# maxpit/human-pose-estimation

Measured on AMD Instinct MI355X. Metric: images/sec (224x224, batch 256/GPU), higher is better.
Workload: dtype f32; 1 GPU; batch=256/GPU 224x224x3 synthetic images, fp32 ResNet-50 v1 + 3-iter regressor + SMPL LBS at all 3 stages (configs[1] at batch 256; the BASELINE metric batch); global_batch=256, parallelism=dp1 (batch shard, replicated weights), regressor=synthetic 'survey' variant, input=float32 images resident in HBM

## Files before the change

human-pose-estimation_amd/_lib.py:

```python
from __future__ import annotations

import ctypes as C
import os

import numpy as np

_HERE = os.path.dirname(os.path.abspath(__file__))
LIB_PATH = os.path.join(_HERE, "lib", "libhpe_hip.so")

NUM_CONV = 53
NUM_DENSE = 3
NUM_CRITIC_DENSE = 9
NUM_VERTS = 6890
THETA_DIM = 85
FEATURE_DIM = 2048


class HpeError(RuntimeError):
    pass


class HpeConfig(C.Structure):
    _fields_ = [
        ("struct_size", C.c_int),
# ... 109 lines not shown
                ("shift", C.c_void_p), ("y", C.c_void_p), ("split_k", C.POINTER(C.c_int))]


CONV_KERNELS = ("f32", "f32s", "bf16", "bf16_p8", "halo3", "wino", "wino_fused", "wino4", "wino4_fused")
BLOCK_JOINS = ("separate", "dual", "chain")


class HpeConvRoute(C.Structure):
    _fields_ = [("struct_size", C.c_int), ("kernel", C.c_int), ("mode", C.c_int), ("tile", C.c_int), ("in_slab8", C.c_int), ("out_slab8", C.c_int),
                ("join", C.c_int), ("join_kernel", C.c_int), ("join_tile", C.c_int), ("next_slab8", C.c_int), ("packs", C.c_uint), ("reserved", C.c_int)]


def conv_route(lib, cfg, idx, B, concurrent=False, residual=False, workspace=True):
    r = HpeConvRoute(struct_size=C.sizeof(HpeConvRoute))
    check(lib.hpe_debug_conv_route(C.byref(cfg), int(idx), int(B), int(concurrent), int(residual), int(workspace), C.byref(r)))
    return r


ENCODER_PACKINGS = ("w", "w_split", "wino_u", "wino4_u", "stem_w", "scale", "shift", "w_dual", "w_dual_split", "shift_dual", "dxw", "flat")

OUTPUT_FIELDS = ("verts", "joints", "cams", "theta", "J_transformed", "kp2d", "verts2d", "Rs")


class HpeOutputs(C.Structure):
    _fields_ = [(n, C.c_void_p) for n in OUTPUT_FIELDS]


REDUCE_FN = C.CFUNCTYPE(C.c_int, C.c_void_p, C.c_void_p, C.c_longlong, C.c_void_p)

_PROTOS = {
    "hpe_last_error": (C.c_char_p, []),
    "hpe_version": (C.c_char_p, []),
    "hpe_conv_layer_name": (C.c_char_p, [C.c_int]),
    "hpe_bn_layer_name": (C.c_char_p, [C.c_int]),
    "hpe_conv_layer_geometry": (C.c_int, [C.c_int, C.POINTER(C.c_int)]),
    "hpe_config_init": (None, [C.POINTER(HpeConfig)]),
    "hpe_create": (C.c_int, [C.POINTER(HpeConfig), C.POINTER(C.c_void_p)]),
    "hpe_destroy": (C.c_int, [C.c_void_p]),
    "hpe_load_smpl": (C.c_int, [C.c_void_p, C.POINTER(HpeSmplModel)]),
    "hpe_load_conv": (C.c_int, [C.c_void_p, C.c_int] + [C.c_void_p] * 6),
    "hpe_load_dense": (C.c_int, [C.c_void_p, C.c_int, C.c_void_p, C.c_void_p]),
    "hpe_load_mean_theta": (C.c_int, [C.c_void_p, C.c_void_p]),
    "hpe_finalize": (C.c_int, [C.c_void_p]),
    "hpe_forward": (C.c_int, [C.c_void_p, C.c_void_p, C.c_int, C.POINTER(HpeOutputs), C.c_int, C.c_void_p]),
    "hpe_forward_pipelined": (C.c_int, [C.c_void_p, C.c_void_p, C.c_int, C.POINTER(HpeOutputs), C.c_int, C.c_void_p]),
    "hpe_join": (C.c_int, [C.c_void_p, C.c_void_p]),
    "hpe_tail": (C.c_int, [C.c_void_p, C.c_void_p, C.c_int, C.POINTER(HpeOutputs), C.c_int, C.c_void_p]),
    "hpe_tail_stream": (C.c_void_p, [C.c_void_p]),
    "hpe_encoder": (C.c_int, [C.c_void_p, C.c_void_p, C.c_int, C.c_void_p, C.c_void_p]),
    "hpe_regress_stage": (C.c_int, [C.c_void_p, C.c_void_p, C.c_void_p, C.c_int, C.c_void_p, C.c_void_p]),
    "hpe_smpl": (C.c_int, [C.c_void_p, C.c_void_p, C.c_int, C.POINTER(HpeOutputs), C.c_void_p]),
    "hpe_smpl_backward": (C.c_int, [C.c_void_p, C.c_void_p, C.c_int, C.POINTER(HpeOutputs), C.c_void_p, C.c_void_p]),
    "hpe_orth_proj": (C.c_int, [C.c_void_p, C.c_void_p, C.c_int, C.c_int, C.c_void_p, C.c_void_p]),
    "hpe_reproject_vertices": (C.c_int, [C.c_void_p, C.c_void_p, C.c_int, C.c_int, C.c_float, C.c_float, C.c_void_p, C.c_void_p]),
    "hpe_preprocess_u8": (C.c_int, [C.c_void_p, C.c_int, C.c_int, C.c_int, C.c_void_p, C.POINTER(C.c_int), C.c_void_p]),
    "hpe_preprocess_u8_batch": (C.c_int, [C.c_void_p, C.POINTER(C.c_longlong), C.POINTER(C.c_int), C.c_int, C.c_int, C.c_void_p, C.POINTER(C.c_int),
                                          C.c_void_p, C.c_void_p]),
    "hpe_augment_plan": (C.c_int, [C.c_int, C.c_void_p, C.c_void_p, C.c_void_p, C.c_void_p, C.c_void_p, C.c_int, C.c_void_p, C.c_void_p, C.c_void_p]),
    "hpe_augment_batch": (C.c_int, [C.c_void_p, C.c_void_p, C.c_void_p, C.c_void_p, C.c_void_p, C.c_int, C.c_void_p, C.c_void_p, C.c_void_p, C.c_void_p]),
    "hpe_adam_advance": (C.c_int, [C.c_void_p, C.c_double, C.c_double, C.c_double, C.c_void_p]),
    "hpe_adam_apply": (C.c_int, [C.c_void_p, C.c_void_p, C.c_void_p, C.c_void_p, C.c_longlong, C.c_void_p, C.c_float, C.c_float, C.c_float, C.c_void_p]),
    "hpe_adam_set_step": (C.c_int, [C.c_void_p, C.c_longlong, C.c_double, C.c_double, C.c_void_p]),
    "hpe_debug_adam_power": (C.c_int, [C.c_double, C.c_longlong, C.POINTER(C.c_double)]),
    "hpe_jpeg_info": (C.c_int, [C.c_int, C.c_void_p, C.c_void_p, C.c_void_p]),
    "hpe_jpeg_decode": (C.c_int, [C.c_int, C.c_void_p, C.c_void_p, C.c_void_p, C.c_int, C.c_void_p, C.c_longlong, C.c_void_p, C.c_void_p, C.c_void_p]),
    "hpe_jpeg_backend": (C.c_int, [C.c_void_p, C.c_void_p, C.c_int, C.c_void_p, C.c_longlong, C.c_void_p, C.c_longlong, C.c_void_p, C.c_longlong,
                                   C.c_void_p]),
    "hpe_jpeg_encode_layout": (C.c_int, [C.c_int, C.c_void_p, C.c_void_p, C.c_int, C.c_int, C.c_int, C.c_void_p, C.c_void_p]),
    "hpe_jpeg_forward": (C.c_int, [C.c_void_p, C.c_void_p, C.c_int, C.c_void_p, C.c_longlong, C.c_void_p, C.c_longlong, C.c_void_p]),
    "hpe_jpeg_entropy_encode": (C.c_int, [C.c_void_p, C.c_int, C.c_void_p, C.c_longlong, C.c_int, C.c_int, C.c_int, C.c_int, C.c_void_p, C.c_longlong,
                                          C.c_void_p, C.c_void_p]),
    "hpe_png_backend": (C.c_int, [C.c_void_p, C.c_void_p, C.c_int, C.c_void_p, C.c_longlong, C.c_void_p, C.c_longlong, C.c_void_p, C.c_longlong,
                                  C.c_void_p]),
    "hpe_png_filter": (C.c_int, [C.c_void_p, C.c_void_p, C.c_int, C.c_void_p, C.c_longlong, C.c_void_p, C.c_longlong, C.c_void_p]),
    "hpe_draw_panels": (C.c_int, [C.c_void_p] * 6 + [C.c_int, C.c_int, C.c_int, C.c_void_p, C.c_void_p]),
    "hpe_draw_skeleton": (C.c_int, [C.c_void_p] * 4 + [C.c_int, C.c_int, C.c_int, C.c_int, C.c_int, C.c_void_p]),
    "hpe_get_original": (C.c_int, [C.c_void_p, C.c_void_p, C.c_int, C.c_int, C.c_int, C.POINTER(C.c_int), C.c_float, C.c_int, C.c_void_p, C.POINTER(C.c_float), C.c_void_p, C.c_void_p, C.c_void_p]),
    "hpe_kp_loss": (C.c_int, [C.c_void_p, C.c_void_p, C.c_int, C.c_int, C.c_void_p, C.c_void_p]),
    "hpe_kp_loss_backward": (C.c_int, [C.c_void_p, C.c_void_p, C.c_int, C.c_int, C.c_void_p, C.c_void_p, C.c_void_p]),
    "hpe_mesh_loss": (C.c_int, [C.c_void_p, C.c_void_p, C.c_void_p, C.c_int, C.c_int, C.c_int, C.c_int, C.c_void_p, C.c_void_p]),
    "hpe_mesh_loss_grad": (C.c_int, [C.c_void_p, C.c_void_p, C.c_void_p, C.c_int, C.c_int, C.c_int, C.c_int, C.c_void_p, C.c_void_p, C.c_void_p,
                                     C.c_void_p, C.c_void_p]),
    "hpe_val_losses": (C.c_int, [C.c_void_p, C.c_void_p, C.c_void_p, C.POINTER(C.c_void_p), C.POINTER(C.c_void_p), C.c_int, C.c_int, C.c_int,
                                 C.c_int, C.c_int, C.c_int, C.c_void_p, C.c_void_p]),
    "hpe_critic_layer_name": (C.c_char_p, [C.c_int]),
    "hpe_critic_layer_shape": (C.c_int, [C.c_int, C.POINTER(C.c_int)]),
    "hpe_load_critic": (C.c_int, [C.c_void_p, C.POINTER(HpeCriticModel)]),
    "hpe_critic": (C.c_int, [C.c_void_p, C.c_void_p, C.c_int, C.c_void_p, C.c_int, C.c_void_p, C.c_int, C.c_void_p, C.c_void_p, C.c_void_p]),
    "hpe_critic_backward": (C.c_int, [C.c_void_p, C.c_void_p, C.c_int, C.c_void_p, C.c_int, C.c_void_p, C.c_int, C.c_void_p, C.c_void_p,
                                      C.c_void_p, C.c_void_p, C.c_void_p, C.c_void_p]),
    "hpe_critic_param_floats": (C.c_int, []),
    "hpe_critic_param_offset": (C.c_int, [C.c_int, C.c_int]),
    "hpe_critic_weight_grad_ws_floats": (C.c_longlong, [C.c_int]),
    "hpe_critic_reserve": (C.c_int, [C.c_void_p, C.c_int]),
    "hpe_critic_weight_grad": (C.c_int, [C.c_void_p, C.c_void_p, C.c_int, C.c_void_p, C.c_int, C.c_void_p, C.c_int, C.c_void_p, C.c_void_p,
                                         C.c_void_p, C.c_void_p, C.c_void_p, C.c_int, C.c_void_p, C.c_void_p]),
    "hpe_critic_get_params": (C.c_int, [C.c_void_p, C.c_void_p, C.c_void_p]),
    "hpe_critic_set_params_dev": (C.c_int, [C.c_void_p, C.c_void_p, C.c_void_p]),
    "hpe_regressor_param_floats": (C.c_int, []),
    "hpe_regressor_param_offset": (C.c_int, [C.c_int, C.c_int]),
    "hpe_regressor_get_params": (C.c_int, [C.c_void_p, C.c_void_p, C.c_void_p]),
    "hpe_regressor_set_params_dev": (C.c_int, [C.c_void_p, C.c_void_p, C.c_void_p]),
    "hpe_regressor_forward_train": (C.c_int, [C.c_void_p, C.c_void_p, C.c_int, C.c_void_p, C.c_void_p, C.c_void_p]),
    "hpe_regressor_backward": (C.c_int, [C.c_void_p, C.c_void_p, C.c_int, C.c_void_p, C.c_void_p, C.c_void_p, C.c_void_p, C.c_void_p]),
    "hpe_encoder_param_floats": (C.c_int, []),
    "hpe_encoder_param_offset": (C.c_int, [C.c_int, C.c_int]),
    "hpe_encoder_train_reserve": (C.c_int, [C.c_void_p, C.c_int]),
    "hpe_encoder_train_ws_floats": (C.c_longlong, [C.c_int]),
    "hpe_encoder_wg_slices": (C.c_int, [C.c_int, C.c_int]),
    "hpe_encoder_forward_train": (C.c_int, [C.c_void_p, C.c_void_p, C.c_int, C.c_void_p, C.c_void_p]),
    "hpe_encoder_backward": (C.c_int, [C.c_void_p, C.c_void_p, C.c_int, C.c_void_p, C.c_void_p, C.c_void_p]),
    "hpe_encoder_get_params": (C.c_int, [C.c_void_p, C.c_void_p, C.c_void_p]),
    "hpe_encoder_set_params": (C.c_int, [C.c_void_p, C.c_void_p]),
    "hpe_encoder_set_params_dev": (C.c_int, [C.c_void_p, C.c_void_p, C.c_void_p]),
    "hpe_debug_encoder_packing_bytes": (C.c_longlong, [C.c_void_p, C.c_int, C.c_int]),
    "hpe_debug_encoder_packing": (C.c_int, [C.c_void_p, C.c_int, C.c_int, C.c_void_p, C.c_void_p]),
    "hpe_debug_conv_backward": (C.c_int, [C.c_void_p, C.c_int, C.c_void_p, C.c_void_p, C.c_void_p, C.c_int, C.c_void_p, C.c_void_p, C.c_void_p]),
    "hpe_debug_maxpool_backward": (C.c_int, [C.c_void_p, C.c_void_p, C.c_int, C.c_int, C.c_int, C.c_void_p, C.c_void_p]),
    "hpe_debug_avgpool_backward": (C.c_int, [C.c_void_p, C.c_int, C.c_int, C.c_int, C.c_void_p, C.c_void_p]),
    "hpe_debug_encoder_stash": (C.c_int, [C.c_void_p, C.c_int, C.c_void_p, C.c_void_p]),
    "hpe_debug_encoder_stash_batch": (C.c_int, [C.c_void_p]),
    "hpe_encoder_stat_floats": (C.c_int, []),
    "hpe_encoder_stat_offset": (C.c_int, [C.c_int, C.c_int]),
    "hpe_encoder_train_reserve_batchnorm": (C.c_int, [C.c_void_p, C.c_int]),
    "hpe_encoder_train_ws_floats_batchnorm": (C.c_longlong, [C.c_int]),
    "hpe_debug_encoder_bn_slices": (C.c_int, [C.c_int, C.c_int]),
    "hpe_encoder_forward_batchnorm": (C.c_int, [C.c_void_p, C.c_void_p, C.c_int, C.c_void_p, C.c_void_p]),
    "hpe_encoder_backward_batchnorm": (C.c_int, [C.c_void_p, C.c_void_p, C.c_int, C.c_void_p, C.c_void_p, C.c_void_p]),
    "hpe_encoder_get_stats": (C.c_int, [C.c_void_p, C.c_void_p, C.c_void_p]),
    "hpe_encoder_update_stats": (C.c_int, [C.c_void_p, C.c_void_p, C.c_double, C.c_int, C.c_void_p]),
    "hpe_encoder_set_stats_dev": (C.c_int, [C.c_void_p, C.c_void_p, C.c_void_p]),
    "hpe_debug_conv_batchnorm": (C.c_int, [C.c_void_p, C.c_int, C.c_void_p, C.c_int, C.c_void_p, C.c_int, C.c_void_p, C.c_void_p, C.c_void_p, C.c_void_p]),
    "hpe_debug_conv_backward_batchnorm": (C.c_int, [C.c_void_p, C.c_int, C.c_void_p, C.c_void_p, C.c_void_p, C.c_void_p, C.c_int, C.c_void_p, C.c_void_p,
                                                    C.c_void_p]),
    "hpe_debug_encoder_stash_raw": (C.c_int, [C.c_void_p, C.c_int, C.c_void_p, C.c_void_p]),
    "hpe_debug_encoder_batch_stats": (C.c_int, [C.c_void_p, C.c_void_p, C.c_void_p]),
    "hpe_encoder_set_reduce": (C.c_int, [C.c_void_p, REDUCE_FN, C.c_void_p, C.c_int]),
    "hpe_debug_bn_sums": (C.c_int, [C.c_void_p, C.c_int, C.c_void_p, C.c_int, C.c_void_p, C.c_void_p]),
    "hpe_debug_bn_finish": (C.c_int, [C.c_void_p, C.c_int, C.c_void_p, C.c_longlong, C.c_void_p, C.c_int, C.c_void_p, C.c_int, C.c_void_p, C.c_void_p,
                                      C.c_void_p]),
    "hpe_debug_bn_backward_sums": (C.c_int, [C.c_void_p, C.c_int, C.c_void_p, C.c_void_p, C.c_void_p, C.c_int, C.c_void_p, C.c_longlong, C.c_void_p,
                                             C.c_void_p]),
    "hpe_debug_bn_backward_finish": (C.c_int, [C.c_void_p, C.c_int, C.c_void_p, C.c_void_p, C.c_void_p, C.c_void_p, C.c_int, C.c_void_p, C.c_void_p,
                                               C.c_longlong, C.c_void_p, C.c_void_p, C.c_void_p]),
    "hpe_device_status": (C.c_int, [C.c_void_p, C.c_void_p]),
    "hpe_debug_conv": (C.c_int, [C.c_void_p, C.c_int, C.c_void_p, C.c_int, C.c_void_p, C.c_int, C.c_void_p, C.c_void_p]),
    "hpe_debug_chain": (C.c_int, [C.c_void_p, C.c_int, C.c_void_p, C.c_void_p, C.c_int, C.c_void_p, C.c_void_p, C.POINTER(C.c_int), C.c_void_p]),
    "hpe_debug_stem": (C.c_int, [C.c_void_p, C.c_void_p, C.c_int, C.c_int, C.c_void_p, C.c_void_p]),
    "hpe_debug_gemm": (C.c_int, [C.c_void_p, C.c_void_p, C.c_void_p, C.c_int, C.c_int, C.c_int, C.c_int, C.c_int, C.c_void_p, C.c_int, C.c_void_p, C.c_void_p]),
    "hpe_debug_gemm_ex": (C.c_int, [C.c_void_p, C.POINTER(HpeDebugGemm), C.c_void_p]),
    "hpe_debug_gemm_check": (C.c_int, [C.POINTER(HpeDebugGemm), C.c_int, C.c_int]),
    "hpe_debug_gemm_launch": (C.c_int, [C.c_void_p, C.POINTER(HpeDebugGemm), C.c_int, C.c_int, C.c_void_p]),
    "hpe_debug_conv_route": (C.c_int, [C.POINTER(HpeConfig), C.c_int, C.c_int, C.c_int, C.c_int, C.c_int, C.POINTER(HpeConvRoute)]),
    "hpe_debug_maxpool": (C.c_int, [C.c_void_p, C.c_int, C.c_int, C.c_int, C.c_void_p, C.c_void_p]),
    "hpe_debug_avgpool": (C.c_int, [C.c_void_p, C.c_int, C.c_int, C.c_int, C.c_void_p, C.c_void_p]),
    "hpe_debug_joint_regress": (C.c_int, [C.c_void_p, C.c_void_p, C.c_int, C.c_int, C.c_void_p, C.c_void_p]),
    "hpe_enable_timing": (C.c_int, [C.c_void_p, C.c_int]),
    "hpe_get_timings": (C.c_int, [C.c_void_p, C.POINTER(C.c_float)]),
    "hpe_get_span_stats": (C.c_int, [C.c_void_p, C.POINTER(C.c_float), C.POINTER(C.c_int)]),
    "hpe_get_loss_timings": (C.c_int, [C.c_void_p, C.POINTER(C.c_float)]),
    "hpe_debug_set_loss_counter": (C.c_int, [C.c_void_p, C.c_void_p]),
    "hpe_get_conv_timings": (C.c_int, [C.c_void_p, C.POINTER(C.c_float)]),
    "hpe_render_params_init": (None, [C.POINTER(HpeRenderParams)]),
    "hpe_renderer_create": (C.c_int, [C.c_int, C.c_void_p, C.c_int, C.c_int, C.c_int, C.POINTER(C.c_void_p)]),
    "hpe_renderer_destroy": (C.c_int, [C.c_void_p]),
    "hpe_render": (C.c_int, [C.c_void_p, C.c_void_p, C.c_void_p, C.c_int, C.c_int, C.c_int, C.c_void_p, C.POINTER(HpeRenderParams), C.c_void_p,
                             C.c_void_p]),
    "hpe_debug_render_ids": (C.c_int, [C.c_void_p, C.c_void_p, C.c_void_p, C.c_int, C.c_int, C.c_int, C.POINTER(HpeRenderParams), C.c_void_p,
                                       C.c_void_p, C.c_void_p]),
    "hpe_debug_render_vertices": (C.c_int, [C.c_void_p, C.c_void_p, C.c_void_p, C.c_int, C.c_int, C.c_int, C.POINTER(HpeRenderParams),
                                            C.c_void_p, C.c_void_p]),
}

_lib = None


def load():
    global _lib
    if _lib is not None:
        return _lib
    if not os.path.exists(LIB_PATH):
        raise HpeError(
            "%s not found: build it with `python -c 'import __graft_entry__ as g; g.build()'` "
            "(hipcc --offload-arch=gfx950).  There is no CPU fallback." % LIB_PATH
        )
    try:
        import torch
    except Exception:
        pass
    lib = C.CDLL(LIB_PATH, mode=C.RTLD_GLOBAL)
    for name, (res, args) in _PROTOS.items():
        fn = getattr(lib, name)
        fn.restype = res
        fn.argtypes = args
    _lib = lib
    return lib


def declared_symbols():
    return sorted(_PROTOS)


def check(rc):
    if rc != 0:
        msg = load().hpe_last_error()
        raise HpeError("libhpe_hip error %d: %s" % (rc, msg.decode() if msg else "?"))


def f32(a):
    arr = np.ascontiguousarray(a, dtype=np.float32)
    return arr, arr.ctypes.data_as(C.c_void_p)
```

human-pose-estimation_amd/build.py:

```python
from __future__ import annotations

import os
import shutil
import subprocess
import sys

HERE = os.path.dirname(os.path.abspath(__file__))
CSRC = os.path.join(HERE, "csrc")
LIBDIR = os.path.join(HERE, "lib")
LIB = os.path.join(LIBDIR, "libhpe_hip.so")
SOURCES = ["conv_gemm.hip", "conv_gemm_f32s.hip", "conv_gemm_bf16.hip", "conv_gemm_bf16_p8.hip", "conv_chain_bf16.hip", "conv_chain_f32.hip", "conv3_halo_bf16.hip", "conv_wino.hip", "conv_wino4.hip", "stem_fused.hip", "encoder_ops.hip", "smpl.hip", "losses.hip", "prepost.hip", "render.hip", "hpe_plan.hip", "hpe_finalize.hip", "hpe_encoder.hip", "hpe_api.hip", "hpe_render_api.hip", "smpl_bwd.hip", "critic.hip", "critic_train.hip", "regressor_train.hip", "augment.hip", "encoder_train.hip", "encoder_grad.hip", "encoder_repack.hip", "encoder_bn.hip", "jpeg_entropy.hip", "jpeg_decode.hip", "jpeg_huffman_enc.hip", "jpeg_encode.hip", "png_decode.hip", "png_encode.hip", "draw.hip", "adam.hip"]
CFLAGS = ["--offload-arch=gfx950", "-O3", "-std=c++17", "-fPIC", "-fvisibility=hidden", "-fno-fast-math"]


def _hipcc():
    for cand in (os.environ.get("HIPCC"), shutil.which("hipcc"), "/opt/rocm/bin/hipcc"):
        if cand and os.path.exists(cand):
            return cand
    raise RuntimeError("hipcc not found (set HIPCC or install ROCm under /opt/rocm)")


def _deps():
    return [os.path.join(CSRC, f) for f in os.listdir(CSRC) if f.endswith(".h")] + [os.path.join(HERE, "..", "include", "hpe.h")]


def _obj_stale(src, obj):
    if not os.path.exists(obj):
        return True
    t = os.path.getmtime(obj)
    return any(os.path.getmtime(d) > t for d in [src] + _deps() if os.path.exists(d))


def _flags_now():
    return " ".join(CFLAGS + os.environ.get("HPE_EXTRA_FLAGS", "").split())


def built_flags():
    tag = os.path.join(LIBDIR, "obj", "flags.txt")
    return open(tag).read() if os.path.exists(tag) else ""


def _stale():
    if not os.path.exists(LIB):
        return True
    if built_flags() != _flags_now():
        return True
    t = os.path.getmtime(LIB)
    deps = [os.path.join(CSRC, f) for f in os.listdir(CSRC)] + [os.path.join(HERE, "..", "include", "hpe.h")]
    return any(os.path.getmtime(d) > t for d in deps if os.path.exists(d))


def build(force=False, verbose=False):
    if not force and not _stale():
        return LIB
    os.makedirs(LIBDIR, exist_ok=True)
    objdir = os.path.join(LIBDIR, "obj")
    os.makedirs(objdir, exist_ok=True)
    extra = os.environ.get("HPE_EXTRA_FLAGS", "").split()
    tag = os.path.join(objdir, "flags.txt")
    flags_now = _flags_now()
    if force or not os.path.exists(tag) or open(tag).read() != flags_now:
        for f in os.listdir(objdir):
            os.remove(os.path.join(objdir, f))
    hipcc = _hipcc()
    jobs = []
    for s in SOURCES:
        src = os.path.join(CSRC, s)
        if not os.path.exists(src):
            continue
        obj = os.path.join(objdir, s.replace(".hip", ".o"))
        jobs.append((src, obj))

    def compile_one(job):
        src, obj = job
        if not _obj_stale(src, obj):
            return None
        cmd = [hipcc] + CFLAGS + extra + ["-c", "-o", obj + ".tmp%d" % os.getpid(), src]
        if verbose:
            print(" ".join(cmd), file=sys.stderr)
        r = subprocess.run(cmd, capture_output=True, text=True)
        if r.returncode != 0:
            return "hipcc failed on %s:\n%s%s" % (os.path.basename(src), r.stdout, r.stderr)
        os.replace(obj + ".tmp%d" % os.getpid(), obj)
        return None

    from concurrent.futures import ThreadPoolExecutor

    with ThreadPoolExecutor(max_workers=min(len(jobs), max(1, (os.cpu_count() or 2) - 1))) as ex:
        errs = [e for e in ex.map(compile_one, jobs) if e]
    if errs:
        raise RuntimeError("\n".join(errs))
    open(tag, "w").write(flags_now)
    tmp = LIB + ".tmp%d" % os.getpid()
    cmd = [hipcc, "--offload-arch=gfx950", "-shared", "-fPIC", "-o", tmp] + [o for _, o in jobs]
    r = subprocess.run(cmd, capture_output=True, text=True)
    if r.returncode != 0:
        raise RuntimeError("link failed:\n" + r.stdout + r.stderr)
    os.replace(tmp, LIB)
    return LIB


if __name__ == "__main__":
    print(build(force="--force" in sys.argv, verbose=True))
```

human-pose-estimation_amd/csrc/conv_gemm_common.h:

```cpp
#pragma once
#include <hip/hip_runtime.h>

#include "hpe_internal.h"

#define BK 32

namespace {

struct RowAddr {
    int base;
    unsigned mask;
};

template <int MODE, int CHUNK = 1>
__device__ __forceinline__ RowAddr make_row(const GemmArgs& p, int m, int c) {
    RowAddr r;
    r.mask = 0x1ffu;
    if (m >= p.M) m = p.M - 1;
    if (MODE == GEMM_DENSE || MODE == GEMM_DUAL) {
        r.base = m * p.lda + c * CHUNK;
    } else {
        const int hw = p.Ho * p.Wo;
        const int b = m / hw;
        const int rem = m - b * hw;
        const int ho = rem / p.Wo;
        const int wo = rem - ho * p.Wo;
        if (MODE == GEMM_STRIDED) {
            r.base = ((b * p.Hi + ho * p.stride) * p.Wi + wo * p.stride) * p.Cin + c * CHUNK;
        } else if (MODE == GEMM_CONV3) {
            r.base = ((b * p.Hi + ho) * p.Wi + wo) * p.Cin + c * CHUNK;
            unsigned mk = 0;
#pragma unroll
            for (int tap = 0; tap < 9; ++tap) {
                const int dh = tap / 3 - 1, dw = tap % 3 - 1;
                if ((unsigned)(ho + dh) < (unsigned)p.Hi && (unsigned)(wo + dw) < (unsigned)p.Wi) mk |= 1u << tap;
            }
            r.mask = mk;
        } else {
            r.base = ((b * p.Hi + 2 * ho + (c * CHUNK >> 5)) * p.Wi + 2 * wo) * 4 + (c * CHUNK & 31);
        }
    }
    return r;
}

struct SlabPos {
    int off;
    int tap;
    int cs;
};

template <int MODE, int SLAB = BK, int STEM_ROWS = 1>
__device__ __forceinline__ void slab_advance(const GemmArgs& p, SlabPos& sp) {
    if (MODE == GEMM_DENSE || MODE == GEMM_STRIDED || MODE == GEMM_DUAL) {
        sp.off += SLAB;
    } else if (MODE == GEMM_CONV3) {
        sp.cs += 1;
        sp.off += SLAB;
        if (sp.cs == p.cin_slabs) {
            sp.cs = 0;
            sp.tap += 1;
            const int kh = sp.tap / 3;
            sp.off = ((kh - 1) * p.Wi + (sp.tap - kh * 3 - 1)) * p.Cin;
        }
    } else {
        sp.off += STEM_ROWS * p.Wi * 4;
    }
}

template <int MODE>
__device__ __forceinline__ SlabPos slab_first(const GemmArgs& p) {
    SlabPos sp;
    sp.tap = 0;
    sp.cs = 0;
    sp.off = (MODE == GEMM_CONV3) ? (-p.Wi - 1) * p.Cin : 0;
    return sp;
}

template <int MODE>
__device__ __forceinline__ SlabPos slab_seek(const GemmArgs& p, int slab) {
    SlabPos sp;
    sp.tap = 0;
    sp.cs = 0;
    if (MODE == GEMM_DENSE || MODE == GEMM_STRIDED || MODE == GEMM_DUAL) {
        sp.off = slab * BK;
    } else if (MODE == GEMM_CONV3) {
        sp.tap = slab / p.cin_slabs;
        sp.cs = slab - sp.tap * p.cin_slabs;
        const int kh = sp.tap / 3;
        sp.off = ((kh - 1) * p.Wi + (sp.tap - kh * 3 - 1)) * p.Cin + sp.cs * BK;
    } else {
        sp.off = slab * p.Wi * 4;
    }
    return sp;
}

#ifdef HPE_F32_RES_NT
#define HPE_RES_LOAD(ptr) __builtin_nontemporal_load(ptr)
#else
#define HPE_RES_LOAD(ptr) (*(ptr))
#endif
template <int BM, int BN, int WM, int WN, int NP>
__device__ __forceinline__ void conv_epilogue(const GemmArgs& p, float* lds, f32x16 (&acc)[BM / WM / 32][BN / WN / 32], int m0, int n0, int t,
                                              int lane, int wm, int wn, const f32x4 (&rpre)[NP], bool use_pre) {
    constexpr int MT = BM / WM / 32;
    constexpr int NT = BN / WN / 32;
    constexpr int NTHR = 64 * WM * WN;
    constexpr int EP = BN + 4;
    {
        const int col_l = lane & 31;
        const int row_l = 4 * (lane >> 5);
#pragma unroll
        for (int j = 0; j < NT; ++j) {
            const int cl = (wn * NT + j) * 32 + col_l;
            const int n = n0 + cl;
            const bool n_ok = n < p.N;
            const float sc = n_ok ? p.scale[n] : 0.f;
            const float sh = n_ok ? p.shift[n] : 0.f;
#pragma unroll
            for (int i = 0; i < MT; ++i) {
                const int rl = (wm * MT + i) * 32 + row_l;
#pragma unroll
                for (int e = 0; e < 16; ++e) lds[(rl + (e & 3) + 8 * (e >> 2)) * EP + cl] = acc[i][j][e] * sc + sh;
            }
        }
    }
    __syncthreads();
    {
        constexpr int TPR = BN / 4;
        constexpr int RPP = NTHR / TPR;
        const int r = t / TPR;
        const int c4 = (t - r * TPR) * 4;
        const int n = n0 + c4;
        const bool full = (n + 3) < p.N;
#pragma unroll
        for (int pass = 0; pass < BM / RPP; ++pass) {
            const int row = pass * RPP + r;
            const int m = m0 + row;
            if (m >= p.M || n >= p.N) continue;
            f32x4 v = *reinterpret_cast<const f32x4*>(&lds[row * EP + c4]);
            if (full) {
                if (use_pre) v += rpre[pass < NP ? pass : 0];
                else if (p.res) v += HPE_RES_LOAD(reinterpret_cast<const f32x4*>(p.res + (size_t)m * p.ldres + n));
                if (p.relu) {
                    v.x = fmaxf(v.x, 0.f);
                    v.y = fmaxf(v.y, 0.f);
                    v.z = fmaxf(v.z, 0.f);
                    v.w = fmaxf(v.w, 0.f);
                }
                if (p.y_slab8)
                    *reinterpret_cast<f32x4*>(p.y + ((size_t)(n >> 3) * p.M + m) * 8 + (n & 7)) = v;
                else
                    *reinterpret_cast<f32x4*>(p.y + (size_t)m * p.ldy + n) = v;
            } else {
                const float vv[4] = {v.x, v.y, v.z, v.w};
#pragma unroll
                for (int u = 0; u < 4; ++u) {
                    if (n + u < p.N) {
                        float o = vv[u];
                        if (p.res) o += p.res[(size_t)m * p.ldres + n + u];
                        if (p.relu) o = fmaxf(o, 0.f);
                        p.y[(size_t)m * p.ldy + n + u] = o;
                    }
                }
            }
        }
    }
}

}
```

human-pose-estimation_amd/csrc/encoder_repack.hip:

```cpp
#include <hip/hip_runtime.h>

#include <string>

#include "hpe_ctx.h"

namespace {

struct RepackLayer {
    float *w, *scale, *shift, *wino_u, *wino4_u, *dxw;
    unsigned short* w_split;
    short kh, wino_split;
    int cin, cout, n_pad, k_pad;
    int off[4];
    int stat;
};

struct RepackDual {
    float *w, *shift;
    unsigned short* split;
    int i2c, i1, K1, K2, N, n_pad;
};

enum { F_WT, F_BN, F_WINO, F_WINO4, F_DXW, F_DUAL, F_COUNT };

// ... 67 lines not shown

__global__ __launch_bounds__(256) void repack_stem_kernel(unsigned short* __restrict__ stem_w, const float* __restrict__ kernel) {
    const int o = blockIdx.x * 256 + threadIdx.x;
    if (o >= 64 * 224) return;
    const int n = o / 224, k = o - n * 224;
    const int kh = k >> 5, kw = (k & 31) >> 2, ci = k & 3;
    float v = 0.f;
    if (kw < 7 && ci < 3) v = kernel[((kh * 7 + kw) * 3 + ci) * 64 + n];
    store_split(stem_w + o, 64 * 224, v);
}

template <int TT>
__global__ __launch_bounds__(256) void repack_wino_kernel(const RepackTable* __restrict__ T, const float* __restrict__ flat) {
    unsigned lb;
    const RepackLayer& L = T->L[find_item(T->F[TT == 4 ? F_WINO : F_WINO4], blockIdx.x, &lb)];
    const int c4 = L.cin / 4;
    const int nb = lb / c4, cb = lb - nb * c4;
    const int n = nb * 64 + (threadIdx.x >> 2), ci = cb * 4 + (threadIdx.x & 3);
    const float* src = flat + L.off[0];
    double g[3][3];
#pragma unroll
    for (int a = 0; a < 3; ++a)
#pragma unroll
        for (int b = 0; b < 3; ++b) g[a][b] = src[(((size_t)a * 3 + b) * L.cin + ci) * L.cout + n];
    float* out = TT == 4 ? L.wino_u + wino_u_base(n, ci, L.cin) : L.wino4_u + wino4_u_base(n, ci, L.cin);
    constexpr size_t step = TT == 4 ? 512 : 256;
#pragma unroll
    for (int xi = 0; xi < TT; ++xi)
#pragma unroll
        for (int nu = 0; nu < TT; ++nu) {
            double gx[3], gn[3];
#pragma unroll
            for (int a = 0; a < 3; ++a) {
                gx[a] = TT == 4 ? wino_g(xi, a) : wino4_g(xi, a);
                gn[a] = TT == 4 ? wino_g(nu, a) : wino4_g(nu, a);
            }
            const float u = wino_elem(gx, gn, g);
            out[(size_t)(xi * TT + nu) * step] = u;
            if (TT == 4 && L.wino_split)
                store_split(wino_u_split_of(L.wino_u, L.cin, L.cout) + wino_us_base(n, ci, L.cin) + (size_t)(xi * 4 + nu) * 512, WINO_US_PIECE, u);
        }
}

__global__ __launch_bounds__(256) void repack_dxw_kernel(const RepackTable* __restrict__ T, const float* __restrict__ flat) {
    unsigned lb;
    const RepackLayer& L = T->L[find_item(T->F[F_DXW], blockIdx.x, &lb)];
    const int taps = L.kh * L.kh, K = taps * L.cout;
    const unsigned o = lb * 256 + threadIdx.x;
    const int ci = (int)(o / (unsigned)K), r = (int)(o - (unsigned)ci * K);
    if (ci >= ((L.cin + 127) / 128) * 128) return;
    const int t = r / L.cout, n = r - t * L.cout;
    L.dxw[o] = ci < L.cin ? flat[L.off[0] + ((size_t)(taps - 1 - t) * L.cin + ci) * L.cout + n] : 0.f;
}

__global__ __launch_bounds__(256) void repack_dual_kernel(const RepackTable* __restrict__ T, const float* __restrict__ flat,
                                                          const float* __restrict__ mean, const double* __restrict__ sd) {
#pragma clang fp contract(off)
    unsigned lb;
    const RepackDual& D = T->D[find_item(T->F[F_DUAL], blockIdx.x, &lb)];
    const int K = D.K1 + D.K2;
    const int kt_n = (K + TILE_K - 1) / TILE_K;
    const int nt = lb / kt_n, kt = lb - nt * kt_n;
    const int k = kt * TILE_K + (threadIdx.x & 63);
    if (k >= K) return;
    const RepackLayer &L2 = T->L[D.i2c], &L1 = T->L[D.i1];
    const RepackLayer& L = k < D.K1 ? L2 : L1;
    const float* src = flat + L.off[0] + (size_t)(k < D.K1 ? k : k - D.K1) * D.N;
    const int n0 = nt * TILE_N + (threadIdx.x >> 6) * 8;
#pragma unroll
    for (int j = 0; j < 8; ++j) {
        const int n = n0 + j;
        if (n >= D.n_pad) break;
        float v = 0.f;
        if (n < D.N) {
            double inv, shift;
            bn_fold_sd(flat[L.off[2] + n], flat[L.off[1] + n], mean[L.stat + n], flat[L.off[3] + n], sd[L.stat + n], &inv, &shift);
            v = (float)(inv * (double)src[n]);
            if (k == 0) {
                double inv1, shift1;
                bn_fold_sd(flat[L1.off[2] + n], flat[L1.off[1] + n], mean[L1.stat + n], flat[L1.off[3] + n], sd[L1.stat + n], &inv1, &shift1);
                D.shift[n] = (float)(shift + shift1);
            }
        }
        D.w[(size_t)n * K + k] = v;
        if (D.split) store_split(D.split + (size_t)n * 3 * K + k, K, v);
    }
}

unsigned blocks_of(int form, const ConvSpec& s, const ConvLayer& L, int idx) {
    switch (form) {
        case F_WT: return (unsigned)(L.n_pad / TILE_N) * ((L.k_pad + TILE_K - 1) / TILE_K);
        case F_BN: return (unsigned)(s.cout + 255) / 256;
        case F_WINO: return L.wino_u ? (unsigned)(s.cin / 4) * (s.cout / 64) : 0;
        case F_WINO4: return L.wino4_u ? (unsigned)(s.cin / 4) * (s.cout / 64) : 0;
        case F_DXW: return (unsigned)((conv_dxw_floats(idx) + 255) / 256);
    }
    return 0;
}

int check_debug(hpe_ctx* c, int idx, int which) {
    if (!c) return fail(HPE_ERR_INVALID, "null ctx");
    if (idx < 0 || idx >= HPE_NUM_CONV || which < 0 || which >= HPE_PACK_COUNT) return fail(HPE_ERR_INVALID, "hpe_debug_encoder_packing: idx or which out of range");
    if (c->dead) return fail(HPE_ERR_STATE, "hpe_finalize failed on this ctx: destroy it and create a new one");
    if (!c->finalized) return fail(HPE_ERR_STATE, "hpe_finalize() has not been called");
    if (!c->have_encoder) return fail(HPE_ERR_STATE, "encoder weights were not loaded before hpe_finalize");
    if (c->bf16) return fail(HPE_ERR_STATE, "hpe_debug_encoder_packing needs an fp32 context");
    return HPE_OK;
}

const void* packing_of(hpe_ctx* c, int idx, int which, size_t* bytes) {
    const ConvSpec& s = specs()[idx];
    const ConvLayer& L = c->conv[idx];
    const size_t wt = (size_t)L.n_pad * L.k_pad, dual = (size_t)round_up(s.cout, 128) * L.k_dual, u = (size_t)s.cin * s.cout;
    const void* p = nullptr;
    size_t n = 0;
    switch (which) {
        case HPE_PACK_W: p = L.w, n = wt * 4; break;
        case HPE_PACK_W_SPLIT: p = L.w_split, n = wt * 3 * 2; break;
        case HPE_PACK_WINO_U: p = L.wino_u, n = u * 16 * 4; break;
        case HPE_PACK_WINO4_U: p = L.wino4_u, n = u * 36 * 4; break;
        case HPE_PACK_STEM_W: p = L.stem_w, n = (size_t)3 * 64 * 224 * 2; break;
        case HPE_PACK_SCALE: p = L.scale, n = (size_t)s.cout * 4; break;
        case HPE_PACK_SHIFT: p = L.shift, n = (size_t)s.cout * 4; break;
        case HPE_PACK_W_DUAL: p = L.w_dual, n = dual * 4; break;
        case HPE_PACK_W_DUAL_SPLIT: p = L.w_dual_split, n = dual * 3 * 2; break;
        case HPE_PACK_SHIFT_DUAL: p = L.shift_dual, n = (size_t)s.cout * 4; break;
        case HPE_PACK_DXW: p = c->et.dxw[idx], n = conv_dxw_floats(idx) * 4; break;
        case HPE_PACK_FLAT:
            if (c->et.flat) p = c->et.flat + layout().off[idx][0];
            n = ((size_t)s.kh * s.kw * s.cin * s.cout + 3 * (size_t)s.cout) * 4;
            break;
    }
    *bytes = p ? n : 0;
    return *bytes ? p : nullptr;
}

}

size_t encoder_repack_reserve_floats() { return (sizeof(RepackTable) + 3) / 4; }

int encoder_repack_reserve(hpe_ctx* c) {
    RepackTable t{};
    for (int i = 0; i < HPE_NUM_CONV; ++i) {
        const ConvSpec& s = specs()[i];
        const ConvLayer& L = c->conv[i];
        RepackLayer& r = t.L[i];
        r.w = L.w;
        r.scale = L.scale;
        r.shift = L.shift;
        r.wino_u = L.wino_u;
        r.wino_split = L.wino_u_split != nullptr;
        r.wino4_u = L.wino4_u;
        r.dxw = c->et.dxw[i];
        r.w_split = static_cast<unsigned short*>(L.w_split);
        r.kh = s.kh;
        r.cin = s.cin;
        r.cout = s.cout;
        r.n_pad = L.n_pad;
        r.k_pad = L.k_pad;
        for (int w = 0; w < 4; ++w) r.off[w] = layout().off[i][w];
        r.stat = layout().stat[i];
        if (s.kh != s.kw || L.n_pad % TILE_N != 0 || ((L.wino_u || L.wino4_u) && (s.cin % 8 != 0 || s.cout % 64 != 0)))
            return fail(HPE_ERR_STATE, std::string("encoder repack: unexpected geometry of ") + s.name);
    }
    for (int f = 0; f < F_DUAL; ++f) {
        RepackForm& F = t.F[f];
        unsigned b = 0;
        for (int i = 0; i < HPE_NUM_CONV; ++i) {
            const unsigned nb = blocks_of(f, specs()[i], c->conv[i], i);
            if (!nb) continue;
            F.item[F.n] = i;
            F.block0[F.n++] = b;
            b += nb;
        }
        F.block0[F.n] = b;
    }
    {
        RepackForm& F = t.F[F_DUAL];
        unsigned b = 0;
        for (const ResBlock& blk : blocks()) {
            if (!blk.first || !c->conv[blk.i2c].w_dual) continue;
            const ConvLayer& L2 = c->conv[blk.i2c];
            RepackDual& d = t.D[F.n];
            d.w = L2.w_dual;
            d.shift = L2.shift_dual;
            d.split = static_cast<unsigned short*>(L2.w_dual_split);
            d.i2c = blk.i2c;
            d.i1 = blk.i1;
            d.K1 = L2.k1_dual;
            d.K2 = L2.k_dual - L2.k1_dual;
            d.N = specs()[blk.i2c].cout;
            d.n_pad = round_up(d.N, 128);
            F.item[F.n] = F.n;
            F.block0[F.n++] = b;
            b += (unsigned)(d.n_pad / TILE_N) * ((L2.k_dual + TILE_K - 1) / TILE_K);
        }
        F.block0[F.n] = b;
    }
    float* p = nullptr;
    int rc = dev_alloc(c, &p, encoder_repack_reserve_floats(), false);
    if (rc) return rc;
    HIP_TRY(hipMemcpy(p, &t, sizeof(t), hipMemcpyHostToDevice));
    c->et.repack = p;
    static_assert(F_COUNT <= 8, "grid array");
    for (int f = 0; f < F_COUNT; ++f) c->et.repack_grid[f] = t.F[f].block0[t.F[f].n];
    return HPE_OK;
}

hipError_t encoder_repack_launch(hpe_ctx* c, const float* flat, hipStream_t st) {
    const EncTrainWork& w = c->et;
    const RepackTable* T = static_cast<const RepackTable*>(w.repack);
    const unsigned* grid = w.repack_grid;
    if (grid[F_WT]) hipLaunchKernelGGL(repack_wt_kernel, dim3(grid[F_WT]), dim3(256), 0, st, T, flat);
    if (grid[F_BN]) hipLaunchKernelGGL(repack_bn_kernel, dim3(grid[F_BN]), dim3(256), 0, st, T, flat, w.mean, w.sd);
    if (c->conv[0].stem_w)
        hipLaunchKernelGGL(repack_stem_kernel, grid1(64 * 224), dim3(256), 0, st, static_cast<unsigned short*>(c->conv[0].stem_w),
                           flat + layout().off[0][0]);
    if (grid[F_WINO]) hipLaunchKernelGGL(repack_wino_kernel<4>, dim3(grid[F_WINO]), dim3(256), 0, st, T, flat);
    if (grid[F_WINO4]) hipLaunchKernelGGL(repack_wino_kernel<6>, dim3(grid[F_WINO4]), dim3(256), 0, st, T, flat);
    if (grid[F_DXW]) hipLaunchKernelGGL(repack_dxw_kernel, dim3(grid[F_DXW]), dim3(256), 0, st, T, flat);
    if (grid[F_DUAL]) hipLaunchKernelGGL(repack_dual_kernel, dim3(grid[F_DUAL]), dim3(256), 0, st, T, flat, w.mean, w.sd);
    HIPE(hipGetLastError());
    return hipMemcpyAsync(w.flat, flat, (size_t)layout().total * sizeof(float), hipMemcpyDeviceToDevice, st);
}

hipError_t encoder_repack_stats_launch(hpe_ctx* c, hipStream_t st) {
    const EncTrainWork& w = c->et;
    const RepackTable* T = static_cast<const RepackTable*>(w.repack);
    const unsigned* grid = w.repack_grid;
    if (grid[F_BN]) hipLaunchKernelGGL(repack_bn_kernel, dim3(grid[F_BN]), dim3(256), 0, st, T, w.flat, w.mean, w.sd);
    if (grid[F_DUAL]) hipLaunchKernelGGL(repack_dual_kernel, dim3(grid[F_DUAL]), dim3(256), 0, st, T, w.flat, w.mean, w.sd);
    return hipGetLastError();
}

#pragma GCC visibility push(default)
extern "C" {

long long hpe_debug_encoder_packing_bytes(hpe_ctx* c, int idx, int which) {
    if (!c || idx < 0 || idx >= HPE_NUM_CONV || which < 0 || which >= HPE_PACK_COUNT) return 0;
    if (c->dead || !c->finalized || !c->have_encoder || c->bf16) return 0;
    size_t n;
    packing_of(c, idx, which, &n);
    return (long long)n;
}

int hpe_debug_encoder_packing(hpe_ctx* c, int idx, int which, void* dst, void* stream) {
    int rc = check_debug(c, idx, which);
    if (rc) return rc;
    if (!dst) return fail(HPE_ERR_INVALID, "null dst_dev");
    size_t n;
    const void* p = packing_of(c, idx, which, &n);
    if (!p) return fail(HPE_ERR_STATE, "hpe_debug_encoder_packing: this context does not hold that form of that layer");
    DeviceGuard g(c->cfg.device);
    HIP_TRY(hipMemcpyAsync(dst, p, n, hipMemcpyDeviceToDevice, static_cast<hipStream_t>(stream)));
    return HPE_OK;
}

}
#pragma GCC visibility pop
```

human-pose-estimation_amd/csrc/hpe_api.hip:

```cpp
#include <hip/hip_runtime.h>

#include <algorithm>
#include <cmath>
#include <cstdint>
#include <cstdio>
#include <cstdlib>
#include <cstring>
#include <string>
#include <vector>

#include "gemm_contract.h"
#include "hpe_ctx.h"

namespace {
thread_local std::string g_err;
}

int fail(int code, const std::string& msg) {
    g_err = msg;
    return code;
}

int check_ready(hpe_ctx* c, int B, int need) {
    if (!c) return fail(HPE_ERR_INVALID, "null ctx");
// ... 624 lines not shown
    const ConvSpec& sn = specs()[idx2c + (first ? 2 : 1)];
    const int C2 = first ? specs()[idx2c + 1].cin : 0;
    if (s2.kh != 1 || s2.cout != 4 * s2.cin || sn.kh != 1 || sn.stride != 1 || sn.cin != s2.cout || !hpe_chain_bf16_supported(s2.cin, s2.cout, sn.cout, C2) ||
        (first && (!c->conv[idx2c].w_dual || specs()[idx2c + 1].stride != 1)))
        return fail(HPE_ERR_INVALID, "hpe_debug_chain: idx2c must be the branch2c of a stage-2 / stage-3 block that is followed by an identity block");
    DeviceGuard g(c->cfg.device);
    hipStream_t st = static_cast<hipStream_t>(stream);
    const long M = (long)B * s2.hout * s2.hout;
    HIP_TRY(hpe_launch_f32_to_bf16(t2, c->T2, M * s2.cin, st));
    HIP_TRY(hpe_launch_f32_to_bf16(residual, c->X0, M * (first ? C2 : s2.cout), st));
    HIP_TRY(run_chain(c, idx2c, first, c->T2, c->X0, B, c->X1, c->T1, st));
    HIP_TRY(hpe_launch_bf16_to_f32(c->X1, t3, M * s2.cout, st));
    HIP_TRY(hpe_launch_bf16_to_f32(c->T1, u1, M * sn.cout, st));
    if (occupancy) HIP_TRY(hpe_chain_bf16_occupancy(occupancy));
    return HPE_OK;
}

int hpe_debug_stem(hpe_ctx* c, const float* images, int B, int rows_per_strip, float* y, void* stream) {
    int rc = check_ready(c, B, NEED_ENC);
    if (rc) return rc;
    if (!images || !y) return fail(HPE_ERR_INVALID, "null pointer");
    if (c->bf16) return fail(HPE_ERR_STATE, "hpe_debug_stem works on fp32 contexts only");
    DeviceGuard g(c->cfg.device);
    const int R = rows_per_strip > 0 ? rows_per_strip : hpe_stem_fused_pick_rows(B);
    HIP_TRY(hpe_launch_stem_fused(images, c->conv[0].stem_w, c->conv[0].scale, c->conv[0].shift, y, B, R, 0, static_cast<hipStream_t>(stream)));
    return HPE_OK;
}

static GemmArgs debug_gemm_args(const HpeDebugGemm* g, int slab) {
    static_assert(HPE_GEMM_DENSE == GEMM_DENSE && HPE_GEMM_STRIDED == GEMM_STRIDED && HPE_GEMM_CONV3 == GEMM_CONV3 && HPE_GEMM_DUAL == GEMM_DUAL,
                  "include/hpe.h numbers the modes as GemmMode does");
    GemmArgs p{};
    p.x = g->x, p.x2 = g->x2, p.w = g->wt, p.res = g->residual, p.y = g->y;
    p.M = g->M, p.N = g->N, p.K = g->K;
    p.lda = g->lda, p.ldw = g->ldw, p.ldy = g->ldy, p.ldres = g->ldres, p.w_rows = g->w_rows;
    p.Hi = g->Hi, p.Wi = g->Wi, p.Cin = g->Cin, p.Ho = g->Ho, p.Wo = g->Wo, p.stride = g->stride;
    p.cin_slabs = g->Cin / slab;
    p.k1_slabs = g->k1_slabs;
    p.relu = g->relu;
    p.y_slab8 = g->y_slab8;
    return p;
}

static std::string debug_gemm_refusal(const HpeDebugGemm* g) {
    if (!g) return "null HpeDebugGemm";
    if (g->struct_size != (int)sizeof(HpeDebugGemm))
        return "HpeDebugGemm.struct_size is " + std::to_string(g->struct_size) + ", this library's is " + std::to_string(sizeof(HpeDebugGemm)) +
               " (other revision of include/hpe.h?)";
    if (g->mode != HPE_GEMM_DENSE && g->mode != HPE_GEMM_STRIDED && g->mode != HPE_GEMM_CONV3 && g->mode != HPE_GEMM_DUAL)
        return "HpeDebugGemm.mode must be dense, strided, conv3 or dual";
    return "";
}

static std::string debug_gemm_rejected(const HpeDebugGemm* g, const char* clause) {
    return "mode " + std::to_string(g->mode) + " tile " + std::to_string(g->tile) + " M " + std::to_string(g->M) + " N " + std::to_string(g->N) + " K " +
           std::to_string(g->K) + " is outside the launcher's contract (gemm_contract.h), clause \"" + clause + "\": nothing was launched";
}

int hpe_debug_gemm_ex(hpe_ctx* c, const HpeDebugGemm* g, void* stream) {
    if (g && g->split_k) *g->split_k = 0;
    if (!c || !c->finalized) return fail(HPE_ERR_STATE, "needs a finalized ctx");
    const std::string why = debug_gemm_refusal(g);
    if (!why.empty()) return fail(HPE_ERR_INVALID, why);
    if ((!g->scale || !g->shift) && g->N > 1024) return fail(HPE_ERR_INVALID, "hpe_debug_gemm_ex: N <= 1024 without scale / shift");
    DeviceGuard guard(c->cfg.device);
    GemmArgs p = debug_gemm_args(g, 32);
    p.scale = g->scale ? g->scale : c->ones;
    p.shift = g->shift ? g->shift : c->zeros;
    p.zero = c->zeros;
    if (g->use_splitk) {
        p.partial = c->partial;
        p.partial_floats = c->partial_floats;
    }
    if (const char* clause = gemm_contract(p, g->mode, g->tile, GEMM_K_F32)) return fail(HPE_ERR_INVALID, "hpe_debug_gemm_ex: " + debug_gemm_rejected(g, clause));
    int split_k = 0;
    const hipError_t e = hpe_launch_gemm(p, g->mode, g->tile, c->plan.splitk_min_slabs, static_cast<hipStream_t>(stream), &split_k);
    if (g->split_k) *g->split_k = split_k;
    if (e == hipErrorInvalidValue && split_k == 0) return fail(HPE_ERR_INVALID, "hpe_debug_gemm_ex: the launcher refused the plan's splitk_min_slabs, nothing was launched");
    HIP_TRY(e);
    return HPE_OK;
}

int hpe_debug_gemm_check(const HpeDebugGemm* g, int kernel, int w_piece) {
    const std::string why = debug_gemm_refusal(g);
    if (!why.empty()) return fail(HPE_ERR_INVALID, why);
    if (kernel < GEMM_K_F32 || kernel > GEMM_K_BF16_P8) return fail(HPE_ERR_INVALID, "hpe_debug_gemm_check: kernel must be 0 (fp32), 1 (f32s), 2 (bf16) or 3 (bf16_p8)");
    const GemmKernel k = static_cast<GemmKernel>(kernel);
    GemmArgs p = debug_gemm_args(g, gemm_rules(k).slab);
    alignas(16) static const float present[4] = {};
    p.scale = p.shift = p.zero = present;
    if (k == GEMM_K_F32S) p.w_piece = w_piece;
    if (const char* clause = gemm_contract(p, g->mode, g->tile, k)) return fail(HPE_ERR_INVALID, "hpe_debug_gemm_check: " + debug_gemm_rejected(g, clause));
    return HPE_OK;
}

int hpe_debug_gemm_launch(hpe_ctx* c, const HpeDebugGemm* g, int kernel, int w_piece, void* stream) {
    if (kernel == GEMM_K_F32) return hpe_debug_gemm_ex(c, g, stream);
    if (g && g->split_k) *g->split_k = 0;
    const std::string why = debug_gemm_refusal(g);
    if (!why.empty()) return fail(HPE_ERR_INVALID, why);
    if (kernel < GEMM_K_F32 || kernel > GEMM_K_BF16_P8) return fail(HPE_ERR_INVALID, "hpe_debug_gemm_launch: kernel must be 0 (fp32), 1 (f32s), 2 (bf16) or 3 (bf16_p8)");
    if ((!g->scale || !g->shift) && g->N > 1024) return fail(HPE_ERR_INVALID, "hpe_debug_gemm_launch: N <= 1024 without scale / shift");
    const GemmKernel k = static_cast<GemmKernel>(kernel);
    GemmArgs p = debug_gemm_args(g, gemm_rules(k).slab);
    if (k == GEMM_K_F32S) p.w_piece = w_piece;
    alignas(16) static const float present[4] = {};
    p.scale = g->scale ? g->scale : present;
    p.shift = g->shift ? g->shift : present;
    p.zero = present;
    if (const char* clause = gemm_contract(p, g->mode, g->tile, k)) return fail(HPE_ERR_INVALID, "hpe_debug_gemm_launch: " + debug_gemm_rejected(g, clause));
    if (!c || !c->finalized) return fail(HPE_ERR_STATE, "needs a finalized ctx");
    DeviceGuard guard(c->cfg.device);
    p.scale = g->scale ? g->scale : c->ones;
    p.shift = g->shift ? g->shift : c->zeros;
    p.zero = c->zeros;
    if (g->use_splitk) {
        p.partial = c->partial;
        p.partial_floats = c->partial_floats;
    }
    if (const char* clause = gemm_contract(p, g->mode, g->tile, k)) return fail(HPE_ERR_INVALID, "hpe_debug_gemm_launch: " + debug_gemm_rejected(g, clause));
    int split_k = 1;
    hipStream_t st = static_cast<hipStream_t>(stream);
    const hipError_t e = k == GEMM_K_F32S ? hpe_launch_gemm_f32s(p, g->mode, g->tile, st)
                       : k == GEMM_K_BF16 ? hpe_launch_gemm_bf16(p, g->mode, g->tile, st)
                                          : hpe_launch_gemm_bf16_p8(p, g->mode, st, &split_k);
    if (g->split_k) *g->split_k = split_k;
    HIP_TRY(e);
    return HPE_OK;
}

int hpe_debug_conv_route(const HpeConfig* cfg, int idx, int B, int concurrent, int residual, int workspace, HpeConvRoute* out) {
    static_assert(HPE_CONV_K_F32 == CONV_K_F32 && HPE_CONV_K_HALO3 == CONV_K_HALO3 && HPE_CONV_K_WINO4_FUSED == CONV_K_WINO4_FUSED && HPE_CONV_K_COUNT == CONV_K_WINO4_FUSED + 1,
                  "include/hpe.h numbers the kernels as ConvKernel does");
    if (!cfg || !out) return fail(HPE_ERR_INVALID, "null argument");
    if (cfg->struct_size != (int)sizeof(HpeConfig) || out->struct_size != (int)sizeof(HpeConvRoute))
        return fail(HPE_ERR_INVALID, "hpe_debug_conv_route: HpeConfig.struct_size / HpeConvRoute.struct_size are " + std::to_string(cfg->struct_size) + " / " +
                                         std::to_string(out->struct_size) + ", this library's are " + std::to_string(sizeof(HpeConfig)) + " / " + std::to_string(sizeof(HpeConvRoute)));
    if (idx < 0 || idx >= HPE_NUM_CONV || B < 1) return fail(HPE_ERR_INVALID, "hpe_debug_conv_route: idx must be in [0, HPE_NUM_CONV) and B >= 1");
    const HpePlan pl = hpe_resolve_plan(*cfg);
    const bool bf16 = cfg->encoder_dtype == 1;
    const ConvQuery q{B, concurrent != 0, residual != 0, workspace != 0};
    const ConvRoute r = route_conv(pl, bf16, idx, q);
    *out = HpeConvRoute{(int)sizeof(HpeConvRoute), r.kernel, r.mode, r.tile, r.in_slab8, 0, 0, -1, -1, 0, layer_packs(pl, bf16, idx), 0};
    for (const ResBlock& blk : blocks()) {
        if (idx != blk.i2a && idx != blk.i2c) continue;
        const BlockRoute b = route_block(pl, bf16, blk, q);
        if (idx == blk.i2a) out->out_slab8 = b.r2a.out_slab8;
        if (idx == blk.i2c) out->join = b.join, out->next_slab8 = b.u1_slab8;
        if (idx == blk.i2c && b.join == JOIN_DUAL) out->join_kernel = b.r2c.kernel, out->join_tile = b.r2c.tile;
    }
    return HPE_OK;
}

int hpe_debug_gemm(hpe_ctx* c, const float* x, const float* wt, int M, int N, int K, int w_rows, int tile, const float* residual,
                   int relu, float* y, void* stream) {
    if (!c || !c->finalized || !c->have_regressor) return fail(HPE_ERR_STATE, "needs a finalized ctx with the regressor loaded");
    if (!x || !wt || !y || N > 1024) return fail(HPE_ERR_INVALID, "bad argument (N <= 1024)");
    HpeDebugGemm g{};
    g.struct_size = (int)sizeof(HpeDebugGemm);
    g.mode = HPE_GEMM_DENSE;
    g.tile = tile;
    g.x = x;
    g.wt = wt;
    g.residual = residual;
    g.y = y;
    g.M = M;
    g.N = N;
    g.K = K;
    g.lda = K;
    g.ldw = K;
    g.w_rows = w_rows;
    g.ldy = N;
    g.ldres = N;
    g.relu = relu;
    g.use_splitk = 0;
    return hpe_debug_gemm_ex(c, &g, stream);
}

int hpe_debug_maxpool(const float* x, int B, int H, int C, float* y, void* stream) {
    if (!x || !y || B < 1) return fail(HPE_ERR_INVALID, "bad argument");
    HIP_TRY(hpe_launch_maxpool(x, y, B, H, C, static_cast<hipStream_t>(stream)));
    return HPE_OK;
}

int hpe_debug_avgpool(const float* x, int B, int HW, int C, float* y, void* stream) {
    if (!x || !y || B < 1) return fail(HPE_ERR_INVALID, "bad argument");
    HIP_TRY(hpe_launch_avgpool(x, y, B, HW, C, C, static_cast<hipStream_t>(stream)));
    return HPE_OK;
}

int hpe_debug_joint_regress(hpe_ctx* c, const float* X, int n, int use_kp, float* out, void* stream) {
    if (!c || !c->finalized || !c->have_smpl) return fail(HPE_ERR_STATE, "SMPL not finalized");
    if (!X || !out || n < 1) return fail(HPE_ERR_INVALID, "bad argument");
    DeviceGuard g(c->cfg.device);
    HIP_TRY(hpe_launch_joint_regress(X, use_kp ? c->smpl.kp_reg : c->smpl.j_reg, n, use_kp ? c->num_kp : 24, out, nullptr, nullptr,
                                     static_cast<hipStream_t>(stream)));
    return HPE_OK;
}

int hpe_device_status(hpe_ctx* c, void* stream) {
    if (!c || !c->finalized) return fail(HPE_ERR_STATE, "needs a finalized ctx");
    DeviceGuard g(c->cfg.device);
    HIP_TRY(hipStreamSynchronize(static_cast<hipStream_t>(stream)));
    if (c->dev_err) {
        unsigned w = 0;
        HIP_TRY(hipMemcpy(&w, c->dev_err, sizeof w, hipMemcpyDeviceToHost));
        if (w) {
            (void)hipMemset(c->dev_err, 0, sizeof w);
            return fail(HPE_ERR_HIP, "device error word " + std::to_string(w) +
                                         ": a stream-K wait of the Winograd GEMM timed out, outputs since the last check are invalid");
        }
    }
    return HPE_OK;
}

int hpe_enable_timing(hpe_ctx* c, int enable) {
    if (!c) return fail(HPE_ERR_INVALID, "null ctx");
    c->timing = enable;
    c->span_n = 0;
    c->timed_valid = false;
    c->conv_timed_valid = false;
    return HPE_OK;
}

int hpe_get_timings(hpe_ctx* c, float ms[5]) {
    if (!c || !ms) return fail(HPE_ERR_INVALID, "null argument");
    if (!c->timed_valid) return fail(HPE_ERR_STATE, "no timed call recorded (hpe_enable_timing first)");
    DeviceGuard g(c->cfg.device);
    HIP_TRY(hipEventSynchronize(c->ev[4]));
    for (int i = 0; i < 5; ++i) ms[i] = 0.f;
    HIP_TRY(hipEventElapsedTime(&ms[0], c->ev[0], c->ev[1]));
    HIP_TRY(hipEventElapsedTime(&ms[4], c->ev[0], c->ev[4]));
    if (c->conv_timed_valid) {
        for (int i = 0; i < HPE_NUM_CONV; ++i) {
            float t = 0.f;
            HIP_TRY(hipEventElapsedTime(&t, c->cev0[i], c->cev1[i]));
            ms[1] += t;
        }
    }
    ms[2] = ms[4] - ms[0];
    return HPE_OK;
}

int hpe_get_span_stats(hpe_ctx* c, float ms[3], int* n_calls) {
    if (!c || !ms || !n_calls) return fail(HPE_ERR_INVALID, "null argument");
    if (c->span_n == 0) return fail(HPE_ERR_STATE, "no timed call recorded (hpe_enable_timing first)");
    DeviceGuard g(c->cfg.device);
    const unsigned n = c->span_n < (unsigned)hpe_ctx::SPAN_RING ? c->span_n : (unsigned)hpe_ctx::SPAN_RING;
    double sum = 0.0;
    float lo = 1e30f, hi = 0.f;
    for (unsigned i = 0; i < n; ++i) {
        float t = 0.f;
        HIP_TRY(hipEventSynchronize(c->span1[i]));
        HIP_TRY(hipEventElapsedTime(&t, c->span0[i], c->span1[i]));
        sum += t;
        lo = t < lo ? t : lo;
        hi = t > hi ? t : hi;
    }
    ms[0] = (float)(sum / n);
    ms[1] = lo;
    ms[2] = hi;
    *n_calls = (int)n;
    return HPE_OK;
}

int hpe_get_loss_timings(hpe_ctx* c, float ms[2]) {
    if (!c || !ms) return fail(HPE_ERR_INVALID, "null argument");
    if (c->loss_timed_stages == 0) return fail(HPE_ERR_STATE, "no timed hpe_val_losses call recorded (hpe_enable_timing first)");
    DeviceGuard g(c->cfg.device);
    HIP_TRY(hipEventSynchronize(c->lev_all[1]));
    HIP_TRY(hipEventElapsedTime(&ms[0], c->lev_all[0], c->lev_all[1]));
    ms[1] = 0.f;
    for (int s = 0; s < c->loss_timed_stages; ++s) {
        float t = 0.f;
        HIP_TRY(hipEventElapsedTime(&t, c->lev0[s], c->lev1[s]));
        ms[1] += t;
    }
    return HPE_OK;
}

int hpe_debug_set_loss_counter(hpe_ctx* c, void* counter_dev) {
    if (!c) return fail(HPE_ERR_INVALID, "null ctx");
    c->loss_counter = static_cast<unsigned long long*>(counter_dev);
    return HPE_OK;
}

int hpe_get_conv_timings(hpe_ctx* c, float* ms) {
    if (!c || !ms) return fail(HPE_ERR_INVALID, "null argument");
    if (!c->conv_timed_valid) return fail(HPE_ERR_STATE, "no level-2 timed call recorded");
    DeviceGuard g(c->cfg.device);
    HIP_TRY(hipEventSynchronize(c->ev[4]));
    for (int i = 0; i < HPE_NUM_CONV; ++i) HIP_TRY(hipEventElapsedTime(&ms[i], c->cev0[i], c->cev1[i]));
    return HPE_OK;
}

}
#pragma GCC visibility pop
```

human-pose-estimation_amd/csrc/hpe_ctx.h:

```cpp
#pragma once
#include <hip/hip_runtime.h>

#include <cmath>
#include <cstdint>
#include <cstring>
#include <string>
#include <vector>

#include "../../include/hpe.h"
#include "bf16_split.h"
#include "hpe_internal.h"
#include "hpe_plan.h"

int fail(int code, const std::string& msg);

#define HIP_TRY(expr)                                                                                             \
    do {                                                                                                          \
        hipError_t _e = (expr);                                                                                   \
        if (_e != hipSuccess)                                                                                     \
            return fail(HPE_ERR_HIP, std::string(#expr) + ": " + hipGetErrorString(_e) + " (" __FILE__ ":" +      \
                                         std::to_string(__LINE__) + ")");                                         \
    } while (0)

struct ConvSpec {
    char name[24];
    char bn[24];
    int kh, kw, cin, cout, stride, hin, hout;
};

const std::vector<ConvSpec>& specs();

struct ResBlock {
    int stage;
    bool first, last;
    int i2a, i2b, i2c, i1;
    int in;
};
const std::vector<ResBlock>& blocks();

inline int round_up(int x, int m) { return ((x + m - 1) / m) * m; }

struct ConvLayer {
    std::vector<float> kernel, bias, gamma, beta, mean, var;
    bool loaded = false;
    float* w = nullptr;
    float* scale = nullptr;
    float* shift = nullptr;
    float* w_dual = nullptr;
    float* shift_dual = nullptr;
    int k_dual = 0, k1_dual = 0;
    void* w_split = nullptr;
    void* w_dual_split = nullptr;
    void* stem_w = nullptr;
    float* wino_u = nullptr;
    unsigned short* wino_u_split = nullptr;
    float* wino4_u = nullptr;
    int n_pad = 0, k_pad = 0;
};

inline int conv_wt_k(int idx, int kh, int kw, int ci) {
    const ConvSpec& s = specs()[idx];
    return idx == 0 ? kh * 32 + kw * 4 + ci : (kh * s.kw + kw) * s.cin + ci;
}

inline int conv_k_pad(int idx, bool bf16) { return round_up(idx == 0 ? 7 * 32 : specs()[idx].kh * specs()[idx].kw * specs()[idx].cin, bf16 ? 64 : 32); }


__host__ __device__ inline size_t wino_u_base(int n, int ci, int cin) {
    return ((((size_t)(n >> 6) * (cin / 8) + (ci >> 3)) * 16) * 2 + ((ci >> 2) & 1)) * 256 + (size_t)(n & 63) * 4 + (ci & 3);
}
constexpr size_t WINO_US_PIECE = 16 * 64 * 8;
__host__ __device__ inline size_t wino_us_base(int n, int ci, int cin) {
    return ((size_t)(n >> 6) * (cin / 8) + (ci >> 3)) * 3 * WINO_US_PIECE + (size_t)(n & 63) * 8 + (ci & 7);
}
__host__ __device__ inline unsigned short* wino_u_split_of(float* wino_u, int cin, int cout) {
    return reinterpret_cast<unsigned short*>(wino_u + (size_t)16 * cin * cout);
}
__host__ __device__ inline size_t wino4_u_base(int n, int ci, int cin) {
    return (((size_t)(n >> 6) * (cin / 4) + (ci >> 2)) * 36) * 256 + (size_t)(n & 63) * 4 + (ci & 3);
}
__host__ __device__ inline double wino_g(int xi, int a) {
    constexpr double G[4][3] = {{1, 0, 0}, {0.5, 0.5, 0.5}, {0.5, -0.5, 0.5}, {0, 0, 1}};
    return G[xi][a];
}
__host__ __device__ inline double wino4_g(int xi, int a) {
    constexpr double G4[6][3] = {{0.25, 0, 0}, {-1.0 / 6, -1.0 / 6, -1.0 / 6}, {-1.0 / 6, 1.0 / 6, -1.0 / 6},
                                 {1.0 / 24, 1.0 / 12, 1.0 / 6}, {1.0 / 24, -1.0 / 12, 1.0 / 6}, {0, 0, 1}};
    return G4[xi][a];
}
__host__ __device__ inline float wino_elem(const double gx[3], const double gn[3], const double g[3][3]) {
#pragma clang fp contract(off)
    double u = 0.0;
    for (int a = 0; a < 3; ++a)
        for (int b = 0; b < 3; ++b) u += gx[a] * gn[b] * g[a][b];
    return (float)u;
}

__host__ __device__ inline void bn_fold_sd(float gamma, float bias, float mean, float beta, double sd, double* scale, double* shift) {
#pragma clang fp contract(off)
    *scale = (double)gamma / sd;
    *shift = ((double)bias - (double)mean) * *scale + (double)beta;
}
inline double bn_sd(const ConvLayer& L, int n, float eps) { return std::sqrt((double)L.var[n] + (double)eps); }
inline void bn_fold(const ConvLayer& L, int n, float eps, double* scale, double* shift) {
    bn_fold_sd(L.gamma[n], L.bias[n], L.mean[n], L.beta[n], bn_sd(L, n, eps), scale, shift);
}
inline float bn_istd(const ConvLayer& L, int n, float eps) { return (float)(1.0 / std::sqrt((double)L.var[n] + (double)eps)); }

struct DenseLayer {
    std::vector<float> kernel, bias;
    bool loaded = false;
};

constexpr int STEM_HP = 230;
constexpr int STEM_WP = 232;
constexpr int THETA_LD = 96;
constexpr size_t WINO_V_PITCH = 802816 + 16384;
constexpr size_t WINO_V_SLACK = 524288;


struct RegTrainWork {
    float *w1k = nullptr;
    float *w2k = nullptr;
    float *w3k = nullptr;
    float *p1 = nullptr;
    float *a1 = nullptr, *a2 = nullptr;
    float *th = nullptr;
    float *g = nullptr;
    float *r = nullptr;
    float *da = nullptr;
    float *dz1 = nullptr, *dz2 = nullptr;
    float *sum1 = nullptr;
    float *zeros = nullptr;
    float *partial = nullptr;
    size_t partial_floats = 0;
};

struct EncTrainWork {
    int B = 0;
    int stash_B = 0;
    float *flat = nullptr;
    float *mean = nullptr, *istd = nullptr;
    double *sd = nullptr;
    void *repack = nullptr;
    unsigned repack_grid[8] = {};
    float *stash = nullptr;
    float *g0 = nullptr, *g1 = nullptr;
    float *sbig = nullptr;
    float *t0 = nullptr, *t1 = nullptr, *ssmall = nullptr;
    float *partial = nullptr;
    size_t partial_floats = 0;
    float *dsh = nullptr;
    float *wgp = nullptr;
    float *zeros = nullptr;
    float *feat = nullptr;
    float *dxw[HPE_NUM_CONV] = {};
    int bn_B = 0;
    int bn_stat_B = 0;
    float *zstash = nullptr;
    float *bn_batch = nullptr;
    float *bn_stats = nullptr;
    double *bn_part = nullptr;
    int *bn_hw = nullptr;
    hpe_reduce_fn reduce = nullptr;
    void *reduce_user = nullptr;
    int reduce_G = 0;
    int reduce_failed = -1;
    int bn_stat_G = 0;
};
constexpr int BN_MAX_SLICES = 512;
constexpr int BN_PART_COLS = 262144;
constexpr int WG_MAX_SLICES = 128;
constexpr int WG_WGP_FLOATS = 1152 * 512;
static_assert(WG_WGP_FLOATS >= 3 * 2 * 2048, "the reduce buffers of data-parallel training fit the weight gradient's scratch");
inline size_t conv_dxw_floats(int idx) {
    const ConvSpec& s = specs()[idx];
    return idx == 0 ? 0 : (size_t)round_up(s.cin, 128) * s.kh * s.kw * s.cout;
}
struct EncLayout {
    int off[HPE_NUM_CONV][4];
    int stat[HPE_NUM_CONV];
    size_t stash[HPE_NUM_CONV];
    size_t stash_pool, stash_per_image;
    int total, channels;
};
const EncLayout& layout();

struct hpe_ctx {
    HpeConfig cfg{};
    bool finalized = false;
    bool dead = false;
    HpePlan plan;
    bool bf16 = false;
    bool have_encoder = false, have_regressor = false, have_smpl = false;
    ConvLayer conv[HPE_NUM_CONV];
    DenseLayer dense[HPE_NUM_DENSE];
    bool smpl_loaded = false, mean_loaded = false;
    std::vector<float> h_vt, h_sd, h_pd, h_jreg, h_w, h_kreg;
    std::vector<int> h_par;
    int num_kp = 19;
    float h_mean[HPE_THETA_DIM];
    float *w1f = nullptr, *w1t = nullptr, *w2 = nullptr, *w3 = nullptr, *b1 = nullptr, *b2 = nullptr, *b3 = nullptr;
    float *ones = nullptr, *zeros = nullptr, *mean_dev = nullptr;
    EncTrainWork et{};
    RegTrainWork rt{};
    SmplDev smpl{};
    SmplWork work{};
    SmplBwdWork bwd{};
    float* smpl_basis_src = nullptr;
    float *padded = nullptr, *X0 = nullptr, *X1 = nullptr, *T1 = nullptr, *T2 = nullptr, *SC = nullptr;
    float *feat = nullptr, *P1 = nullptr, *H1 = nullptr, *H2 = nullptr, *thA = nullptr, *thB = nullptr;
    float* critic_buf = nullptr;
    CriticW critic{};
    bool have_critic = false;
    float* critic_ws = nullptr;
    size_t critic_ws_floats = 0;
    float* loss_ws = nullptr;
    size_t loss_ws_floats = 0;
    std::vector<void*> allocs;
    float* partial = nullptr;
    size_t partial_floats = 0;
    float* wino_v = nullptr;
    float* wino_ws = nullptr;
    unsigned* wino_flags = nullptr;
    unsigned* dev_err = nullptr;
    unsigned wino_epoch = 0;
    int n_cu = 0;
    bool loss_attr_done = false;
    unsigned long long* loss_counter = nullptr;
    hipStream_t aux[3]{};
    hipEvent_t ev_fork{}, ev_join[3]{};
    hipStream_t tail_st{};
    hipEvent_t ev_enc{}, ev_tail{}, ev_feat_free[2]{};
    bool feat_free_valid[2] = {false, false};
    bool tail_pending = false;
    unsigned pipe_idx = 0;
    float* feat_alt = nullptr;
    int co_running = 1;
    float* w4_split = nullptr;
    float* partial_tail = nullptr;
    size_t partial_tail_floats = 0;
    bool dense_on_tail = false;
    int timing = 0;
    hipEvent_t ev[8]{};
    static constexpr int SPAN_RING = 64;
    hipEvent_t span0[SPAN_RING]{}, span1[SPAN_RING]{};
    unsigned span_n = 0;
    hipEvent_t cev0[HPE_NUM_CONV]{}, cev1[HPE_NUM_CONV]{};
    hipEvent_t lev0[16]{}, lev1[16]{}, lev_all[2]{};
    int loss_timed_stages = 0;
    bool ev_ok = false, timed_valid = false, conv_timed_valid = false;
};

struct DeviceGuard {
    int prev = -1;
    bool changed = false;
    explicit DeviceGuard(int dev) {
        if (hipGetDevice(&prev) == hipSuccess && prev != dev) changed = hipSetDevice(dev) == hipSuccess;
    }
    ~DeviceGuard() {
        if (changed) (void)hipSetDevice(prev);
    }
};

int dev_alloc(hpe_ctx* c, float** p, size_t n_floats, bool zero);
int upload(hpe_ctx* c, float** p, const std::vector<float>& h);
int upload_split(hpe_ctx* c, void** p, const std::vector<float>& wt, int rows, int K);

#define HIPE(expr)                               \
    do {                                         \
        hipError_t _e = (expr);                  \
        if (_e != hipSuccess) return _e;         \
    } while (0)

enum { NEED_ENC = 1, NEED_REG = 2, NEED_SMPL = 4 };
int check_ready(hpe_ctx* c, int B, int need);

int finalize_impl(hpe_ctx* c);
void release_device_state(hpe_ctx* c);
int repack_encoder(hpe_ctx* c);

hipError_t run_conv(hpe_ctx* c, int idx, const ConvRoute& r, const float* x, int B, const float* res, int relu, float* y, hipStream_t st,
                    float* wino_v = nullptr, int slot = 0, const float* scale = nullptr, const float* shift = nullptr);
hipError_t run_conv_nhwc(hpe_ctx* c, int idx, const float* x, int B, const float* res, int relu, float* y, hipStream_t st,
                         const float* scale = nullptr, const float* shift = nullptr);
hipError_t run_chain(hpe_ctx* c, int i2c, bool first, const float* t2, const float* res, int B, float* t3, float* u1, hipStream_t st,
                     bool u1_slab8 = false);
hipError_t encoder_impl(hpe_ctx* c, const float* images, int B, float* features, int ldfeat, hipStream_t st);
hipError_t run_dense(hpe_ctx* c, const float* x, int lda, int M, int K, const float* w, int w_rows, int N, const float* scale, const float* shift,
                     const float* res, int ldres, int relu, float* y, int ldy, hipStream_t st, float* partial = nullptr, size_t partial_floats = 0);
hipError_t regress_impl(hpe_ctx* c, const float* th_prev, float* th_next, int B, hipStream_t st);
hipError_t features_proj(hpe_ctx* c, const float* features, int B, hipStream_t st);
hipError_t tail_impl(hpe_ctx* c, const float* feat, int B, const HpeOutputs* stage_outs, int n_outs, hipStream_t ts, hipEvent_t feat_free);
hipError_t join_tail(hpe_ctx* c, hipStream_t st);
int forward_impl(hpe_ctx* c, const float* images, int B, const HpeOutputs* stage_outs, int n_outs, hipStream_t st, bool pipelined);

size_t encoder_repack_reserve_floats();
int encoder_repack_reserve(hpe_ctx* c);
hipError_t encoder_repack_launch(hpe_ctx* c, const float* flat_dev, hipStream_t st);

hipError_t encoder_repack_stats_launch(hpe_ctx* c, hipStream_t st);

int bn_slices(int M, int N);
hipError_t bn_launch_stats(const float* z, int M, int N, float eps, double* part, float* mu, float* var, float* r, hipStream_t st);
hipError_t bn_launch_apply(const float* z, const float* mu, const float* r, const float* gamma, const float* beta, const float* res, int relu, float* y,
                           int M, int N, hipStream_t st);
hipError_t bn_launch_bwd_reduce(const float* dy, const float* y, const float* z, const float* mu, const float* r, int M, int N, double* part, float* db,
                                float* dgamma, float* dbeta, hipStream_t st);
hipError_t bn_launch_bwd_apply(const float* dy, const float* y, const float* z, const float* mu, const float* r, const float* gamma, const float* dgamma,
                               const float* dbeta, int M, int N, float* dz, float* dzraw, hipStream_t st, double M_all = 0.0);
hipError_t bn_launch_stats_sums(const float* z, int M, int N, double* part, double* sums, hipStream_t st);
hipError_t bn_launch_stats_from_sums(const double* sums, double M_all, int N, float eps, float* mu, float* var, float* r, hipStream_t st);
hipError_t bn_launch_bwd_sums(const float* dy, const float* y, const float* z, const float* mu, const float* r, int M, int N, double* part, double* sums,
                              float* db, float* dgamma, float* dbeta, hipStream_t st);
hipError_t bn_launch_bwd_from_sums(const double* sums, int N, float* red, hipStream_t st);
hipError_t bn_launch_momentum(float* stats, const float* batch, const int* hw, int B, int channels, double momentum, int unbiased, hipStream_t st);
hipError_t bn_launch_install(const float* stats, int channels, float eps, float* keep, float* mean, float* istd, double* sd, hipStream_t st);

void wg_slicing(int idx, int B, int* P, int* slices);
size_t wg_partial_floats(int B);
void gate(const float* dy, const float* y, const float* s, float* dz, float* dzs, long n, int N, hipStream_t st);
hipError_t weight_grad(hpe_ctx* c, int idx, const float* x, const float* dz, int B, float* grad_layer, hipStream_t st, bool bn = false);
hipError_t data_grad(hpe_ctx* c, int idx, const float* dzs, int B, const float* res, float* out, hipStream_t st);
void scatter2(const float* lo, float* hi, int B, int H, int C, hipStream_t st);
void avgpool_bwd(const float* dy, float* dx, int B, int HW, int C, hipStream_t st);
void maxpool_bwd(const float* x, const float* dy, float* dx, int B, int H, int C, hipStream_t st);

int regressor_param_offset(int idx, bool bias);
hipError_t regressor_train_forward(hpe_ctx* c, const float* features, int B, const float* drop, hipStream_t st);
hipError_t regressor_train_backward(hpe_ctx* c, const float* features, int B, const float* drop, const float* grad_thetas, float* grad_flat,
                                    float* grad_features, hipStream_t st);
hipError_t regressor_params_copy(hpe_ctx* c, float* flat, bool set, hipStream_t st);
```

human-pose-estimation_amd/csrc/hpe_encoder.hip:

```cpp
#include <hip/hip_runtime.h>

#include <cmath>
#include <cstdint>
#include <cstdio>
#include <cstdlib>
#include <cstring>
#include <string>
#include <vector>

#include "hpe_ctx.h"

static hipError_t launch_gemm(hpe_ctx* c, GemmArgs& p, const ConvRoute& r, const void* w_split, hipStream_t st) {
    if (!r.concurrent) p.partial = c->partial, p.partial_floats = c->partial_floats;
    if (r.kernel == CONV_K_BF16 || r.kernel == CONV_K_BF16_P8) return hpe_launch_gemm_bf16(p, r.mode, r.tile, st);
    if (r.kernel != CONV_K_F32S) return hpe_launch_gemm(p, r.mode, r.tile, c->plan.splitk_min_slabs, st);
    if (!w_split) return hipErrorInvalidValue;
    p.w = static_cast<const float*>(w_split);
    p.w_piece = p.ldw;
    p.ldw *= 3;
    return hpe_launch_gemm_f32s(p, r.mode, r.tile, st);
}

hipError_t run_conv(hpe_ctx* c, int idx, const ConvRoute& r, const float* x, int B, const float* res, int relu, float* y, hipStream_t st,
                    float* wino_v, int slot, const float* scale, const float* shift) {
    const ConvSpec& s = specs()[idx];
    const ConvLayer& L = c->conv[idx];
    if (!scale) scale = L.scale;
    if (!shift) shift = L.shift;
    const int H = s.hin;
    const bool f2 = r.kernel == CONV_K_WINO || r.kernel == CONV_K_WINO_FUSED, f4 = r.kernel == CONV_K_WINO4 || r.kernel == CONV_K_WINO4_FUSED;
    if ((r.kernel >= CONV_K_HALO3 && res) || (f2 && !L.wino_u) || (f4 && !L.wino4_u) || ((f2 || f4) && !r.in_slab8 && !wino_v)) return hipErrorInvalidValue;
    switch (r.kernel) {
        case CONV_K_WINO4_FUSED: return hpe_launch_wino4_fused_conv3(x, L.wino4_u, scale, shift, c->zeros, y, s.cout, B, H, H, s.cin, s.cout, relu, st);
        case CONV_K_WINO_FUSED: return hpe_launch_wino_fused_conv3(x, L.wino_u_split, scale, shift, c->zeros, y, s.cout, B, H, H, s.cin, s.cout, relu, st);
        case CONV_K_WINO4:
            return hpe_launch_wino4_conv3(x, s.cin, L.wino4_u, scale, shift, y, s.cout, B, H, H, s.cin, s.cout, relu, wino_v, st, r.concurrent ? c->co_running : 1,
                                          c->w4_split && slot >= 0 && slot < 4 ? c->w4_split + (size_t)slot * hpe_wino4_split_ws_floats() : nullptr, c->plan.wino4_n32,
                                          c->plan.w4_abl);
        case CONV_K_WINO: {
            WinoStreamK sk{};
            if (c->wino_ws && slot >= 0 && slot < 4) {
                sk.ws = c->wino_ws + (size_t)slot * c->n_cu * HPE_WINO_WS_FLOATS;
                sk.flags = c->wino_flags + (size_t)slot * c->n_cu;
                sk.epoch = ++c->wino_epoch;
                if (sk.epoch == 0) sk.epoch = ++c->wino_epoch;
                sk.n_wg = c->n_cu;
                sk.err = c->dev_err;
            }
            return hpe_launch_wino_conv3(x, s.cin, L.wino_u, scale, shift, y, s.cout, B, H, H, s.cin, s.cout, relu, wino_v, c->wino_ws ? &sk : nullptr, st);
        }
        case CONV_K_HALO3: {
            Halo3Args h{};
            h.x = reinterpret_cast<const __bf16*>(x), h.w = reinterpret_cast<const __bf16*>(L.w), h.y = reinterpret_cast<__bf16*>(y);
            h.scale = scale, h.shift = shift;
            h.M = B * s.hout * s.hout, h.N = s.cout, h.ldw = L.k_pad;
            h.relu = relu, h.two = c->plan.halo3_two;
            return hpe_launch_halo3_bf16(h, H, s.cin, st);
        }
    }
    GemmArgs p{};
    p.x = x, p.w = L.w, p.scale = scale, p.shift = shift, p.res = res, p.y = y, p.zero = c->zeros;
    p.M = B * s.hout * s.hout, p.N = s.cout, p.K = L.k_pad;
    p.lda = s.cin, p.ldw = L.k_pad, p.w_rows = L.n_pad, p.ldy = p.ldres = s.cout;
    p.Hi = p.Wi = H, p.Cin = s.cin, p.Ho = p.Wo = s.hout, p.stride = s.stride;
    p.cin_slabs = s.cin / (c->bf16 ? 64 : 32);
    p.relu = relu, p.y_slab8 = r.out_slab8 ? 1 : 0;
    if (r.mode == GEMM_STEM) p.Hi = STEM_HP, p.Wi = STEM_WP, p.Cin = 4;
    return launch_gemm(c, p, r, L.w_split, st);
}

hipError_t run_conv_nhwc(hpe_ctx* c, int idx, const float* x, int B, const float* res, int relu, float* y, hipStream_t st, const float* scale,
                         const float* shift) {
    const ConvRoute r = route_conv(c->plan, c->bf16, idx, ConvQuery{B, false, res != nullptr, c->wino_v != nullptr});
    if (r.in_slab8) {
        const ConvSpec& s = specs()[idx];
        HIPE(hpe_launch_nhwc_to_slab8(x, c->T1, (long)B * s.hin * s.hin, s.cin, st));
        x = c->T1;
    }
    return run_conv(c, idx, r, x, B, res, relu, y, st, c->wino_v, 0, scale, shift);
}

static hipError_t run_dual(hpe_ctx* c, int i2c, int i1, const ConvRoute& r, const float* t2, const float* x, int B, float* y, hipStream_t st) {
    const ConvSpec& s2 = specs()[i2c];
    const ConvSpec& s1 = specs()[i1];
    const ConvLayer& L = c->conv[i2c];
    GemmArgs p{};
    p.x = t2, p.x2 = x, p.w = L.w_dual, p.scale = c->ones, p.shift = L.shift_dual, p.y = y, p.zero = c->zeros;
    p.M = B * s2.hout * s2.hout, p.N = s2.cout, p.K = L.k_dual;
    p.k1_slabs = L.k1_dual / (c->bf16 ? 64 : 32), p.relu = 1;
    p.lda = s2.cin, p.ldw = L.k_dual, p.w_rows = round_up(s2.cout, 128), p.ldy = s2.cout;
    p.Hi = p.Wi = s1.hin, p.Cin = s1.cin, p.Ho = p.Wo = s1.hout, p.stride = s1.stride;
    return launch_gemm(c, p, r, L.w_dual_split, st);
}

hipError_t run_chain(hpe_ctx* c, int i2c, bool first, const float* t2, const float* res, int B, float* t3, float* u1, hipStream_t st,
                     bool u1_slab8) {
    const ConvSpec& s2 = specs()[i2c];
    const int inext = i2c + (first ? 2 : 1);
    const ConvSpec& sn = specs()[inext];
    const ConvLayer& L2 = c->conv[i2c];
    const ConvLayer& Ln = c->conv[inext];
    if (!c->bf16) {
        ChainArgsF32 q{};
        q.t2 = t2;
        q.res = res;
        q.w2c = L2.w;
        q.w2a = Ln.w;
        q.scaleA = L2.scale;
        q.shiftA = L2.shift;
        q.scaleB = Ln.scale;
        q.shiftB = Ln.shift;
        q.t3 = t3;
        q.u1 = u1;
        q.M = B * s2.hout * s2.hout;
        q.ldw2c = L2.k_pad;
        q.ldw2a = Ln.k_pad;
        q.u1_slab8 = u1_slab8 ? 1 : 0;
        return hpe_launch_chain_f32(q, s2.cin, s2.cout, sn.cout, st);
    }
    ChainArgs p{};
    p.t2 = reinterpret_cast<const __bf16*>(t2);
    if (first) {
        p.x2 = reinterpret_cast<const __bf16*>(res);
        p.w2c = reinterpret_cast<const __bf16*>(L2.w_dual);
        p.scaleA = c->ones;
        p.shiftA = L2.shift_dual;
        p.ldw2c = L2.k_dual;
    } else {
        p.res = reinterpret_cast<const __bf16*>(res);
        p.w2c = reinterpret_cast<const __bf16*>(L2.w);
        p.scaleA = L2.scale;
        p.shiftA = L2.shift;
        p.ldw2c = L2.k_pad;
    }
    p.w2a = reinterpret_cast<const __bf16*>(Ln.w);
    p.scaleB = Ln.scale;
    p.shiftB = Ln.shift;
    p.t3 = reinterpret_cast<__bf16*>(t3);
    p.u1 = reinterpret_cast<__bf16*>(u1);
    p.M = B * s2.hout * s2.hout;
    p.ldw2a = Ln.k_pad;
    return hpe_launch_chain_bf16(p, s2.cin, s2.cout, sn.cout, first ? specs()[i2c + 1].cin : 0, st);
}

hipError_t run_dense(hpe_ctx* c, const float* x, int lda, int M, int K, const float* w, int w_rows, int N, const float* scale,
                     const float* shift, const float* res, int ldres, int relu, float* y, int ldy, hipStream_t st, float* partial,
                     size_t partial_floats) {
    if (M <= 4) return hpe_launch_dense_gemv(x, lda, M, K, w, N, scale, shift, res, ldres, relu, y, ldy, st);
    GemmArgs p{};
    p.zero = shift;
    p.partial = partial ? partial : c->dense_on_tail ? c->partial_tail : c->partial;
    p.partial_floats = partial ? partial_floats : c->dense_on_tail ? c->partial_tail_floats : c->partial_floats;
    p.x = x;
    p.w = w;
    p.scale = scale;
    p.shift = shift;
    p.res = res;
    p.y = y;
    p.M = M;
    p.N = N;
    p.K = K;
    p.lda = lda;
    p.ldw = K;
    p.w_rows = w_rows;
    p.ldy = ldy;
    p.ldres = ldres;
    p.relu = relu;
    return hpe_launch_gemm(p, GEMM_DENSE, TILE_64x64, c->plan.splitk_min_slabs, st);
}

static hipError_t timed_conv(hpe_ctx* c, int idx, const ConvRoute& r, const float* x, int B, const float* res, int relu, float* y, hipStream_t st,
                             float* wino_v = nullptr, int slot = 0) {
    const bool t2 = c->timing >= 2;
    if (t2) HIPE(hipEventRecord(c->cev0[idx], st));
    HIPE(run_conv(c, idx, r, x, B, res, relu, y, st, wino_v, slot));
    if (t2) HIPE(hipEventRecord(c->cev1[idx], st));
    return hipSuccess;
}

static hipError_t encoder_chunk(hpe_ctx* c, const float* images, int i0, int B, float* features, int ldfeat, hipStream_t st, int slot = 0,
                         bool concurrent = false) {
    const int esz = c->bf16 ? 2 : 4;
    auto at = [&](float* base, size_t elems) { return reinterpret_cast<float*>(reinterpret_cast<char*>(base) + elems * esz); };
    const size_t o_img = (size_t)i0 * HPE_IMG_SIZE * HPE_IMG_SIZE * 3;
    const size_t o_pad = (size_t)i0 * STEM_HP * STEM_WP * 4;
    const size_t o_big = (size_t)i0 * 802816;
    const size_t o_mid = (size_t)i0 * 200704;
    float* padded = at(c->padded, o_pad);
    float* SC = at(c->SC, o_big);
    float* T1 = at(c->T1, o_mid);
    float* T2 = at(c->T2, o_mid);
    float* cur = at(c->X0, o_big);
    float* nxt = at(c->X1, o_big);
    float* wv = (c->wino_v && (i0 == 0 || B >= 32)) ? c->wino_v + (size_t)i0 * WINO_V_PITCH : nullptr;
    const ConvQuery q{B, concurrent, false, wv != nullptr};
    if (c->plan.stem_fused && (reinterpret_cast<uintptr_t>(images + o_img) & 15) == 0) {
        const bool t2 = c->timing >= 2;
        if (t2) HIPE(hipEventRecord(c->cev0[0], st));
        HIPE(hpe_launch_stem_fused(images + o_img, c->conv[0].stem_w, c->conv[0].scale, c->conv[0].shift, cur, B, hpe_stem_fused_pick_rows(B),
                                   c->bf16 ? 1 : 0, st));
        if (t2) HIPE(hipEventRecord(c->cev1[0], st));
    } else if (c->bf16) {
        HIPE(hpe_launch_pad_input_bf16(images + o_img, padded, B, HPE_IMG_SIZE, HPE_IMG_SIZE, STEM_HP, STEM_WP, st));
        HIPE(timed_conv(c, 0, route_conv(c->plan, true, 0, q), padded, B, nullptr, 1, SC, st));
        HIPE(hpe_launch_maxpool_bf16(SC, cur, B, 112, 64, st));
    } else {
        HIPE(hpe_launch_pad_input(images + o_img, padded, B, HPE_IMG_SIZE, HPE_IMG_SIZE, STEM_HP, STEM_WP, st));
        HIPE(timed_conv(c, 0, route_conv(c->plan, false, 0, q), padded, B, nullptr, 1, SC, st));
        HIPE(hpe_launch_maxpool(SC, cur, B, 112, 64, st));
    }
    bool have_2a = false;
    for (const ResBlock& blk : blocks()) {
        const bool first = blk.first;
        const int i2a = blk.i2a, i2b = blk.i2b, i2c = blk.i2c, i1 = blk.i1;
        const BlockRoute br = route_block(c->plan, c->bf16, blk, q);
        if (have_2a) {
            if (c->timing >= 2) {
                HIPE(hipEventRecord(c->cev0[i2a], st));
                HIPE(hipEventRecord(c->cev1[i2a], st));
            }
        } else {
            HIPE(timed_conv(c, i2a, br.r2a, cur, B, nullptr, 1, T1, st));
        }
        have_2a = false;
        HIPE(timed_conv(c, i2b, br.r2b, T1, B, nullptr, 1, T2, st, wv, slot));
        const float* res = cur;
        if (br.join == JOIN_CHAIN) {
            const bool t2 = c->timing >= 2;
            if (t2) HIPE(hipEventRecord(c->cev0[i2c], st));
            HIPE(run_chain(c, i2c, first, T2, cur, B, nxt, T1, st, br.u1_slab8));
            if (t2) {
                HIPE(hipEventRecord(c->cev1[i2c], st));
                if (first) {
                    HIPE(hipEventRecord(c->cev0[i1], st));
                    HIPE(hipEventRecord(c->cev1[i1], st));
                }
            }
            have_2a = true;
        } else if (br.join == JOIN_DUAL) {
            const bool t2 = c->timing >= 2;
            if (t2) HIPE(hipEventRecord(c->cev0[i2c], st));
            HIPE(run_dual(c, i2c, i1, br.r2c, T2, cur, B, nxt, st));
            if (t2) {
                HIPE(hipEventRecord(c->cev1[i2c], st));
// ... 144 lines not shown
```

human-pose-estimation_amd/csrc/hpe_finalize.hip:

```cpp
#include <hip/hip_runtime.h>

#include <algorithm>
#include <cmath>
#include <cstdint>
#include <cstdio>
#include <cstdlib>
#include <cstring>
#include <string>
#include <vector>

#include "hpe_ctx.h"

int dev_alloc(hpe_ctx* c, float** p, size_t n_floats, bool zero) {
    void* q = nullptr;
    HIP_TRY(hipMalloc(&q, n_floats * sizeof(float)));
    c->allocs.push_back(q);
    if (zero) HIP_TRY(hipMemset(q, 0, n_floats * sizeof(float)));
    *p = static_cast<float*>(q);
    return HPE_OK;
}

int upload(hpe_ctx* c, float** p, const std::vector<float>& h) {
    int rc = dev_alloc(c, p, h.size(), false);
    if (rc) return rc;
    HIP_TRY(hipMemcpy(*p, h.data(), h.size() * sizeof(float), hipMemcpyHostToDevice));
    return HPE_OK;
}

static int upload_to(hpe_ctx* c, float** p, const std::vector<float>& h) {
    if (!*p) return upload(c, p, h);
    HIP_TRY(hipMemcpy(*p, h.data(), h.size() * sizeof(float), hipMemcpyHostToDevice));
    return HPE_OK;
}

static int upload_bf16(hpe_ctx* c, void** p, const std::vector<unsigned short>& h) {
    if (!*p) {
        HIP_TRY(hipMalloc(p, h.size() * 2));
        c->allocs.push_back(*p);
    }
    HIP_TRY(hipMemcpy(*p, h.data(), h.size() * 2, hipMemcpyHostToDevice));
    return HPE_OK;
}

static int upload_bf16(hpe_ctx* c, float** p, const std::vector<unsigned short>& h) {
    void* q = *p;
    const int rc = upload_bf16(c, &q, h);
    *p = static_cast<float*>(q);
    return rc;
}

static std::vector<unsigned short> to_bf16(const std::vector<float>& v) {
    std::vector<unsigned short> h(v.size());
    for (size_t q = 0; q < v.size(); ++q) h[q] = f2bf(v[q]);
    return h;
}

int upload_split(hpe_ctx* c, void** p, const std::vector<float>& wt, int rows, int K) {
    std::vector<unsigned short> ws((size_t)rows * 3 * K);
    for (int n = 0; n < rows; ++n)
        for (int k = 0; k < K; ++k) {
            unsigned short h[3];
            bf16_split3(wt[(size_t)n * K + k], h);
            unsigned short* d = &ws[(size_t)n * 3 * K + k];
            d[0] = h[0];
            d[K] = h[1];
            d[2 * K] = h[2];
        }
    return upload_bf16(c, p, ws);
}

#pragma GCC visibility push(default)
extern "C" {

int hpe_load_smpl(hpe_ctx* c, const HpeSmplModel* m) {
    if (!c || !m) return fail(HPE_ERR_INVALID, "null argument");
    if (c->finalized) return fail(HPE_ERR_STATE, "already finalized");
    if (!m->v_template || !m->shapedirs || !m->posedirs || !m->J_regressor || !m->weights || !m->kp_regressor || !m->parents)
        return fail(HPE_ERR_INVALID, "null SMPL array");
    if (m->num_kp < 1 || m->num_kp > HPE_MAX_KP) return fail(HPE_ERR_INVALID, "num_kp must be in [1,24]");
    if (m->parents[0] >= 0) return fail(HPE_ERR_INVALID, "parents[0] must be negative (root)");
    for (int i = 1; i < 24; ++i)
        if (m->parents[i] < 0 || m->parents[i] >= i) return fail(HPE_ERR_INVALID, "parents[i] must satisfy 0 <= parents[i] < i");
    const int V = HPE_NUM_VERTS;
    c->h_vt.assign(m->v_template, m->v_template + V * 3);
    c->h_sd.assign(m->shapedirs, m->shapedirs + (size_t)V * 3 * 10);
    c->h_pd.assign(m->posedirs, m->posedirs + (size_t)V * 3 * 207);
    c->h_jreg.assign(m->J_regressor, m->J_regressor + (size_t)24 * V);
    c->h_w.assign(m->weights, m->weights + (size_t)V * 24);
    c->h_kreg.assign(m->kp_regressor, m->kp_regressor + (size_t)m->num_kp * V);
    c->h_par.assign(m->parents, m->parents + 24);
    c->num_kp = m->num_kp;
    c->smpl_loaded = true;
    return HPE_OK;
}

int hpe_load_conv(hpe_ctx* c, int idx, const float* kernel, const float* bias, const float* gamma, const float* beta,
                  const float* mean, const float* var) {
    if (!c || idx < 0 || idx >= HPE_NUM_CONV) return fail(HPE_ERR_INVALID, "bad conv index");
    if (c->finalized) return fail(HPE_ERR_STATE, "already finalized");
    if (!kernel || !bias || !gamma || !beta || !mean || !var) return fail(HPE_ERR_INVALID, "null conv array");
    const ConvSpec& s = specs()[idx];
    ConvLayer& L = c->conv[idx];
    L.kernel.assign(kernel, kernel + (size_t)s.kh * s.kw * s.cin * s.cout);
    L.bias.assign(bias, bias + s.cout);
    L.gamma.assign(gamma, gamma + s.cout);
    L.beta.assign(beta, beta + s.cout);
    L.mean.assign(mean, mean + s.cout);
    L.var.assign(var, var + s.cout);
    L.loaded = true;
    return HPE_OK;
}

int hpe_load_dense(hpe_ctx* c, int idx, const float* kernel, const float* bias) {
    if (!c || idx < 0 || idx >= HPE_NUM_DENSE) return fail(HPE_ERR_INVALID, "bad dense index");
    if (c->finalized) return fail(HPE_ERR_STATE, "already finalized");
    if (!kernel || !bias) return fail(HPE_ERR_INVALID, "null dense array");
    const int din[3] = {2133, 1024, 1024}, dout[3] = {1024, 1024, 85};
    c->dense[idx].kernel.assign(kernel, kernel + (size_t)din[idx] * dout[idx]);
    c->dense[idx].bias.assign(bias, bias + dout[idx]);
    c->dense[idx].loaded = true;
    return HPE_OK;
}

int hpe_load_mean_theta(hpe_ctx* c, const float* mean85) {
    if (!c || !mean85) return fail(HPE_ERR_INVALID, "null argument");
    if (c->finalized) return fail(HPE_ERR_STATE, "already finalized");
    memcpy(c->h_mean, mean85, sizeof(float) * HPE_THETA_DIM);
    c->mean_loaded = true;
    return HPE_OK;
}

}
#pragma GCC visibility pop

void release_device_state(hpe_ctx* c) {
    for (void* p : c->allocs) (void)hipFree(p);
    c->allocs.clear();
    c->rt = RegTrainWork{};
    c->et = EncTrainWork{};
    if (c->critic_buf) {
        (void)hipFree(c->critic_buf);
        c->critic_buf = nullptr;
        c->critic = CriticW{};
        c->have_critic = false;
    }
    if (c->critic_ws) {
        (void)hipFree(c->critic_ws);
        c->critic_ws = nullptr;
        c->critic_ws_floats = 0;
    }
    for (auto& a : c->aux)
        if (a) {
            (void)hipStreamDestroy(a);
            a = nullptr;
        }
    auto kill = [](hipEvent_t& e) {
        if (e) {
            (void)hipEventDestroy(e);
            e = nullptr;
        }
    };
    kill(c->ev_fork);
    kill(c->ev_enc);
    kill(c->ev_tail);
    for (auto& e : c->ev_feat_free) kill(e);
    if (c->tail_st) {
        (void)hipStreamDestroy(c->tail_st);
        c->tail_st = nullptr;
    }
    for (auto& e : c->ev_join) kill(e);
    for (auto& e : c->ev) kill(e);
    for (auto& e : c->span0) kill(e);
    for (auto& e : c->span1) kill(e);
    for (auto& e : c->cev0) kill(e);
    for (auto& e : c->cev1) kill(e);
    for (auto& e : c->lev0) kill(e);
    for (auto& e : c->lev1) kill(e);
    for (auto& e : c->lev_all) kill(e);
    c->ev_ok = false;
}

static int check_loaded(hpe_ctx* c) {
    int nconv = 0, ndense = 0;
    for (int i = 0; i < HPE_NUM_CONV; ++i) nconv += c->conv[i].loaded ? 1 : 0;
    for (int i = 0; i < HPE_NUM_DENSE; ++i) ndense += c->dense[i].loaded ? 1 : 0;
    if (nconv != 0 && nconv != HPE_NUM_CONV) {
        for (int i = 0; i < HPE_NUM_CONV; ++i)
            if (!c->conv[i].loaded) return fail(HPE_ERR_STATE, std::string("conv layer not loaded: ") + specs()[i].name);
    }
    if (ndense != 0 && (ndense != HPE_NUM_DENSE || !c->mean_loaded))
        return fail(HPE_ERR_STATE, "regressor needs all 3 dense layers and the mean theta");
    c->have_encoder = nconv == HPE_NUM_CONV;
    c->have_regressor = ndense == HPE_NUM_DENSE && c->mean_loaded;
    c->have_smpl = c->smpl_loaded;
    if (!c->have_encoder && !c->have_regressor && !c->have_smpl) return fail(HPE_ERR_STATE, "nothing was loaded");
    return HPE_OK;
}

static int pack_dual_weights(hpe_ctx* c) {
    int rc;
    for (const ResBlock& blk : blocks()) {
        const unsigned packs = layer_packs(c->plan, c->bf16, blk.i2c);
        if (!(packs & PACK_W_DUAL)) continue;
        const ConvSpec& s2 = specs()[blk.i2c];
        const ConvSpec& s1 = specs()[blk.i1];
        ConvLayer& L2 = c->conv[blk.i2c];
        const ConvLayer& L1 = c->conv[blk.i1];
        const int K1 = s2.cin, K2 = s1.cin, N = s2.cout;
        const int n_pad = round_up(N, 128), K = K1 + K2;
        std::vector<float> wt((size_t)n_pad * K, 0.f), sh(N);
        for (int n = 0; n < N; ++n) {
            double inv2, inv1, shift2, shift1;
            bn_fold(L2, n, c->cfg.bn_eps, &inv2, &shift2);
            bn_fold(L1, n, c->cfg.bn_eps, &inv1, &shift1);
            for (int k = 0; k < K1; ++k) wt[(size_t)n * K + k] = (float)(inv2 * (double)L2.kernel[(size_t)k * N + n]);
            for (int k = 0; k < K2; ++k) wt[(size_t)n * K + K1 + k] = (float)(inv1 * (double)L1.kernel[(size_t)k * N + n]);
            sh[n] = (float)(shift2 + shift1);
        }
        if (c->bf16) {
            if ((rc = upload_bf16(c, &L2.w_dual, to_bf16(wt)))) return rc;
        } else {
            if ((rc = upload_to(c, &L2.w_dual, wt))) return rc;
            if ((packs & PACK_W_DUAL_SPLIT) && (rc = upload_split(c, &L2.w_dual_split, wt, n_pad, K))) return rc;
        }
        if ((rc = upload_to(c, &L2.shift_dual, sh))) return rc;
        L2.k_dual = K;
        L2.k1_dual = K1;
    }
    return HPE_OK;
}

static int pack_wino_weights(hpe_ctx* c, const ConvSpec& s, ConvLayer& L) {
    int rc;
    std::vector<float> U((size_t)16 * s.cin * s.cout);
    for (int ci = 0; ci < s.cin; ++ci)
        for (int n = 0; n < s.cout; ++n) {
            double g[3][3];
            for (int a = 0; a < 3; ++a)
                for (int b = 0; b < 3; ++b) g[a][b] = L.kernel[(((size_t)a * 3 + b) * s.cin + ci) * s.cout + n];
            const size_t base = wino_u_base(n, ci, s.cin);
            for (int xi = 0; xi < 4; ++xi)
                for (int nu = 0; nu < 4; ++nu) {
                    const double gx[3] = {wino_g(xi, 0), wino_g(xi, 1), wino_g(xi, 2)}, gn[3] = {wino_g(nu, 0), wino_g(nu, 1), wino_g(nu, 2)};
                    U[base + (size_t)(xi * 4 + nu) * 512] = wino_elem(gx, gn, g);
                }
        }
    if (!(c->plan.wino_fused && s.hin >= c->plan.wino_fused_min_hw)) return upload_to(c, &L.wino_u, U);
    const size_t nu = U.size();
    std::vector<unsigned short> Us((size_t)3 * nu);
    for (int ci = 0; ci < s.cin; ++ci)
        for (int n = 0; n < s.cout; ++n)
            for (int e = 0; e < 16; ++e) {
                unsigned short h[3];
                bf16_split3(U[wino_u_base(n, ci, s.cin) + (size_t)e * 512], h);
                for (int j = 0; j < 3; ++j) Us[wino_us_base(n, ci, s.cin) + j * WINO_US_PIECE + (size_t)e * 512] = h[j];
            }
    U.resize(nu + Us.size() / 2);
    memcpy(U.data() + nu, Us.data(), Us.size() * 2);
    if ((rc = upload_to(c, &L.wino_u, U))) return rc;
    L.wino_u_split = wino_u_split_of(L.wino_u, s.cin, s.cout);
    return HPE_OK;
}

static int pack_wino4_weights(hpe_ctx* c, const ConvSpec& s, ConvLayer& L) {
    int rc;
    std::vector<float> U((size_t)36 * s.cin * s.cout);
    for (int ci = 0; ci < s.cin; ++ci)
        for (int n = 0; n < s.cout; ++n) {
            double g[3][3];
            for (int a = 0; a < 3; ++a)
                for (int b = 0; b < 3; ++b) g[a][b] = L.kernel[(((size_t)a * 3 + b) * s.cin + ci) * s.cout + n];
            const size_t base = wino4_u_base(n, ci, s.cin);
            for (int xi = 0; xi < 6; ++xi)
                for (int nu = 0; nu < 6; ++nu) {
                    const double gx[3] = {wino4_g(xi, 0), wino4_g(xi, 1), wino4_g(xi, 2)}, gn[3] = {wino4_g(nu, 0), wino4_g(nu, 1), wino4_g(nu, 2)};
                    U[base + (size_t)(xi * 6 + nu) * 256] = wino_elem(gx, gn, g);
                }
        }
    if ((rc = upload_to(c, &L.wino4_u, U))) return rc;
    return HPE_OK;
}

static int pack_stem_weights(hpe_ctx* c, ConvLayer& L) {
    const size_t ld = 7 * 32;
    std::vector<float> wp(64 * ld, 0.f);
    for (int kh = 0; kh < 7; ++kh)
        for (int kw = 0; kw < 7; ++kw)
            for (int ci = 0; ci < 3; ++ci) {
                const int k = conv_wt_k(0, kh, kw, ci);
                for (int n = 0; n < 64; ++n) wp[n * ld + k] = L.kernel[(((size_t)kh * 7 + kw) * 3 + ci) * 64 + n];
            }
    if (c->bf16) return upload_bf16(c, &L.stem_w, to_bf16(wp));
    std::vector<unsigned short> ws(3 * wp.size());
    for (size_t o = 0; o < wp.size(); ++o) {
        unsigned short h[3];
        bf16_split3(wp[o], h);
        for (int j = 0; j < 3; ++j) ws[j * wp.size() + o] = h[j];
    }
    return upload_bf16(c, &L.stem_w, ws);
}

static int pack_conv_weights(hpe_ctx* c) {
    int rc;
    for (int i = 0; i < HPE_NUM_CONV; ++i) {
        const ConvSpec& s = specs()[i];
        ConvLayer& L = c->conv[i];
        const unsigned packs = layer_packs(c->plan, c->bf16, i);
        L.n_pad = round_up(s.cout, 128);
        L.k_pad = conv_k_pad(i, c->bf16);
        std::vector<float> wt((size_t)L.n_pad * L.k_pad, 0.f);
        for (int kh = 0; kh < s.kh; ++kh)
            for (int kw = 0; kw < s.kw; ++kw)
                for (int ci = 0; ci < s.cin; ++ci) {
                    const int k = conv_wt_k(i, kh, kw, ci);
                    const float* src = &L.kernel[(((size_t)kh * s.kw + kw) * s.cin + ci) * s.cout];
                    for (int n = 0; n < s.cout; ++n) wt[(size_t)n * L.k_pad + k] = src[n];
                }
        if (c->bf16) {
            if ((rc = upload_bf16(c, &L.w, to_bf16(wt)))) return rc;
        } else {
            if ((rc = upload_to(c, &L.w, wt))) return rc;
            if ((packs & PACK_W_SPLIT) && (rc = upload_split(c, &L.w_split, wt, L.n_pad, L.k_pad))) return rc;
            if ((packs & PACK_WINO_U) && (rc = pack_wino_weights(c, s, L))) return rc;
            if ((packs & PACK_WINO4_U) && (rc = pack_wino4_weights(c, s, L))) return rc;
        }
        if ((packs & PACK_STEM_W) && (rc = pack_stem_weights(c, L))) return rc;
        std::vector<float> sc(s.cout), sh(s.cout);
        for (int n = 0; n < s.cout; ++n) {
            double scale, shift;
            bn_fold(L, n, c->cfg.bn_eps, &scale, &shift);
            sc[n] = (float)scale;
            sh[n] = (float)shift;
        }
        if ((rc = upload_to(c, &L.scale, sc))) return rc;
        if ((rc = upload_to(c, &L.shift, sh))) return rc;
        std::vector<float>().swap(L.kernel);
    }
    return HPE_OK;
}

static int pack_regressor(hpe_ctx* c) {
    int rc;
    const struct {
        float** p;
        size_t n;
    } live[] = {
        {&c->w1f, (size_t)1024 * 2048},
        {&c->w1t, (size_t)1024 * THETA_LD},
        {&c->w2, (size_t)1024 * 1024},
        {&c->w3, (size_t)128 * 1024},
        {&c->b1, 1024},
        {&c->b2, 1024},
        {&c->b3, 128},
        {&c->mean_dev, HPE_THETA_DIM},
        {&c->rt.w1k, (size_t)(2048 + 128) * 1024},
        {&c->rt.w2k, (size_t)1024 * 1024},
        {&c->rt.w3k, (size_t)1024 * THETA_LD},
    };
    for (const auto& b : live)
        if ((rc = dev_alloc(c, b.p, b.n, true))) return rc;
    std::vector<float> flat((size_t)regressor_param_offset(4, false));
    for (int i = 0; i < HPE_NUM_DENSE; ++i) {
        std::copy(c->dense[i].kernel.begin(), c->dense[i].kernel.end(), flat.begin() + regressor_param_offset(i, false));
        std::copy(c->dense[i].bias.begin(), c->dense[i].bias.end(), flat.begin() + regressor_param_offset(i, true));
    }
    std::copy(c->h_mean, c->h_mean + HPE_THETA_DIM, flat.begin() + regressor_param_offset(3, false));
    float* tmp = nullptr;
    if ((rc = upload(c, &tmp, flat))) return rc;
    HIP_TRY(regressor_params_copy(c, tmp, true, nullptr));
    HIP_TRY(hipDeviceSynchronize());
    c->allocs.pop_back();
    HIP_TRY(hipFree(tmp));
    return HPE_OK;
}

static int pack_smpl(hpe_ctx* c) {
    int rc;
    const int V = HPE_NUM_VERTS, V3 = V * 3;
    std::vector<float> src((size_t)11 * V3);
    memcpy(src.data(), c->h_vt.data(), sizeof(float) * V3);
    for (int i = 0; i < V3; ++i)
        for (int k = 0; k < 10; ++k) src[(size_t)(1 + k) * V3 + i] = c->h_sd[(size_t)i * 10 + k];
    if ((rc = upload(c, &c->smpl_basis_src, src))) return rc;
    c->smpl.v_template = c->smpl_basis_src;
    c->smpl.shapedirs = c->smpl_basis_src + V3;
    std::vector<float> pd((size_t)207 * V3);
    for (int i = 0; i < V3; ++i)
        for (int k = 0; k < 207; ++k) pd[(size_t)k * V3 + i] = c->h_pd[(size_t)i * 207 + k];
    float* p = nullptr;
    if ((rc = upload(c, &p, pd))) return rc;
    c->smpl.posedirs = p;
    if ((rc = upload(c, &p, c->h_w))) return rc;
    c->smpl.weights = p;
    std::vector<float> jr((size_t)V * SMPL_KP_PITCH, 0.f), kr((size_t)V * SMPL_KP_PITCH, 0.f);
    for (int j = 0; j < 24; ++j)
        for (int v = 0; v < V; ++v) jr[(size_t)v * SMPL_KP_PITCH + j] = c->h_jreg[(size_t)j * V + v];
    for (int j = 0; j < c->num_kp; ++j)
        for (int v = 0; v < V; ++v) kr[(size_t)v * SMPL_KP_PITCH + j] = c->h_kreg[(size_t)j * V + v];
    if ((rc = upload(c, &p, jr))) return rc;
    c->smpl.j_reg = p;
    if ((rc = upload(c, &p, kr))) return rc;
    c->smpl.kp_reg = p;
    int depth[24], maxd = 0;
    for (int j = 0; j < 24; ++j) {
        depth[j] = c->h_par[j] < 0 ? 0 : depth[c->h_par[j]] + 1;
        if (depth[j] > maxd) maxd = depth[j];
    }
    void* ip = nullptr;
    HIP_TRY(hipMalloc(&ip, sizeof(int) * 48));
    c->allocs.push_back(ip);
    HIP_TRY(hipMemcpy(ip, c->h_par.data(), sizeof(int) * 24, hipMemcpyHostToDevice));
    HIP_TRY(hipMemcpy(static_cast<int*>(ip) + 24, depth, sizeof(int) * 24, hipMemcpyHostToDevice));
    c->smpl.parents = static_cast<int*>(ip);
    c->smpl.depth = static_cast<int*>(ip) + 24;
    c->smpl.max_depth = maxd;
    c->smpl.num_kp = c->num_kp;
    float* jb = nullptr;
    if ((rc = dev_alloc(c, &jb, 11 * 24 * 3, true))) return rc;
    HIP_TRY(hpe_launch_joint_regress(c->smpl_basis_src, c->smpl.j_reg, 11, 24, jb, nullptr, nullptr, nullptr));
    HIP_TRY(hipDeviceSynchronize());
    c->smpl.j_basis = jb;
    return HPE_OK;
}

static int size_workspaces(hpe_ctx* c) {
    int rc;
    const size_t B = (size_t)c->cfg.max_batch;
    const size_t Bpad = (size_t)round_up(c->cfg.max_batch, SMPL_IMG_TILE);
    if (c->have_encoder) {
        if ((rc = dev_alloc(c, &c->padded, B * STEM_HP * STEM_WP * 4 + 64, true))) return rc;
        if ((rc = dev_alloc(c, &c->X0, B * 802816, false))) return rc;
        if ((rc = dev_alloc(c, &c->X1, B * 802816, false))) return rc;
        if ((rc = dev_alloc(c, &c->SC, B * 802816, false))) return rc;
        if ((rc = dev_alloc(c, &c->T1, B * 200704, false))) return rc;
        if ((rc = dev_alloc(c, &c->T2, B * 200704, false))) return rc;
        if ((rc = dev_alloc(c, &c->feat, B * HPE_FEATURE_DIM, true))) return rc;
        if ((rc = dev_alloc(c, &c->feat_alt, B * HPE_FEATURE_DIM, true))) return rc;
    }
    if (c->have_encoder && !c->bf16 && c->plan.wino_min_c > 0) {
        if ((rc = dev_alloc(c, &c->wino_v, B * WINO_V_PITCH + WINO_V_SLACK, false))) return rc;
        if (c->plan.wino_f4 && c->plan.wino4_ksplit) {
            const size_t nws = hpe_wino4_split_ws_floats();
            if ((rc = dev_alloc(c, &c->w4_split, 4 * nws, false))) return rc;
            for (int k = 0; k < 4; ++k) HIP_TRY(hipMemset(c->w4_split + (k + 1) * nws - 256, 0, 256 * sizeof(unsigned)));
        }
        if (c->plan.wino_streamk) {
            hipDeviceProp_t prop;
            HIP_TRY(hipGetDeviceProperties(&prop, c->cfg.device));
            c->n_cu = prop.multiProcessorCount;
            if ((rc = dev_alloc(c, &c->wino_ws, (size_t)4 * c->n_cu * HPE_WINO_WS_FLOATS, false))) return rc;
            float* fl = nullptr;
            if ((rc = dev_alloc(c, &fl, (size_t)4 * c->n_cu + 4, true))) return rc;
            c->wino_flags = reinterpret_cast<unsigned*>(fl);
            c->dev_err = c->wino_flags + (size_t)4 * c->n_cu;
        }
    }
    {
        c->partial_floats = (size_t)512 * 128 * 128;
        if ((rc = dev_alloc(c, &c->partial, c->partial_floats, false))) return rc;
        c->partial_tail_floats = (size_t)64 * 128 * 128;
        if ((rc = dev_alloc(c, &c->partial_tail, c->partial_tail_floats, false))) return rc;
    }
    if (c->have_regressor) {
        if ((rc = dev_alloc(c, &c->P1, B * 1024, true))) return rc;
        if ((rc = dev_alloc(c, &c->H1, B * 1024, true))) return rc;
        if ((rc = dev_alloc(c, &c->H2, B * 1024, true))) return rc;
        if ((rc = dev_alloc(c, &c->thA, B * THETA_LD, true))) return rc;
        if ((rc = dev_alloc(c, &c->thB, B * THETA_LD, true))) return rc;
        const size_t S = (size_t)c->cfg.num_stage;
        RegTrainWork& t = c->rt;
        if ((rc = dev_alloc(c, &t.p1, B * 1024, true))) return rc;
        if ((rc = dev_alloc(c, &t.a1, S * B * 1024, true))) return rc;
        if ((rc = dev_alloc(c, &t.a2, S * B * 1024, true))) return rc;
        if ((rc = dev_alloc(c, &t.th, (S + 1) * B * THETA_LD, true))) return rc;
        if ((rc = dev_alloc(c, &t.g, (S + 1) * B * THETA_LD, true))) return rc;
// ... 80 lines not shown
```

human-pose-estimation_amd/csrc/hpe_internal.h:

```cpp
#pragma once
#include <hip/hip_runtime.h>
#include <stddef.h>

#include "../../include/hpe.h"

typedef float f32x4 __attribute__((ext_vector_type(4)));
typedef float f32x16 __attribute__((ext_vector_type(16)));

template <typename Id>
__device__ __forceinline__ int xcd_remap(Id bid, int total) {
    const int xcd = bid & 7;
    const int q = total >> 3, rr = total & 7;
    return (xcd < rr ? xcd * (q + 1) : rr * (q + 1) + (xcd - rr) * q) + (bid >> 3);
}

inline dim3 grid1(long n) { return dim3((unsigned)((n + 255) / 256)); }

enum GemmMode { GEMM_DENSE = 0, GEMM_STRIDED = 1, GEMM_CONV3 = 2, GEMM_STEM = 3, GEMM_DUAL = 4 };
enum GemmTile { TILE_128x128 = 0, TILE_128x64 = 1, TILE_64x64 = 2, TILE_64x128 = 3, TILE_128x128_W8 = 4, TILE_128x64_W8 = 5, TILE_256x128_W8 = 6,
                TILE_P8_256x256 = 7  };

struct GemmArgs {
    const float* x;
    const float* w;
    const float* scale;
    const float* shift;
    const float* res;
    float* y;
    int M, N, K;
    int lda, ldw, ldy, ldres, w_rows;
    int relu;
    int Hi, Wi, Cin, Ho, Wo, stride, cin_slabs;
    int n_mtiles, n_ntiles;
    int split_k;
    float* partial;
    size_t partial_floats;
    const float* zero;
    void* reserved;
    const float* x2;
    int k1_slabs;
    int res_prefetch;
    int y_slab8;
    int w_piece;
};

hipError_t hpe_launch_gemm(GemmArgs p, int mode, int tile, int splitk_min_slabs, hipStream_t st, int* split_k_out = nullptr);
hipError_t hpe_launch_gemm_f32s(GemmArgs p, int mode, int tile, hipStream_t st);

size_t hpe_wino_v_floats(int B, int H, int W, int C);
hipError_t hpe_wino_init_device();
#define HPE_WINO_WS_FLOATS 65536
struct WinoStreamK {
    float* ws;
    unsigned* flags;
    unsigned epoch;
    int n_wg;
    unsigned* err;
};
hipError_t hpe_launch_wino_conv3(const float* x, int lda, const float* U, const float* scale, const float* shift, float* y, int ldy,
                                 int B, int H, int W, int C, int N, int relu, float* V, const WinoStreamK* sk, hipStream_t st);

hipError_t hpe_launch_wino_fused_conv3(const float* xs, const unsigned short* Us, const float* scale, const float* shift, const float* zero16, float* y,
                                       int ldy, int B, int H, int W, int C, int N, int relu, hipStream_t st);
int hpe_wino_fused_items(int B, int H, int W, int N);
hipError_t hpe_launch_nhwc_to_slab8(const float* x, float* xs, long M, int C, hipStream_t st);

size_t hpe_wino4_v_floats(int B, int H, int W, int C);
int hpe_wino4_items(int B, int H, int W, int N);
hipError_t hpe_wino4_init_device();
hipError_t hpe_launch_wino4_conv3(const float* x, int lda, const float* U, const float* scale, const float* shift, float* y, int ldy, int B,
                                  int H, int W, int C, int N, int relu, float* V, hipStream_t st, int co_running, float* split_ws, int n32_below, int abl);
size_t hpe_wino4_split_ws_floats();

hipError_t hpe_launch_wino4_fused_conv3(const float* xs, const float* U, const float* scale, const float* shift, const float* zero16, float* y,
                                        int ldy, int B, int H, int W, int C, int N, int relu, hipStream_t st);
int hpe_wino4_fused_items(int B, int H, int W, int N);

hipError_t hpe_launch_gemm_bf16(GemmArgs p, int mode, int tile, hipStream_t st);
hipError_t hpe_launch_gemm_bf16_p8(GemmArgs p, int mode, hipStream_t st, int* split_k_out = nullptr);
struct ChainArgs {
    const __bf16* t2;
    const __bf16* res;
    const __bf16* x2;
    const __bf16* w2c;
    const __bf16* w2a;
    const float *scaleA, *shiftA;
    const float *scaleB, *shiftB;
    __bf16* t3;
    __bf16* u1;
    int M, ldw2c, ldw2a;
};
struct Halo3Args {
    const __bf16* x;
    const __bf16* w;
    const float* scale;
    const float* shift;
    __bf16* y;
    int M, N, ldw, relu;
    int n_ntiles;
    int two;
};
bool hpe_halo3_bf16_supported(int HW, int Cin, int N);
hipError_t hpe_launch_halo3_bf16(const Halo3Args& p, int HW, int Cin, hipStream_t st);

bool hpe_chain_bf16_supported(int C, int C4, int CP, int C2);
hipError_t hpe_launch_chain_bf16(const ChainArgs& p, int C, int C4, int CP, int C2, hipStream_t st);
hipError_t hpe_chain_bf16_occupancy(int out[3]);
struct ChainArgsF32 {
    const float *t2, *res, *w2c, *w2a, *scaleA, *shiftA, *scaleB, *shiftB;
    float *t3, *u1;
    int M, ldw2c, ldw2a, u1_slab8;
};
bool hpe_chain_f32_supported(int C, int C4, int CP);
hipError_t hpe_launch_chain_f32(const ChainArgsF32& p, int C, int C4, int CP, hipStream_t st);
hipError_t hpe_chain_f32_occupancy(int* out);
hipError_t hpe_launch_f32_to_bf16(const float* x, void* y, long n, hipStream_t st);
hipError_t hpe_launch_bf16_to_f32(const void* x, float* y, long n, hipStream_t st);
hipError_t hpe_launch_pad_input_bf16(const float* img, void* out, int B, int H, int W, int Hp, int Wp, hipStream_t st);
hipError_t hpe_launch_maxpool_bf16(const void* x, void* y, int B, int H, int C, hipStream_t st);
hipError_t hpe_launch_avgpool_bf16(const void* x, float* y, int B, int HW, int C, int ldy, hipStream_t st);

hipError_t hpe_launch_stem_fused(const float* img, const void* w, const float* scale, const float* shift, void* y, int B, int R, int bf16,
                                 hipStream_t st);
hipError_t hpe_stem_fused_init_device();
int hpe_stem_fused_pick_rows(int B);

hipError_t hpe_launch_pad_input(const float* img, float* out, int B, int H, int W, int Hp, int Wp, hipStream_t st);
hipError_t hpe_launch_maxpool(const float* x, float* y, int B, int H, int C, hipStream_t st);
hipError_t hpe_launch_avgpool(const float* x, float* y, int B, int HW, int C, int ldy, hipStream_t st);
hipError_t hpe_launch_dense_gemv(const float* x, int lda, int M, int K, const float* wt, int N, const float* scale, const float* shift, const float* res,
                                 int ldres, int relu, float* y, int ldy, hipStream_t st);
hipError_t hpe_launch_tile_theta(const float* mean85, float* theta, int B, int ld, hipStream_t st);
hipError_t hpe_launch_copy_theta(const float* src, int lds, float* dst, int ldd, int B, int n, hipStream_t st);

struct SmplDev {
    const float* v_template;
    const float* shapedirs;
    const float* posedirs;
    const float* weights;
    const float* kp_reg;
    const float* j_reg;
    const float* j_basis;
    const int* parents;
    const int* depth;
    int num_kp;
    int max_depth;
};
#define SMPL_V 6890
#define SMPL_KP_PITCH 24
#define SMPL_IMG_TILE 8
#define SMPL_SMALL_B 8

struct SmplWork {
    float* pfT;
    float* betaT;
    float* A;
    float* cams;
    float* verts_tmp;
    float* kp_part;
    int Bpad;
};

struct HpeOutputs;
hipError_t hpe_launch_smpl(const SmplDev& d, const SmplWork& w, const float* theta, int ldtheta, int B, const HpeOutputs* o,
                           hipStream_t st);
hipError_t hpe_launch_joint_regress(const float* X, const float* reg, int n, int K, float* out, const float* cams,
                                    float* kp2d, hipStream_t st);
hipError_t hpe_launch_orth_proj(const float* X, const float* cam, int B, int P, float sx, float sy, int pixels, float* out,
                                hipStream_t st);

#define SMPL_BWD_PART 512
struct SmplBwdWork {
    float* pfT;
    float* betaT;
    float* A;
    float* cams;
    float* rjg;
    float* gj;
    float* part;
    int Bpad;
};
size_t hpe_smpl_bwd_part_floats(int Bpad);
hipError_t hpe_launch_smpl_backward(const SmplDev& d, const SmplBwdWork& w, const float* theta, int B, const HpeOutputs* g,
                                    float* grad_theta, hipStream_t st);

#define CRITIC_ROWS 4
struct CriticLayerSpec {
    const char* name;
    int in, out;
};
const CriticLayerSpec* hpe_critic_layers();
struct CriticW {
    const float* w[HPE_NUM_CRITIC_DENSE];
    const float* wt[HPE_NUM_CRITIC_DENSE];
    const float* b[HPE_NUM_CRITIC_DENSE];
};
size_t hpe_critic_live_floats();
CriticW hpe_critic_live_view(const float* buf);
hipError_t hpe_launch_critic(const CriticW& w, const float* joints, int K, const float* betas, int betas_stride, const float* Rs, long N,
                             float* scores, float* kcs, hipStream_t st);
// ... 69 lines not shown
```

human-pose-estimation_amd/csrc/hpe_plan.h:

```cpp
#pragma once
#include "../../include/hpe.h"
#include "hpe_internal.h"

struct HpePlan {
    int n_streams = 2;
    int dual_gemm = 1;
    int stem_fused = 1;
    int wino_min_c = 128;
    int wino_min_items = 128;
    int wino_fused = 1;
    int wino_fused_min_hw = 28;
    int mesh_a2b = 0;
    int wino_f4 = 7;
    int wino4_fused = 0;
    int bf16_p8 = 0;
    int wino4_ksplit = 1;
    int chain_fuse = 0;
    int halo3 = 0;
    int f32_split = 0;
    int chunk_images = 0;
    int min_chunk = 32;
    int halo3_two = 4;
    int f32s_min_tiles = 128;
    int wino_streamk = 0;
    int concurrent_tiles = 0;
    int bf16_w8_min_tiles = 128;
    int wide128_min_tiles = 384;
    int force_wide = -1;
    int splitk_min_slabs = 4;
    int wino4_min_items = 64;
    int wino4_n32 = 256;
    int w4_abl = 0;
};

constexpr int PLAN_BF16_128_MIN_TILES = 192;
constexpr int PLAN_BF16_P8_MIN_N = 256;
constexpr int PLAN_BF16_P8_MIN_K = 512;
constexpr int PLAN_EXPAND_SMALL_GRID = 128;
constexpr int PLAN_SHORTK_TILE = TILE_128x64_W8;
constexpr int PLAN_F32S_TILE = TILE_128x128;
constexpr int PLAN_F32S_EXPAND_TILE = TILE_128x128_W8;
constexpr int PLAN_F32S_EXPAND_MIN_K = 256;

HpePlan hpe_resolve_plan(const HpeConfig& cfg);

inline int stage_bit(int hout) { return hout >= 56 ? 1 : (hout >= 28 ? 2 : (hout >= 14 ? 4 : 8)); }
inline int f4_bit(int hin) { return hin <= 7 ? 1 : (hin <= 14 ? 2 : (hin <= 28 ? 4 : 8)); }

constexpr unsigned PACK_W_SPLIT = 1u << HPE_PACK_W_SPLIT, PACK_WINO_U = 1u << HPE_PACK_WINO_U, PACK_WINO4_U = 1u << HPE_PACK_WINO4_U,
                   PACK_STEM_W = 1u << HPE_PACK_STEM_W, PACK_W_DUAL = 1u << HPE_PACK_W_DUAL, PACK_W_DUAL_SPLIT = 1u << HPE_PACK_W_DUAL_SPLIT;
unsigned layer_packs(const HpePlan& pl, bool bf16, int idx);

enum ConvKernel { CONV_K_F32 = 0, CONV_K_F32S, CONV_K_BF16, CONV_K_BF16_P8, CONV_K_HALO3, CONV_K_WINO, CONV_K_WINO_FUSED, CONV_K_WINO4, CONV_K_WINO4_FUSED };
struct ConvQuery { int B; bool concurrent, residual, workspace; };
struct ConvRoute {
    int kernel, mode, tile;
    bool in_slab8;
    bool out_slab8;
    bool concurrent;
};
enum BlockJoin { JOIN_SEPARATE = 0, JOIN_DUAL, JOIN_CHAIN };
struct BlockRoute {
    ConvRoute r2a, r2b, r2c, r1;
    int join;
    bool u1_slab8;
};
struct ResBlock;
ConvRoute route_conv(const HpePlan& pl, bool bf16, int idx, const ConvQuery& q);
BlockRoute route_block(const HpePlan& pl, bool bf16, const ResBlock& blk, ConvQuery q);
int pick_tile(const HpePlan& pl, int M, int N, int K, bool residual_expand = false, bool concurrent = false);
```

human-pose-estimation_amd/csrc/hpe_plan.hip:

```cpp
#include <hip/hip_runtime.h>

#include <climits>
#include <cmath>
#include <cstdint>
#include <cstdio>
#include <cstdlib>
#include <cstring>
#include <string>
#include <vector>

#include "gemm_contract.h"
#include "hpe_ctx.h"

namespace {

struct Network {
    std::vector<ConvSpec> specs;
    std::vector<ResBlock> blocks;
};

Network build_network() {
    Network net;
    std::vector<ConvSpec>& v = net.specs;
    auto add = [&](const std::string& n, const std::string& b, int kh, int cin, int cout, int s, int hin, int hout) {
        ConvSpec c;
        snprintf(c.name, sizeof c.name, "%s", n.c_str());
        snprintf(c.bn, sizeof c.bn, "%s", b.c_str());
        c.kh = c.kw = kh;
        c.cin = cin;
        c.cout = cout;
        c.stride = s;
        c.hin = hin;
        c.hout = hout;
        v.push_back(c);
    };
    add("conv1", "bn_conv1", 7, 3, 64, 2, 224, 112);
    const int nblk[4] = {3, 4, 6, 3};
    const int filt[4][3] = {{64, 64, 256}, {128, 128, 512}, {256, 256, 1024}, {512, 512, 2048}};
    int cin = 64, h = 56;
    int in = -1;
    for (int st = 0; st < 4; ++st) {
        for (int b = 0; b < nblk[st]; ++b) {
            const bool first = b == 0;
            const int s = (first && st > 0) ? 2 : 1;
            const int hout = h / s;
            const int i2a = (int)v.size();
            net.blocks.push_back(ResBlock{st, first, b == nblk[st] - 1, i2a, i2a + 1, i2a + 2, first ? i2a + 3 : -1, in});
            in = i2a + 2;
            char base[24], bn[24];
            snprintf(base, sizeof base, "res%d%c_branch", st + 2, 'a' + b);
            snprintf(bn, sizeof bn, "bn%d%c_branch", st + 2, 'a' + b);
            add(std::string(base) + "2a", std::string(bn) + "2a", 1, cin, filt[st][0], s, h, hout);
            add(std::string(base) + "2b", std::string(bn) + "2b", 3, filt[st][0], filt[st][1], 1, hout, hout);
            add(std::string(base) + "2c", std::string(bn) + "2c", 1, filt[st][1], filt[st][2], 1, hout, hout);
            if (first) add(std::string(base) + "1", std::string(bn) + "1", 1, cin, filt[st][2], s, h, hout);
            cin = filt[st][2];
            h = hout;
        }
    }
    return net;
}

const Network& network() {
    static const Network n = build_network();
    return n;
}

}

const std::vector<ConvSpec>& specs() { return network().specs; }
const std::vector<ResBlock>& blocks() { return network().blocks; }

struct PlanOption {
    int HpePlan::*member;
    int HpeConfig::*cfg;
    const char* env;
    int dflt[2];
    int mask[2];
    int lo, hi;
};

constexpr int ANY = -1, NO_LO = INT_MIN, NO_HI = INT_MAX;

const PlanOption kPlanOptions[] = {
    {&HpePlan::n_streams, &HpeConfig::n_streams, "HPE_STREAMS", {2, 2}, {ANY, ANY}, 1, 4},
    {&HpePlan::dual_gemm, &HpeConfig::dual_gemm, "HPE_DUAL", {1, 1}, {ANY, ANY}, NO_LO, NO_HI},
    {&HpePlan::stem_fused, &HpeConfig::stem_fused, "HPE_STEM_FUSED", {1, 1}, {ANY, ANY}, NO_LO, NO_HI},
    {&HpePlan::wino_min_c, &HpeConfig::wino_min_c, "HPE_WINO_MINC", {128, 128}, {ANY, ANY}, NO_LO, NO_HI},
    {&HpePlan::wino_min_items, &HpeConfig::wino_min_items, "HPE_WINO_MIN_ITEMS", {128, 128}, {ANY, ANY}, NO_LO, NO_HI},
    {&HpePlan::wino_fused, &HpeConfig::wino_fused, "HPE_WINO_FUSED", {1, 1}, {ANY, ANY}, NO_LO, NO_HI},
    {&HpePlan::wino_fused_min_hw, &HpeConfig::wino_fused_min_hw, "HPE_WINO_FUSED_MINHW", {28, 28}, {ANY, ANY}, NO_LO, NO_HI},
    {&HpePlan::mesh_a2b, &HpeConfig::mesh_a2b, "HPE_MESH_A2B", {0, 0}, {ANY, ANY}, NO_LO, NO_HI},
    {&HpePlan::wino_f4, &HpeConfig::wino_f4, "HPE_WINO_F4", {7, 7}, {ANY, ANY}, NO_LO, NO_HI},
    {&HpePlan::wino4_fused, &HpeConfig::wino4_fused, "HPE_WINO4_FUSED", {0, 0}, {12, 12}, NO_LO, NO_HI},
    {&HpePlan::bf16_p8, &HpeConfig::bf16_p8, "HPE_BF16_P8", {0, 0}, {ANY, ANY}, NO_LO, NO_HI},
    {&HpePlan::wino4_ksplit, &HpeConfig::wino4_ksplit, "HPE_WINO4_KSPLIT", {1, 1}, {ANY, ANY}, NO_LO, NO_HI},
    {&HpePlan::chain_fuse, &HpeConfig::chain_fuse, "HPE_CHAIN", {8, 7}, {8, 23}, NO_LO, NO_HI},
    {&HpePlan::halo3, &HpeConfig::halo3, "HPE_HALO3", {15, 15}, {0, 15}, NO_LO, NO_HI},
    {&HpePlan::f32_split, &HpeConfig::f32_split, "HPE_F32_SPLIT", {14, 14}, {15, 0}, NO_LO, NO_HI},
    {&HpePlan::chunk_images, nullptr, "HPE_CHUNK", {0, 0}, {ANY, ANY}, NO_LO, NO_HI},
    {&HpePlan::min_chunk, nullptr, "HPE_MIN_CHUNK", {32, 24}, {ANY, ANY}, NO_LO, NO_HI},
    {&HpePlan::halo3_two, nullptr, "HPE_HALO3_TWO", {4, 4}, {7, 7}, NO_LO, NO_HI},
    {&HpePlan::f32s_min_tiles, nullptr, "HPE_F32S_MIN_TILES", {128, 128}, {ANY, ANY}, NO_LO, NO_HI},
    {&HpePlan::wino_streamk, nullptr, "HPE_WINO_STREAMK", {0, 0}, {ANY, ANY}, NO_LO, NO_HI},
    {&HpePlan::concurrent_tiles, nullptr, "HPE_CONCURRENT_TILES", {0, 0}, {ANY, ANY}, NO_LO, NO_HI},
    {&HpePlan::bf16_w8_min_tiles, nullptr, "HPE_BF16_W8_MIN_TILES", {128, 128}, {ANY, ANY}, NO_LO, NO_HI},
    {&HpePlan::wide128_min_tiles, nullptr, "HPE_WIDE128_MIN_TILES", {384, 384}, {ANY, ANY}, NO_LO, NO_HI},
    {&HpePlan::force_wide, nullptr, "HPE_TILE_WIDE", {-1, -1}, {ANY, ANY}, NO_LO, NO_HI},
    {&HpePlan::splitk_min_slabs, nullptr, "HPE_SPLITK_SLABS", {4, 4}, {ANY, ANY}, 2, NO_HI},
    {&HpePlan::wino4_min_items, nullptr, "HPE_WINO4_MIN_ITEMS", {64, 64}, {ANY, ANY}, NO_LO, NO_HI},
    {&HpePlan::wino4_n32, nullptr, "HPE_WINO4_N32", {256, 256}, {ANY, ANY}, NO_LO, NO_HI},
    {&HpePlan::w4_abl, nullptr, "HPE_W4_ABL", {0, 0}, {ANY, ANY}, NO_LO, NO_HI},
};

HpePlan hpe_resolve_plan(const HpeConfig& cfg) {
    const int dt = cfg.encoder_dtype == 1 ? 1 : 0;
    HpePlan pl;
    for (const PlanOption& o : kPlanOptions) {
        int v = o.dflt[dt];
        const char* e = getenv(o.env);
        if (o.cfg && cfg.*o.cfg >= 0) v = cfg.*o.cfg;
        else if (e && o.member == &HpePlan::mesh_a2b) v = e[0] == 'v' ? 1 : (e[0] == 'm' ? 2 : 0);
        else if (e) v = atoi(e);
        v &= o.mask[dt];
        pl.*o.member = v < o.lo ? o.lo : (v > o.hi ? o.hi : v);
    }
    if (pl.min_chunk < 8) pl.min_chunk = dt ? 24 : 32;
    pl.wino_fused = pl.wino_fused && pl.wino_min_c > 0;
    if (pl.wino_min_c <= 0) pl.wino_f4 = pl.wino4_fused = 0;
    return pl;
}

static int pick_f32s(const HpePlan& pl, bool split_packed, int M, int N, int K, bool residual_expand) {
    if (!split_packed || N <= 64) return -1;
    if (residual_expand && K < PLAN_F32S_EXPAND_MIN_K) return -1;
    const int tile = residual_expand ? PLAN_F32S_EXPAND_TILE : PLAN_F32S_TILE;
    const TileShape ts = tile_shape(GEMM_K_F32S, tile);
    return (long)((M + ts.bm - 1) / ts.bm) * ((N + ts.bn - 1) / ts.bn) >= pl.f32s_min_tiles ? tile : -1;
}

int pick_tile(const HpePlan& pl, int M, int N, int K, bool residual_expand, bool concurrent) {
    const bool wide = N > 64;
    if (wide && residual_expand) return (long)((M + 127) / 128) * ((N + 63) / 64) < PLAN_EXPAND_SMALL_GRID ? TILE_64x64 : TILE_128x64_W8;
    if (wide && pl.force_wide >= 0) return pl.force_wide;
    if (!wide) return TILE_128x64;
    if (K <= 128 && M >= 150000) return PLAN_SHORTK_TILE;
    if ((concurrent || pl.concurrent_tiles) && pl.wide128_min_tiles > 0 && (long)((M + 127) / 128) * ((N + 127) / 128) >= pl.wide128_min_tiles) return TILE_128x128;
    if (M >= 150000) return TILE_64x128;
    return TILE_64x64;
}

static int pick_bf16(const HpePlan& pl, int M, int N, int K, bool residual_expand, bool concurrent, int mode) {
    if (pl.bf16_p8 && N >= PLAN_BF16_P8_MIN_N && N % 256 == 0 && K >= PLAN_BF16_P8_MIN_K && !residual_expand) {
        const int bit = mode == GEMM_CONV3 ? (N == 256 ? 1 : 2) : (mode == GEMM_DUAL ? (N >= 2048 ? 8 : 16) : 4);
        if (pl.bf16_p8 & bit) return TILE_P8_256x256;
    }
    if (N <= 64) return TILE_128x64;
    const long t128 = (long)((M + 127) / 128) * ((N + 127) / 128);
    int tile = t128 >= ((concurrent || pl.concurrent_tiles) ? PLAN_BF16_128_MIN_TILES : 512) ? TILE_128x128 : TILE_64x128;
    if (residual_expand) tile = TILE_128x64_W8;
    else if (M <= 16384 && M >= 8192 && K >= 1024 && N >= 256) tile = TILE_256x128_W8;
    if (pl.bf16_w8_min_tiles > 0 && t128 >= pl.bf16_w8_min_tiles) tile = TILE_128x128_W8;
    return tile;
}

unsigned layer_packs(const HpePlan& pl, bool bf16, int idx) {
    const ConvSpec& s = specs()[idx];
    unsigned m = idx == 0 ? PACK_STEM_W : 0;
    const int slab = bf16 ? 64 : 32;
    const ResBlock* blk = nullptr;
    for (const ResBlock& b : blocks())
        if (b.first && b.i2c == idx) blk = &b;
    if (pl.dual_gemm && blk && s.cin % slab == 0 && specs()[blk->i1].cin % slab == 0) {
        m |= PACK_W_DUAL;
        if (!bf16 && (pl.f32_split & stage_bit(s.hout))) m |= PACK_W_DUAL_SPLIT;
    }
    if (bf16) return m;
    if (idx != 0 && s.kh == 1 && (pl.f32_split & stage_bit(s.hout))) m |= PACK_W_SPLIT;
    const bool wino = s.kh == 3 && s.stride == 1 && s.cin % 32 == 0 && s.cout % 64 == 0;
    if (wino && pl.wino_min_c > 0 && (s.cin >= pl.wino_min_c || (pl.wino_fused && s.hin >= pl.wino_fused_min_hw))) m |= PACK_WINO_U;
    if (wino && ((pl.wino_f4 | pl.wino4_fused) & f4_bit(s.hin))) m |= PACK_WINO4_U;
    return m;
}

static ConvRoute route_gemm(const HpePlan& pl, bool bf16, int mode, int M, int N, int K, bool expand, bool split_packed, bool concurrent) {
    ConvRoute r{CONV_K_F32, mode, -1, false, false, concurrent};
    if (bf16) {
        r.tile = pick_bf16(pl, M, N, K, expand, concurrent, mode);
        r.kernel = r.tile == TILE_P8_256x256 ? CONV_K_BF16_P8 : CONV_K_BF16;
    } else if ((r.tile = pick_f32s(pl, split_packed, M, N, K, expand)) >= 0) {
        r.kernel = CONV_K_F32S;
    } else {
        r.tile = pick_tile(pl, M, N, K, expand, concurrent);
    }
    return r;
}

ConvRoute route_conv(const HpePlan& pl, bool bf16, int idx, const ConvQuery& q) {
    const ConvSpec& s = specs()[idx];
    const unsigned packs = layer_packs(pl, bf16, idx);
    const int B = q.B, H = s.hin;
    const int mode = idx == 0 ? GEMM_STEM : s.kh == 3 ? GEMM_CONV3 : s.stride == 1 ? GEMM_DENSE : GEMM_STRIDED;
    const bool plain3 = mode == GEMM_CONV3 && s.stride == 1 && !q.residual;
    auto special = [&](int kernel) { return ConvRoute{kernel, mode, -1, kernel == CONV_K_WINO_FUSED || kernel == CONV_K_WINO4_FUSED, false, q.concurrent}; };
    const int min4 = pl.wino_min_items < pl.wino4_min_items ? pl.wino_min_items : pl.wino4_min_items;
    if (plain3 && (packs & PACK_WINO4_U) && (pl.wino4_fused & f4_bit(H)) && hpe_wino4_fused_items(B, H, H, s.cout) >= min4) return special(CONV_K_WINO4_FUSED);
    const bool f4 = plain3 && (packs & PACK_WINO4_U) && (pl.wino_f4 & f4_bit(H)) && hpe_wino4_items(B, H, H, s.cout) >= min4;
    if (plain3 && !f4 && pl.wino_fused && (packs & PACK_WINO_U) && H >= pl.wino_fused_min_hw && hpe_wino_fused_items(B, H, H, s.cout) >= pl.wino_min_items)
        return special(CONV_K_WINO_FUSED);
    if (f4 && q.workspace) return special(CONV_K_WINO4);
    if (plain3 && (packs & PACK_WINO_U) && q.workspace && s.cin >= pl.wino_min_c &&
        (long)((B * ((H + 1) / 2) * ((H + 1) / 2) + 63) / 64) * (s.cout / 64) >= pl.wino_min_items)
        return special(CONV_K_WINO);
    if (bf16 && plain3 && (pl.halo3 & f4_bit(H)) && hpe_halo3_bf16_supported(H, s.cin, s.cout)) return special(CONV_K_HALO3);
    return route_gemm(pl, bf16, mode, B * s.hout * s.hout, s.cout, conv_k_pad(idx, bf16), mode == GEMM_DENSE && q.residual && s.cout == 4 * s.cin,
                      (packs & PACK_W_SPLIT) != 0, q.concurrent);
}

static bool use_chain(const HpePlan& pl, bool bf16, const ResBlock& blk) {
    if (blk.last) return false;
    const int stg = blk.stage, i2c = blk.i2c;
    const ConvSpec& s2 = specs()[i2c];
    const ConvSpec& sn = specs()[i2c + (blk.first ? 2 : 1)];
    if (sn.kh != 1 || sn.stride != 1 || sn.cin != s2.cout) return false;
    if (!bf16) return !blk.first && stg == 0 && (pl.chain_fuse & 8) && hpe_chain_f32_supported(s2.cin, s2.cout, sn.cout);
    if (blk.first) {
        const ConvSpec& s1 = specs()[blk.i1];
        return stg == 0 && (pl.chain_fuse & 4) && (layer_packs(pl, bf16, i2c) & PACK_W_DUAL) && s1.stride == 1 && s1.hin == s2.hin &&
               hpe_chain_bf16_supported(s2.cin, s2.cout, sn.cout, s1.cin);
    }
    const int bit = stg == 0 ? 1 : stg == 1 ? 2 : stg == 2 ? 16 : 0;
    return (pl.chain_fuse & bit) && hpe_chain_bf16_supported(s2.cin, s2.cout, sn.cout, 0);
}

BlockRoute route_block(const HpePlan& pl, bool bf16, const ResBlock& blk, ConvQuery q) {
    BlockRoute b{};
    q.residual = false;
    b.r2a = route_conv(pl, bf16, blk.i2a, q);
    b.r2b = route_conv(pl, bf16, blk.i2b, q);
    b.r2a.out_slab8 = b.r2b.in_slab8;
    const ConvSpec& s2 = specs()[blk.i2c];
    if (use_chain(pl, bf16, blk)) {
        b.join = JOIN_CHAIN;
        b.u1_slab8 = route_conv(pl, bf16, blk.i2c + (blk.first ? 3 : 2), q).in_slab8;
    } else if (blk.first && (layer_packs(pl, bf16, blk.i2c) & PACK_W_DUAL)) {
        b.join = JOIN_DUAL;
        b.r2c = route_gemm(pl, bf16, GEMM_DUAL, q.B * s2.hout * s2.hout, s2.cout, s2.cin + specs()[blk.i1].cin, false,
                           (layer_packs(pl, bf16, blk.i2c) & PACK_W_DUAL_SPLIT) != 0, q.concurrent);
    } else {
        if (blk.first) b.r1 = route_conv(pl, bf16, blk.i1, q);
        q.residual = true;
        b.r2c = route_conv(pl, bf16, blk.i2c, q);
    }
    return b;
}
```

human-pose-estimation_amd/engine.py:

```python
from __future__ import annotations

import ctypes as C

import numpy as np

from . import _lib
from .critic_spec import PARAM_FLOATS
from .regressor_spec import PARAM_FLOATS as REGRESSOR_PARAM_FLOATS
from .resnet_spec import CONV_SPECS, ENCODER_PARAM_FLOATS, ENCODER_STAT_FLOATS

NUM_VERTS = _lib.NUM_VERTS


def _torch():
    import torch

    return torch


def _require_cuda_tensor(t, name, shape_tail=None):
    torch = _torch()
    if not isinstance(t, torch.Tensor):
        raise TypeError("%s must be a torch.Tensor on the GPU" % name)
    if not t.is_cuda:
# ... 671 lines not shown
        return dx, gl

    def encoder_params(self):
        out = self._new(ENCODER_PARAM_FLOATS)
        _lib.check(self.lib.hpe_encoder_get_params(self._h, out.data_ptr(), self._stream()))
        return out

    def set_encoder_params(self, flat):
        torch = _torch()
        if isinstance(flat, torch.Tensor):
            flat = flat.detach().to("cpu", torch.float32).numpy()
        arr, ptr = _lib.f32(np.asarray(flat).reshape(-1))
        if arr.shape != (ENCODER_PARAM_FLOATS,):
            raise ValueError("flat must be [%d], got %s" % (ENCODER_PARAM_FLOATS, arr.shape))
        _lib.check(self.lib.hpe_encoder_set_params(self._h, ptr))

    def set_encoder_params_dev(self, flat):
        flat = _require_cuda_tensor(flat.detach(), "flat")
        if tuple(flat.shape) != (ENCODER_PARAM_FLOATS,):
            raise ValueError("flat must be [%d], got %s" % (ENCODER_PARAM_FLOATS, tuple(flat.shape)))
        _lib.check(self.lib.hpe_encoder_set_params_dev(self._h, flat.data_ptr(), self._stream()))

    def encoder_packing(self, idx, which):
        torch = _torch()
        if isinstance(which, str):
            which = _lib.ENCODER_PACKINGS.index(which)
        n = self.lib.hpe_debug_encoder_packing_bytes(self._h, int(idx), int(which))
        if n == 0:
            return None
        out = torch.empty(n, dtype=torch.uint8, device=self.tdev)
        _lib.check(self.lib.hpe_debug_encoder_packing(self._h, int(idx), int(which), out.data_ptr(), self._stream()))
        return out

    def encoder_forward_train(self, images, bn="frozen"):
        fn = self.lib.hpe_encoder_forward_batchnorm if self._bn_mode(bn) else self.lib.hpe_encoder_forward_train
        images = _require_cuda_tensor(images.detach(), "images", (224, 224, 3))
        B = images.shape[0]
        out = self._new(B, 2048)
        self._check_hooked(fn(self._h, images.data_ptr(), B, out.data_ptr(), self._stream()))
        return out

    def encoder_backward(self, images, grad_features, bn="frozen"):
        fn = self.lib.hpe_encoder_backward_batchnorm if self._bn_mode(bn) else self.lib.hpe_encoder_backward
        images = _require_cuda_tensor(images.detach(), "images", (224, 224, 3))
        B = images.shape[0]
        grad_features = _require_cuda_tensor(grad_features.detach(), "grad_features")
        if tuple(grad_features.shape) != (B, 2048):
            raise ValueError("grad_features must be [%d,2048], got %s" % (B, tuple(grad_features.shape)))
        g = self._new(ENCODER_PARAM_FLOATS)
        self._check_hooked(fn(self._h, images.data_ptr(), B, grad_features.data_ptr(), g.data_ptr(), self._stream()))
        return g

    def debug_conv_backward(self, idx, x, y, dy, want_dx=True):
        s = CONV_SPECS[idx]
        x, dy = _require_cuda_tensor(x, "x"), _require_cuda_tensor(dy, "dy")
        y = _require_cuda_tensor(y, "y") if y is not None else None
        B = x.shape[0]
        want_dx = want_dx and idx != 0
        dx = self._new(B, s.hin, s.hin, s.cin) if want_dx else None
        gl = self._new(s.kh * s.kw * s.cin * s.cout + 3 * s.cout)
        _lib.check(self.lib.hpe_debug_conv_backward(self._h, idx, x.data_ptr(), y.data_ptr() if y is not None else None, dy.data_ptr(), B,
                                                    dx.data_ptr() if want_dx else None, gl.data_ptr(), self._stream()))
        return dx, gl

    def debug_maxpool_backward(self, x, dy):
        x, dy = _require_cuda_tensor(x, "x"), _require_cuda_tensor(dy, "dy")
        dx = self._new(*x.shape)
        _lib.check(self.lib.hpe_debug_maxpool_backward(x.data_ptr(), dy.data_ptr(), x.shape[0], x.shape[1], x.shape[3], dx.data_ptr(), self._stream()))
        return dx

    def debug_avgpool_backward(self, dy, HW):
        dy = _require_cuda_tensor(dy, "dy")
        dx = self._new(dy.shape[0], HW, dy.shape[1])
        _lib.check(self.lib.hpe_debug_avgpool_backward(dy.data_ptr(), dy.shape[0], HW, dy.shape[1], dx.data_ptr(), self._stream()))
        return dx

    def encoder_stash(self, idx):
        B = self.lib.hpe_debug_encoder_stash_batch(self._h)
        if B < 1:
            raise _lib.HpeError("encoder_stash: no training forward has run")
        s = CONV_SPECS[idx] if idx >= 0 else None
        out = self._new(B, s.hout, s.hout, s.cout) if s else self._new(B, 56, 56, 64)
        _lib.check(self.lib.hpe_debug_encoder_stash(self._h, idx, out.data_ptr(), self._stream()))
        return out

    def mesh_loss(self, seg, verts2d):
        torch = _torch()
        seg = _require_cuda_tensor(seg, "seg")
        verts2d = _require_cuda_tensor(verts2d, "verts2d")
        B, H, W = seg.shape[0], seg.shape[1], seg.shape[2]
        P = verts2d.shape[1]
        out = torch.zeros(4, dtype=torch.float32, device=self.tdev)
        _lib.check(self.lib.hpe_mesh_loss(self._h, seg.data_ptr(), verts2d.data_ptr(), B, H, W, P, out.data_ptr(), self._stream()))
        return out[0]

    def mesh_loss_grad(self, seg, verts2d, want_neighbours=False):
        torch = _torch()
        seg = _require_cuda_tensor(seg, "seg")
        verts2d = _require_cuda_tensor(verts2d, "verts2d")
        if seg.dim() != 3 or verts2d.dim() != 3 or verts2d.shape[2] != 2 or verts2d.shape[0] != seg.shape[0]:
            raise ValueError("seg must be [B,H,W] and verts2d [B,P,2], got %s and %s" % (tuple(seg.shape), tuple(verts2d.shape)))
        B, H, W = seg.shape[0], seg.shape[1], seg.shape[2]
        P = verts2d.shape[1]
        out = torch.zeros(4, dtype=torch.float32, device=self.tdev)
        grad = torch.empty((B, P, 2), dtype=torch.float32, device=self.tdev)
        nn_pix = nn_vert = None
        if want_neighbours:
            nn_pix = torch.empty((B, H, W), dtype=torch.int32, device=self.tdev)
            nn_vert = torch.empty((B, P), dtype=torch.int32, device=self.tdev)
        _lib.check(self.lib.hpe_mesh_loss_grad(self._h, seg.data_ptr(), verts2d.data_ptr(), B, H, W, P, out.data_ptr(), grad.data_ptr(),
                                               nn_pix.data_ptr() if want_neighbours else None,
                                               nn_vert.data_ptr() if want_neighbours else None, self._stream()))
        return (out[0], grad, nn_pix, nn_vert) if want_neighbours else (out[0], grad)

    def val_losses(self, kp_gt, kp2d_stages, seg=None, verts2d_stages=None, out=None):
        torch = _torch()
        kp_gt = _require_cuda_tensor(kp_gt, "kp_gt")
        n = len(kp2d_stages)
        kp2d = [_require_cuda_tensor(t, "kp2d") for t in kp2d_stages]
        B, K = kp_gt.shape[0], kp_gt.shape[1]
        kp_ptrs = (C.c_void_p * n)(*[t.data_ptr() for t in kp2d])
        H = W = P = 0
        seg_ptr, v_ptrs, keep = None, None, None
        if seg is not None and verts2d_stages is not None:
            seg = _require_cuda_tensor(seg, "seg")
            keep = [_require_cuda_tensor(t, "verts2d") for t in verts2d_stages]
            if len(keep) != n or seg.shape[0] != B:
                raise ValueError("one verts2d tensor per stage and one silhouette per image are needed")
            H, W, P = seg.shape[1], seg.shape[2], keep[0].shape[1]
            seg_ptr = seg.data_ptr()
            v_ptrs = (C.c_void_p * n)(*[t.data_ptr() for t in keep])
        if out is None:
            out = torch.empty((n, 4), dtype=torch.float32, device=self.tdev)
        _lib.check(self.lib.hpe_val_losses(self._h, seg_ptr, kp_gt.data_ptr(), kp_ptrs, v_ptrs, n, B, K, H, W, P, out.data_ptr(), self._stream()))
        return out

    def check_device(self):
        _lib.check(self.lib.hpe_device_status(self._h, self._stream()))

    def debug_conv(self, idx, x, residual=None, relu=True):
        s = CONV_SPECS[idx]
        x = _require_cuda_tensor(x, "x")
        B = x.shape[0]
        y = self._new(B, s.hout, s.hout, s.cout)
        r = None
        if residual is not None:
            r = _require_cuda_tensor(residual, "residual").data_ptr()
        _lib.check(self.lib.hpe_debug_conv(self._h, idx, x.data_ptr(), B, r, int(relu), y.data_ptr(), self._stream()))
        return y

    def conv_route(self, idx, B, concurrent=False, residual=False, workspace=True):
        return _lib.conv_route(self.lib, self._cfg, idx, B, concurrent, residual, workspace)

    def _debug_gemm(self, call, what, mode, tile, x, wt, y, M, N, K, kw):
        g = _lib.HpeDebugGemm()
        g.struct_size = C.sizeof(_lib.HpeDebugGemm)
        fields = dict(lda=K, ldw=K, ldy=N, ldres=N, mode=mode, tile=tile, x=x, wt=wt, y=y, M=M, N=N, K=K)
        fields.update(kw)
        for k, v in fields.items():
            if k in ("x", "x2", "wt", "residual", "scale", "shift", "y"):
                v = v.data_ptr() if hasattr(v, "data_ptr") else v
            elif k in ("struct_size", "split_k") or not hasattr(g, k):
                raise TypeError("%s: unknown argument %r" % (what, k))
            setattr(g, k, v)
        sk = C.c_int(-1)
        g.split_k = C.pointer(sk)
        _lib.check(call(g))
        return sk.value

    def debug_gemm_ex(self, mode, tile, x, wt, y, M, N, K, **kw):
        return self._debug_gemm(lambda g: self.lib.hpe_debug_gemm_ex(self._h, C.byref(g), self._stream()), "debug_gemm_ex", mode, tile, x, wt, y, M, N, K, kw)

    def debug_gemm_launch(self, kernel, mode, tile, x, wt, y, M, N, K, w_piece=0, **kw):
        return self._debug_gemm(lambda g: self.lib.hpe_debug_gemm_launch(self._h, C.byref(g), int(kernel), int(w_piece), self._stream()),
                                "debug_gemm_launch", mode, tile, x, wt, y, M, N, K, kw)

    def debug_chain(self, idx2c, t2, residual):
        s = CONV_SPECS[idx2c]
        first = CONV_SPECS[idx2c + 1].name.endswith("branch1")
        sn = CONV_SPECS[idx2c + (2 if first else 1)]
        t2 = _require_cuda_tensor(t2, "t2", (s.hin, s.hin, s.cin))
        residual = _require_cuda_tensor(residual, "residual", (s.hout, s.hout, CONV_SPECS[idx2c + 1].cin if first else s.cout))
        B = t2.shape[0]
        t3 = self._new(B, s.hout, s.hout, s.cout)
        u1 = self._new(B, sn.hout, sn.hout, sn.cout)
        occ = (C.c_int * 3)()
        _lib.check(self.lib.hpe_debug_chain(self._h, idx2c, t2.data_ptr(), residual.data_ptr(), B, t3.data_ptr(), u1.data_ptr(), occ, self._stream()))
        return t3, u1, (occ[0], occ[1], occ[2])

    def debug_stem(self, images, rows_per_strip=0):
        images = _require_cuda_tensor(images, "images", (224, 224, 3))
        y = self._new(images.shape[0], 56, 56, 64)
        _lib.check(self.lib.hpe_debug_stem(self._h, images.data_ptr(), images.shape[0], int(rows_per_strip), y.data_ptr(), self._stream()))
        return y

    def joint_regress(self, X, use_kp_regressor=True):
        X = _require_cuda_tensor(X, "X", (NUM_VERTS, 3))
        K = self.num_kp if use_kp_regressor else 24
        out = self._new(X.shape[0], K, 3)
        _lib.check(self.lib.hpe_debug_joint_regress(self._h, X.data_ptr(), X.shape[0], int(use_kp_regressor), out.data_ptr(), self._stream()))
        return out

    def encoder_kernel_description(self):
        if self.encoder_dtype == "fp32":
            return ("conv_gemm_f32s_dma_kernel (the 1x1 / strided / dual-source layers of stages 3-5 on the bf16 matrix cores, operands split "
                    "exactly into three bf16 pieces) + conv_gemm_f32_dma_kernel (the other 1x1 layers) + w4_input_kernel + w4_gemm_kernel / w4_gemm32_kernel "
                    "(the 13 3x3 layers on the 28x28 / 14x14 / 7x7 maps as fp32 Winograd F(4x4,3x3); F(2x2,3x3) / direct below 64 work "
                    "items) + wino_fused_split_kernel (the three 56x56 3x3 layers, F(2x2,3x3) on the bf16 matrix cores through the same exact split) + stem_fused_f32s_kernel (image and weights split like the 1x1 layers) -- the 53 conv layers of one "
                    "step, priced at their direct-convolution FLOPs")
        return ("conv_gemm_bf16_dma_kernel (1x1 / strided / dual-source layers) + chain_expand_reduce_bf16_kernel (branch2c + next branch2a of "
                "stages 2-3 as one launch) + conv3_halo_bf16_kernel (the sixteen 3x3 layers, tile + halo resident in LDS) + stem_fused_bf16_kernel "
                "-- the 53 conv layers of one step, priced at their algorithmic HBM bytes")

    def enable_timing(self, level=1):
        _lib.check(self.lib.hpe_enable_timing(self._h, int(level)))

    def timings(self):
        ms = (C.c_float * 5)()
        _lib.check(self.lib.hpe_get_timings(self._h, ms))
        return dict(encoder_ms=ms[0], conv_ms=ms[1], regress_smpl_ms=ms[2], total_ms=ms[4])

    def span_stats(self):
        ms = (C.c_float * 3)()
        n = C.c_int()
        _lib.check(self.lib.hpe_get_span_stats(self._h, ms, C.byref(n)))
        return dict(mean_ms=ms[0], min_ms=ms[1], max_ms=ms[2], calls=n.value)

    def set_loss_counter(self, counter=None):
        _lib.check(self.lib.hpe_debug_set_loss_counter(self._h, None if counter is None else counter.data_ptr()))
        self._loss_counter = counter

    def loss_timings(self):
        ms = (C.c_float * 2)()
        _lib.check(self.lib.hpe_get_loss_timings(self._h, ms))
        return dict(val_losses_ms=ms[0], a2b_search_ms=ms[1])

    def conv_timings(self):
        ms = (C.c_float * _lib.NUM_CONV)()
        _lib.check(self.lib.hpe_get_conv_timings(self._h, ms))
        return list(ms)


def _cur_stream(t):
    return C.c_void_p(_torch().cuda.current_stream(t.device).cuda_stream)


def orth_proj(X, camera):
    X = _require_cuda_tensor(X, "X")
    camera = _require_cuda_tensor(camera, "camera").reshape(-1, 3)
    B, P = X.shape[0], X.shape[1]
    out = _torch().empty((B, P, 2), dtype=_torch().float32, device=X.device)
    with _torch().cuda.device(X.device):
        _lib.check(_lib.load().hpe_orth_proj(X.data_ptr(), camera.data_ptr(), B, P, out.data_ptr(), _cur_stream(X)))
    return out


def reproject(verts, cam, im_w, im_h):
    verts = _require_cuda_tensor(verts, "verts")
    cam = _require_cuda_tensor(cam, "cam").reshape(-1, 3)
    B, P = verts.shape[0], verts.shape[1]
    out = _torch().empty((B, P, 2), dtype=_torch().float32, device=verts.device)
    with _torch().cuda.device(verts.device):
        _lib.check(
            _lib.load().hpe_reproject_vertices(verts.data_ptr(), cam.data_ptr(), B, P, float(im_w), float(im_h), out.data_ptr(), _cur_stream(verts))
        )
    return out


def kp_loss_backward(kp_gt, kp_pred, grad_loss=None):
    kp_gt = _require_cuda_tensor(kp_gt, "kp_gt")
    kp_pred = _require_cuda_tensor(kp_pred, "kp_pred")
    B, K = kp_gt.shape[0], kp_gt.shape[1]
    gl = None
    if grad_loss is not None:
        grad_loss = _require_cuda_tensor(grad_loss.reshape(1), "grad_loss")
        gl = grad_loss.data_ptr()
    out = _torch().empty((B, K, 2), dtype=_torch().float32, device=kp_gt.device)
    with _torch().cuda.device(kp_gt.device):
        _lib.check(_lib.load().hpe_kp_loss_backward(kp_gt.data_ptr(), kp_pred.data_ptr(), B, K, gl, out.data_ptr(), _cur_stream(kp_gt)))
    return out


def kp_loss_parts(kp_gt, kp_pred):
    kp_gt = _require_cuda_tensor(kp_gt, "kp_gt")
    kp_pred = _require_cuda_tensor(kp_pred, "kp_pred")
    B, K = kp_gt.shape[0], kp_gt.shape[1]
    out = _torch().zeros(4, dtype=_torch().float32, device=kp_gt.device)
    with _torch().cuda.device(kp_gt.device):
        _lib.check(_lib.load().hpe_kp_loss(kp_gt.data_ptr(), kp_pred.data_ptr(), B, K, out.data_ptr(), _cur_stream(kp_gt)))
    return out[:3]
```

include/hpe.h:

```cpp
#ifndef HPE_H_
#define HPE_H_

#ifdef __cplusplus
extern "C" {
#endif

#define HPE_OK 0
#define HPE_ERR_INVALID 1
#define HPE_ERR_HIP 2
#define HPE_ERR_STATE 3
#define HPE_ERR_NO_DEVICE 4
#define HPE_ERR_REDUCE 5

#define HPE_NUM_CONV 53
#define HPE_NUM_DENSE 3
#define HPE_NUM_CRITIC_DENSE 9
#define HPE_NUM_VERTS 6890
#define HPE_NUM_JOINTS 24
#define HPE_NUM_BETAS 10
#define HPE_NUM_POSE_BASIS 207
#define HPE_THETA_DIM 85
#define HPE_FEATURE_DIM 2048
#define HPE_MAX_KP 24
#define HPE_IMG_SIZE 224
// ... 236 lines not shown
    int hmax, vmax;
    int blocks_w[3], blocks_h[3];
    int idct_group0;
    int store_group0;
    unsigned char quant[3][64];
} HpeJpegImage;

int hpe_jpeg_info(int B, const unsigned char* const* streams, const long long* lengths, HpeJpegInfo* info_out);
int hpe_jpeg_decode(int B, const unsigned char* const* streams, const long long* lengths, const int* channels, int threads,
                    short* coef_out, long long coef_capacity, HpeJpegImage* table_out, int* status_out, long long* totals_out);
int hpe_jpeg_backend(const HpeJpegImage* table_host, const HpeJpegImage* table_dev, int B, const short* coef_dev, long long coef_count,
                     unsigned char* workspace_dev, long long workspace_bytes, unsigned char* frames_dev, long long frames_bytes,
                     void* stream);

#define HPE_JPEG_ENC_HEADER_BYTES 640
#define HPE_JPEG_ENC_BLOCK_BYTES 416
typedef struct HpeJpegEncImage {
    long long frame_offset;
    long long coef_offset[3];
    int H, W;
    int C;
    int hmax, vmax;
    int blocks_w[3], blocks_h[3];
    int real_w[3], real_h[3];
    int group0;
    unsigned char quant[2][64];
} HpeJpegEncImage;

int hpe_jpeg_encode_layout(int B, const int* shapes, const long long* frame_offsets, int hmax, int vmax, int quality,
                           HpeJpegEncImage* table_out, long long* totals_out);
int hpe_jpeg_forward(const HpeJpegEncImage* table_host, const HpeJpegEncImage* table_dev, int B, const unsigned char* frames_dev,
                     long long frames_bytes, short* coef_dev, long long coef_count, void* stream);
int hpe_jpeg_entropy_encode(const HpeJpegEncImage* table, int B, const short* coef, long long coef_count, int units, int xdensity,
                            int ydensity, int threads, unsigned char* out, long long out_capacity, long long* offsets_out,
                            long long* lengths_out);

#define HPE_PNG_MAX_SIDE 16384
#define HPE_PNG_STORE_BYTES_PER_GROUP 1024
typedef struct HpePngImage {
    long long raw_offset;
    long long pal_offset;
    long long work_offset;
    long long out_offset;
    int H, W;
    int color_type;
    int depth;
    int channels;
    int rowbytes;
    int bpp;
    int store_group0;
} HpePngImage;

int hpe_png_backend(const HpePngImage* table_host, const HpePngImage* table_dev, int B, const unsigned char* raw_dev, long long raw_bytes,
                    unsigned char* workspace_dev, long long workspace_bytes, unsigned char* frames_dev, long long frames_bytes,
                    void* stream);

typedef struct HpePngFilterImage {
    long long frame_offset;
    long long scan_offset;
    int H, W;
    int C;
    int row0;
} HpePngFilterImage;

int hpe_png_filter(const HpePngFilterImage* table_host, const HpePngFilterImage* table_dev, int B, const unsigned char* frames_dev,
                   long long frames_bytes, unsigned char* scan_dev, long long scan_bytes, void* stream);

#define HPE_DRAW_JOINTS 19
#define HPE_DRAW_MAX_RADIUS 256
int hpe_draw_panels(const float* images, const float* kp_gt, const float* kp_pred, const unsigned char* rend_img,
                    const unsigned char* rend_seg, const int* skeleton, int n, int T, int S, unsigned char* out, void* stream);
int hpe_draw_skeleton(unsigned char* images, const float* joints, const unsigned char* vis, const int* skeleton, int n, int H, int W,
                      int draw_edges, int radius, void* stream);

typedef struct hpe_renderer hpe_renderer;

typedef struct HpeRenderParams {
    int struct_size;
    int color_id;
    int do_alpha;
    int rot_axis;
    float rot_deg;
    float near;
    float far;
} HpeRenderParams;

void hpe_render_params_init(HpeRenderParams* p);
int hpe_renderer_create(int device, const int* faces_host, int Fn, int P, int max_batch, hpe_renderer** out);
int hpe_renderer_destroy(hpe_renderer* r);
int hpe_render(hpe_renderer* r, const float* verts_dev, const float* cam_dev, int B, int H, int W, const unsigned char* bg_dev,
               const HpeRenderParams* p, unsigned char* out_dev, void* stream);

int hpe_debug_render_ids(hpe_renderer* r, const float* verts_dev, const float* cam_dev, int B, int H, int W, const HpeRenderParams* p,
                         int* face_dev, float* z_dev, void* stream);
int hpe_debug_render_vertices(hpe_renderer* r, const float* verts_dev, const float* cam_dev, int B, int H, int W, const HpeRenderParams* p,
                              void* rec_dev, void* stream);

int hpe_debug_conv(hpe_ctx* ctx, int idx, const float* x_dev, int B, const float* residual_dev, int relu, float* y_dev,
                   void* stream);
int hpe_debug_chain(hpe_ctx* ctx, int idx2c, const float* t2_dev, const float* residual_dev, int B, float* t3_dev, float* u1_dev,
                    int* occupancy, void* stream);
int hpe_debug_stem(hpe_ctx* ctx, const float* images_dev, int B, int rows_per_strip, float* y_dev, void* stream);
#define HPE_GEMM_DENSE 0
#define HPE_GEMM_STRIDED 1
#define HPE_GEMM_CONV3 2
#define HPE_GEMM_DUAL 4
typedef struct HpeDebugGemm {
    int struct_size;
    int mode;
    int tile;
    int M, N, K;
    int lda, ldw, ldy, ldres, w_rows;
    int relu;
    int Hi, Wi, Cin, Ho, Wo, stride;
    int k1_slabs;
    int y_slab8;
    int use_splitk;
    int reserved;
    const float* x;
    const float* x2;
    const float* wt;
    const float* residual;
    const float* scale;
    const float* shift;
    float* y;
    int* split_k;
} HpeDebugGemm;
int hpe_debug_gemm_ex(hpe_ctx* ctx, const HpeDebugGemm* g, void* stream);
int hpe_debug_gemm_check(const HpeDebugGemm* g, int kernel, int w_piece);
int hpe_debug_gemm_launch(hpe_ctx* ctx, const HpeDebugGemm* g, int kernel, int w_piece, void* stream);
enum {
    HPE_CONV_K_F32 = 0,
    HPE_CONV_K_F32S,
    HPE_CONV_K_BF16,
    HPE_CONV_K_BF16_P8,
    HPE_CONV_K_HALO3,
    HPE_CONV_K_WINO,
    HPE_CONV_K_WINO_FUSED,
    HPE_CONV_K_WINO4,
    HPE_CONV_K_WINO4_FUSED,
    HPE_CONV_K_COUNT
};
typedef struct HpeConvRoute {
    int struct_size;
    int kernel;
    int mode;
    int tile;
    int in_slab8, out_slab8;
    int join, join_kernel, join_tile, next_slab8;
    unsigned packs;
    int reserved;
} HpeConvRoute;
int hpe_debug_conv_route(const HpeConfig* cfg, int idx, int B, int concurrent, int residual, int workspace, HpeConvRoute* out);
int hpe_debug_gemm(hpe_ctx* ctx, const float* x_dev, const float* wt_dev, int M, int N, int K, int w_rows, int tile,
                   const float* residual_dev, int relu, float* y_dev, void* stream);
int hpe_debug_maxpool(const float* x_dev, int B, int H, int C, float* y_dev, void* stream);
int hpe_debug_avgpool(const float* x_dev, int B, int HW, int C, float* y_dev, void* stream);
int hpe_debug_joint_regress(hpe_ctx* ctx, const float* X_dev, int n, int use_kp_regressor, float* out_dev, void* stream);
int hpe_enable_timing(hpe_ctx* ctx, int level);
int hpe_device_status(hpe_ctx* ctx, void* stream);
int hpe_get_timings(hpe_ctx* ctx, float ms[5]);
int hpe_get_span_stats(hpe_ctx* ctx, float ms[3], int* n_calls);
int hpe_get_loss_timings(hpe_ctx* ctx, float ms[2]);
int hpe_debug_set_loss_counter(hpe_ctx* ctx, void* counter_dev);
int hpe_get_conv_timings(hpe_ctx* ctx, float* ms53);

#ifdef __cplusplus
}
#endif
#endif
```

Before: 22160 images/sec.

## Add persistent weight-stationary streaming kernel for f32 1x1 expand and dual convs

Adds a persistent kernel for fp32 1x1 expand convolutions (K=64/128, N multiple of 128) and for dual-source branch2c+shortcut launches. It keeps the bf16-split weights in registers per wave and walks M-tiles with double-buffered LDS DMA of the activations. It also prefetches the residual and converts activations to three bf16 planes in LDS for split-precision MFMA. The aim is to avoid re-reading weights per tile and to overlap activation loads with compute on the large-M early stages. The tradeoff is limited occupancy and fixed grid sizing based on CU count, and this path now runs by default for layers with M at least 25088.

```diff
diff --git a/human-pose-estimation_amd/_lib.py b/human-pose-estimation_amd/_lib.py
--- a/human-pose-estimation_amd/_lib.py
+++ b/human-pose-estimation_amd/_lib.py
@@ -285,6 +285,8 @@
     "hpe_debug_gemm_check": (C.c_int, [C.POINTER(HpeDebugGemm), C.c_int, C.c_int]),
     "hpe_debug_gemm_launch": (C.c_int, [C.c_void_p, C.POINTER(HpeDebugGemm), C.c_int, C.c_int, C.c_void_p]),
     "hpe_debug_conv_route": (C.c_int, [C.POINTER(HpeConfig), C.c_int, C.c_int, C.c_int, C.c_int, C.c_int, C.POINTER(HpeConvRoute)]),
+    "hpe_debug_conv_stream1x1": (C.c_int, [C.POINTER(HpeConfig), C.c_int, C.c_int, C.c_int, C.c_int]),
+    "hpe_debug_dual": (C.c_int, [C.c_void_p, C.c_int, C.c_void_p, C.c_void_p, C.c_int, C.c_void_p, C.c_void_p]),
     "hpe_debug_maxpool": (C.c_int, [C.c_void_p, C.c_int, C.c_int, C.c_int, C.c_void_p, C.c_void_p]),
     "hpe_debug_avgpool": (C.c_int, [C.c_void_p, C.c_int, C.c_int, C.c_int, C.c_void_p, C.c_void_p]),
     "hpe_debug_joint_regress": (C.c_int, [C.c_void_p, C.c_void_p, C.c_int, C.c_int, C.c_void_p, C.c_void_p]),
diff --git a/human-pose-estimation_amd/build.py b/human-pose-estimation_amd/build.py
--- a/human-pose-estimation_amd/build.py
+++ b/human-pose-estimation_amd/build.py
@@ -9,7 +9,7 @@
 CSRC = os.path.join(HERE, "csrc")
 LIBDIR = os.path.join(HERE, "lib")
 LIB = os.path.join(LIBDIR, "libhpe_hip.so")
-SOURCES = ["conv_gemm.hip", "conv_gemm_f32s.hip", "conv_gemm_bf16.hip", "conv_gemm_bf16_p8.hip", "conv_chain_bf16.hip", "conv_chain_f32.hip", "conv3_halo_bf16.hip", "conv_wino.hip", "conv_wino4.hip", "stem_fused.hip", "encoder_ops.hip", "smpl.hip", "losses.hip", "prepost.hip", "render.hip", "hpe_plan.hip", "hpe_finalize.hip", "hpe_encoder.hip", "hpe_api.hip", "hpe_render_api.hip", "smpl_bwd.hip", "critic.hip", "critic_train.hip", "regressor_train.hip", "augment.hip", "encoder_train.hip", "encoder_grad.hip", "encoder_repack.hip", "encoder_bn.hip", "jpeg_entropy.hip", "jpeg_decode.hip", "jpeg_huffman_enc.hip", "jpeg_encode.hip", "png_decode.hip", "png_encode.hip", "draw.hip", "adam.hip"]
+SOURCES = ["conv_gemm.hip", "conv_gemm_f32s.hip", "conv_stream_f32s.hip", "conv_gemm_bf16.hip", "conv_gemm_bf16_p8.hip", "conv_chain_bf16.hip", "conv_chain_f32.hip", "conv3_halo_bf16.hip", "conv_wino.hip", "conv_wino4.hip", "stem_fused.hip", "encoder_ops.hip", "smpl.hip", "losses.hip", "prepost.hip", "render.hip", "hpe_plan.hip", "hpe_finalize.hip", "hpe_encoder.hip", "hpe_api.hip", "hpe_render_api.hip", "smpl_bwd.hip", "critic.hip", "critic_train.hip", "regressor_train.hip", "augment.hip", "encoder_train.hip", "encoder_grad.hip", "encoder_repack.hip", "encoder_bn.hip", "jpeg_entropy.hip", "jpeg_decode.hip", "jpeg_huffman_enc.hip", "jpeg_encode.hip", "png_decode.hip", "png_encode.hip", "draw.hip", "adam.hip"]
 CFLAGS = ["--offload-arch=gfx950", "-O3", "-std=c++17", "-fPIC", "-fvisibility=hidden", "-fno-fast-math"]
 
 
diff --git a/human-pose-estimation_amd/csrc/conv_gemm_common.h b/human-pose-estimation_amd/csrc/conv_gemm_common.h
--- a/human-pose-estimation_amd/csrc/conv_gemm_common.h
+++ b/human-pose-estimation_amd/csrc/conv_gemm_common.h
@@ -99,9 +99,10 @@
 #else
 #define HPE_RES_LOAD(ptr) (*(ptr))
 #endif
-template <int BM, int BN, int WM, int WN, int NP>
+template <int BM, int BN, int WM, int WN, bool STREAM = false, int NP>
 __device__ __forceinline__ void conv_epilogue(const GemmArgs& p, float* lds, f32x16 (&acc)[BM / WM / 32][BN / WN / 32], int m0, int n0, int t,
-                                              int lane, int wm, int wn, const f32x4 (&rpre)[NP], bool use_pre) {
+                                              int lane, int wm, int wn, const f32x4 (&rpre)[NP], bool use_pre, float sc0 = 0.f, float sh0 = 0.f) {
+    static_assert(!STREAM || BN / WN == 32, "STREAM: one column per lane");
     constexpr int MT = BM / WM / 32;
     constexpr int NT = BN / WN / 32;
     constexpr int NTHR = 64 * WM * WN;
@@ -114,8 +115,8 @@
             const int cl = (wn * NT + j) * 32 + col_l;
             const int n = n0 + cl;
             const bool n_ok = n < p.N;
-            const float sc = n_ok ? p.scale[n] : 0.f;
-            const float sh = n_ok ? p.shift[n] : 0.f;
+            const float sc = STREAM ? sc0 : n_ok ? p.scale[n] : 0.f;
+            const float sh = STREAM ? sh0 : n_ok ? p.shift[n] : 0.f;
 #pragma unroll
             for (int i = 0; i < MT; ++i) {
                 const int rl = (wm * MT + i) * 32 + row_l;
@@ -124,7 +125,8 @@
             }
         }
     }
-    __syncthreads();
+    if constexpr (STREAM) asm volatile("s_waitcnt lgkmcnt(0)\n\ts_barrier" ::: "memory");
+    else __syncthreads();
     {
         constexpr int TPR = BN / 4;
         constexpr int RPP = NTHR / TPR;
diff --git a/human-pose-estimation_amd/csrc/conv_stream_f32s.hip b/human-pose-estimation_amd/csrc/conv_stream_f32s.hip
--- /dev/null
+++ b/human-pose-estimation_amd/csrc/conv_stream_f32s.hip
@@ -0,0 +1,187 @@
+#include <hip/hip_runtime.h>
+#include <stdint.h>
+
+#include "bf16_split.h"
+#include "conv_gemm_common.h"
+#include "gemm_contract.h"
+#include "hpe_internal.h"
+#include "lds_dma.h"
+
+namespace {
+
+constexpr int SBM = 32, SBN = 128, SNW = 4;
+
+template <int K, bool DUAL>
+__global__ __launch_bounds__(64 * SNW, 2) void conv_stream_f32s_kernel(GemmArgs p, int walkers) {
+    constexpr bool RES = !DUAL;
+    constexpr int NRES = RES ? SBM / (64 * SNW / (SBN / 4)) : 0;
+    constexpr int KS = K / 16;
+    constexpr int CH = K / 8;
+    constexpr int RAW_BYTES = SBM * K * 4;
+    constexpr int PLANE_BYTES = SBM * K * 2;
+    constexpr int EP_BYTES = SBM * (SBN + 4) * 4;
+    constexpr int WORK_BYTES = 3 * PLANE_BYTES > EP_BYTES ? 3 * PLANE_BYTES : EP_BYTES;
+    constexpr int AP = RAW_BYTES / 1024 / SNW;
+    constexpr int UN = SBM * CH / (64 * SNW);
+    constexpr int NPASS = SBM / (64 * SNW / (SBN / 4));
+    static_assert(K == 64 || K == 128, "K = 64 or 128");
+    static_assert(!DUAL || K == 128, "dual: two sources of 64");
+    static_assert(AP >= 1 && UN >= 1 && NPASS == 4, "tile geometry");
+
+    __shared__ __attribute__((aligned(16))) float lds[WORK_BYTES / 4];
+    __shared__ __attribute__((aligned(16))) float raw_lds[2 * RAW_BYTES / 4];
+    char* const work = reinterpret_cast<char*>(lds);
+    char* const raw = reinterpret_cast<char*>(raw_lds);
+
+    const int bid = blockIdx.x;
+    const int j = bid >> 3;
+    const int slice = j % p.n_ntiles;
+    const int walker = (j / p.n_ntiles) * 8 + (bid & 7);
+    if (walker >= walkers || walker >= p.n_mtiles) return;
+    const int n0 = slice * SBN;
+    const int cnt = (p.n_mtiles - walker + walkers - 1) / walkers;
+
+    const int t = threadIdx.x;
+    const int lane = t & 63;
+    const int wave = __builtin_amdgcn_readfirstlane(t >> 6);
+    const int hi = lane >> 5;
+
+    bf16x8 wreg[KS][3];
+    {
+        const __bf16* wsrc = reinterpret_cast<const __bf16*>(p.w) + (size_t)(n0 + 32 * wave + (lane & 31)) * p.ldw + 8 * hi;
+#pragma unroll
+        for (int q = 0; q < KS; ++q)
+#pragma unroll
+            for (int pc = 0; pc < 3; ++pc) wreg[q][pc] = *reinterpret_cast<const bf16x8*>(wsrc + pc * p.w_piece + 16 * q);
+    }
+    const int ncol = n0 + 32 * wave + (lane & 31);
+    const float sc0 = p.scale[ncol], sh0 = p.shift[ncol];
+
+    int dma_row[AP], dma_col[AP];
+#pragma unroll
+    for (int i = 0; i < AP; ++i) {
+        const int s = (SNW * i + wave) * 64 + lane;
+        dma_row[i] = s / (K / 4);
+        dma_col[i] = (s % (K / 4)) * 4;
+    }
+    int sp_src[UN], sp_dst[UN];
+#pragma unroll
+    for (int u = 0; u < UN; ++u) {
+        const int un = t + 64 * SNW * u;
+        const int r = un / CH, c = un % CH;
+        sp_src[u] = r * (K * 4) + c * 32;
+        sp_dst[u] = r * (K * 2) + ((c ^ ((r / (16 / CH)) & (CH - 1))) << 4);
+    }
+    const int a_row = (lane & 31) * (K * 2);
+    const int a_x = ((lane & 31) / (16 / CH)) & (CH - 1);
+    const int r_row = t >> 5;
+    const float* const res_col = RES ? p.res + n0 + (t & 31) * 4 : nullptr;
+
+    auto issue_tile = [&](int m0, int buf, f32x4 (&rnext)[NPASS]) {
+        asm volatile("" ::: "memory");
+#pragma unroll
+        for (int i = 0; i < AP; ++i) {
+            int m = m0 + dma_row[i];
+            m = m < p.M ? m : p.M - 1;
+            const float* src = p.x + ((size_t)m * p.lda + dma_col[i]);
+            if (DUAL && dma_col[i] >= 64) src = p.x2 + ((size_t)m * p.Cin + (dma_col[i] - 64));
+            dma16(src, raw + buf * RAW_BYTES + (SNW * i + wave) * 1024);
+        }
+        asm volatile("" ::: "memory");
+#pragma unroll
+        for (int pass = 0; pass < NRES; ++pass) {
+            int m = m0 + pass * 8 + r_row;
+            m = m < p.M ? m : p.M - 1;
+            rnext[pass] = HPE_RES_LOAD(reinterpret_cast<const f32x4*>(res_col + (size_t)m * p.ldres));
+        }
+        asm volatile("" ::: "memory");
+    };
+
+    auto tile_step = [&](int k, int buf, f32x4 (&rcur)[NPASS], f32x4 (&rnext)[NPASS]) {
+        const int m0 = (walker + k * walkers) * SBM;
+        const int m0n = k + 1 < cnt ? m0 + walkers * SBM : m0;
+        wait_counts<NRES + NPASS>();
+        bare_barrier();
+        const unsigned rb = (unsigned)(uintptr_t)(const __attribute__((address_space(3))) char*)(raw + buf * RAW_BYTES);
+#pragma unroll
+        for (int u = 0; u < UN; ++u) {
+            f32x4 lo, up;
+            asm volatile("ds_read_b128 %0, %2\n\tds_read_b128 %1, %2 offset:16\n\ts_waitcnt lgkmcnt(0)" : "=&v"(lo), "=&v"(up) : "v"(rb + sp_src[u]) : "memory");
+            bf16x8 h0, h1, h2;
+            bf16_split3_cast<8>([&](int e) { return e < 4 ? lo[e] : up[e - 4]; }, h0, h1, h2);
+            *reinterpret_cast<bf16x8*>(work + sp_dst[u]) = h0;
+            *reinterpret_cast<bf16x8*>(work + PLANE_BYTES + sp_dst[u]) = h1;
+            *reinterpret_cast<bf16x8*>(work + 2 * PLANE_BYTES + sp_dst[u]) = h2;
+        }
+        lds_barrier();
+        issue_tile(m0n, buf ^ 1, rnext);
+
+        f32x16 acc[1][1], acx;
+#pragma unroll
+        for (int e = 0; e < 16; ++e) acc[0][0][e] = acx[e] = 0.f;
+#pragma unroll
+        for (int q = 0; q < KS; ++q) {
+            const int off = a_row + (((2 * q + hi) ^ a_x) << 4);
+            const bf16x8 a0 = *reinterpret_cast<const bf16x8*>(work + off);
+            const bf16x8 a1 = *reinterpret_cast<const bf16x8*>(work + PLANE_BYTES + off);
+            const bf16x8 a2 = *reinterpret_cast<const bf16x8*>(work + 2 * PLANE_BYTES + off);
+            acx = __builtin_amdgcn_mfma_f32_32x32x16_bf16(a2, wreg[q][0], acx, 0, 0, 0);
+            acx = __builtin_amdgcn_mfma_f32_32x32x16_bf16(a1, wreg[q][1], acx, 0, 0, 0);
+            acx = __builtin_amdgcn_mfma_f32_32x32x16_bf16(a0, wreg[q][2], acx, 0, 0, 0);
+            acx = __builtin_amdgcn_mfma_f32_32x32x16_bf16(a1, wreg[q][0], acx, 0, 0, 0);
+            acx = __builtin_amdgcn_mfma_f32_32x32x16_bf16(a0, wreg[q][1], acx, 0, 0, 0);
+            acc[0][0] = __builtin_amdgcn_mfma_f32_32x32x16_bf16(a0, wreg[q][0], acc[0][0], 0, 0, 0);
+        }
+        acc[0][0] += acx;
+        wait_counts<AP + NRES, 0>();
+        bare_barrier();
+        conv_epilogue<SBM, SBN, 1, SNW, true>(p, lds, acc, m0, n0, t, lane, 0, wave, rcur, RES, sc0, sh0);
+    };
+
+    f32x4 ra[NPASS], rb[NPASS];
+    issue_tile(walker * SBM, 0, ra);
+    wait_counts<0>();
+    for (int k = 0; k < cnt; k += 2) {
+        tile_step(k, 0, ra, rb);
+        if (k + 1 < cnt) tile_step(k + 1, 1, rb, ra);
+    }
+    wait_counts<0>();
+}
+
+int device_cus() {
+    static int n = 0;
+    if (n == 0) {
+        int dev = 0, v = 0;
+        if (hipGetDevice(&dev) == hipSuccess && hipDeviceGetAttribute(&v, hipDeviceAttributeMultiprocessorCount, dev) == hipSuccess && v > 0) n = v;
+        else n = 256;
+    }
+    return n;
+}
+
+}
+
+bool hpe_stream_f32s_supported(int M, int N, int K) { return M > 0 && (K == 64 || K == 128) && N >= SBN && N % SBN == 0; }
+
+bool hpe_stream_f32s_dual_supported(int M, int N, int K1, int K2, int stride, int Hi, int Ho) {
+    return K1 == 64 && K2 == 64 && stride == 1 && Hi == Ho && hpe_stream_f32s_supported(M, N, K1 + K2);
+}
+
+hipError_t hpe_launch_stream_f32s(GemmArgs p, int mode, int max_walkers, hipStream_t st) {
+    if ((mode != GEMM_DENSE && mode != GEMM_DUAL) || gemm_contract(p, mode, TILE_128x128, GEMM_K_F32S) || !hpe_stream_f32s_supported(p.M, p.N, p.K))
+        return hipErrorInvalidValue;
+    if (mode == GEMM_DENSE ? !p.res : (p.res || !hpe_stream_f32s_dual_supported(p.M, p.N, p.k1_slabs * BK, p.Cin, p.stride, p.Hi, p.Ho) || p.Wi != p.Wo))
+        return hipErrorInvalidValue;
+    p.n_mtiles = (p.M + SBM - 1) / SBM;
+    p.n_ntiles = p.N / SBN;
+    p.split_k = 1;
+    p.res_prefetch = 1;
+    int walkers = 2 * device_cus() / p.n_ntiles;
+    if (max_walkers > 0 && walkers > max_walkers) walkers = max_walkers;
+    if (walkers > p.n_mtiles) walkers = p.n_mtiles;
+    if (walkers < 1) walkers = 1;
+    const int grid = 8 * p.n_ntiles * ((walkers + 7) / 8);
+    if (mode == GEMM_DUAL) hipLaunchKernelGGL((conv_stream_f32s_kernel<128, true>), dim3(grid), dim3(64 * SNW), 0, st, p, walkers);
+    else if (p.K == 64) hipLaunchKernelGGL((conv_stream_f32s_kernel<64, false>), dim3(grid), dim3(64 * SNW), 0, st, p, walkers);
+    else hipLaunchKernelGGL((conv_stream_f32s_kernel<128, false>), dim3(grid), dim3(64 * SNW), 0, st, p, walkers);
+    return hipGetLastError();
+}
diff --git a/human-pose-estimation_amd/csrc/encoder_repack.hip b/human-pose-estimation_amd/csrc/encoder_repack.hip
--- a/human-pose-estimation_amd/csrc/encoder_repack.hip
+++ b/human-pose-estimation_amd/csrc/encoder_repack.hip
@@ -243,7 +243,7 @@
         r.wino_split = L.wino_u_split != nullptr;
         r.wino4_u = L.wino4_u;
         r.dxw = c->et.dxw[i];
-        r.w_split = static_cast<unsigned short*>(L.w_split);
+        r.w_split = L.w_split ? static_cast<unsigned short*>(L.w_split) : L.w_stream;
         r.kh = s.kh;
         r.cin = s.cin;
         r.cout = s.cout;
@@ -275,7 +275,7 @@
             RepackDual& d = t.D[F.n];
             d.w = L2.w_dual;
             d.shift = L2.shift_dual;
-            d.split = static_cast<unsigned short*>(L2.w_dual_split);
+            d.split = L2.w_dual_split ? static_cast<unsigned short*>(L2.w_dual_split) : L2.w_dual_stream;
             d.i2c = blk.i2c;
             d.i1 = blk.i1;
             d.K1 = L2.k1_dual;
diff --git a/human-pose-estimation_amd/csrc/hpe_api.hip b/human-pose-estimation_amd/csrc/hpe_api.hip
--- a/human-pose-estimation_amd/csrc/hpe_api.hip
+++ b/human-pose-estimation_amd/csrc/hpe_api.hip
@@ -800,6 +800,37 @@
     return HPE_OK;
 }
 
+int hpe_debug_conv_stream1x1(const HpeConfig* cfg, int idx, int B, int concurrent, int residual) {
+    if (!cfg || cfg->struct_size != (int)sizeof(HpeConfig) || idx < 0 || idx >= HPE_NUM_CONV || B < 1) {
+        fail(HPE_ERR_INVALID, "hpe_debug_conv_stream1x1: cfg (struct_size), idx in [0, HPE_NUM_CONV) and B >= 1");
+        return -1;
+    }
+    const HpePlan pl = hpe_resolve_plan(*cfg);
+    const bool bf16 = cfg->encoder_dtype == 1;
+    const ConvQuery q{B, concurrent != 0, residual != 0, true};
+    for (const ResBlock& blk : blocks())
+        if (blk.first && blk.i2c == idx) {
+            const BlockRoute b = route_block(pl, bf16, blk, q);
+            return (stream1x1_dual(pl, bf16, blk) ? 2 : 0) | (b.join == JOIN_DUAL && b.r2c.stream ? 1 : 0);
+        }
+    return (stream1x1_layer(pl, bf16, idx) ? 2 : 0) | (route_conv(pl, bf16, idx, q).stream ? 1 : 0);
+}
+
+int hpe_debug_dual(hpe_ctx* c, int idx2c, const float* t2, const float* x, int B, float* y, void* stream) {
+    int rc = check_ready(c, B, NEED_ENC);
+    if (rc) return rc;
+    if (!t2 || !x || !y || c->bf16) return fail(HPE_ERR_INVALID, "hpe_debug_dual: null pointer, or a bf16 context");
+    for (const ResBlock& blk : blocks()) {
+        if (!blk.first || blk.i2c != idx2c) continue;
+        const BlockRoute b = route_block(c->plan, false, blk, ConvQuery{B, false, false, c->wino_v != nullptr});
+        if (b.join != JOIN_DUAL) break;
+        DeviceGuard g(c->cfg.device);
+        HIP_TRY(run_dual(c, blk.i2c, blk.i1, b.r2c, t2, x, B, y, static_cast<hipStream_t>(stream)));
+        return HPE_OK;
+    }
+    return fail(HPE_ERR_INVALID, "hpe_debug_dual: idx2c must be the branch2c of a conv_block that this plan runs as the dual-source launch");
+}
+
 int hpe_debug_gemm(hpe_ctx* c, const float* x, const float* wt, int M, int N, int K, int w_rows, int tile, const float* residual,
                    int relu, float* y, void* stream) {
     if (!c || !c->finalized || !c->have_regressor) return fail(HPE_ERR_STATE, "needs a finalized ctx with the regressor loaded");
diff --git a/human-pose-estimation_amd/csrc/hpe_ctx.h b/human-pose-estimation_amd/csrc/hpe_ctx.h
--- a/human-pose-estimation_amd/csrc/hpe_ctx.h
+++ b/human-pose-estimation_amd/csrc/hpe_ctx.h
@@ -51,6 +51,8 @@
     int k_dual = 0, k1_dual = 0;
     void* w_split = nullptr;
     void* w_dual_split = nullptr;
+    unsigned short* w_stream = nullptr;
+    unsigned short* w_dual_stream = nullptr;
     void* stem_w = nullptr;
     float* wino_u = nullptr;
     unsigned short* wino_u_split = nullptr;
@@ -73,6 +75,7 @@
 __host__ __device__ inline size_t wino_us_base(int n, int ci, int cin) {
     return ((size_t)(n >> 6) * (cin / 8) + (ci >> 3)) * 3 * WINO_US_PIECE + (size_t)(n & 63) * 8 + (ci & 7);
 }
+inline unsigned short* w_stream_of(float* w, int n_pad, int k_pad) { return reinterpret_cast<unsigned short*>(w + (size_t)n_pad * k_pad); }
 __host__ __device__ inline unsigned short* wino_u_split_of(float* wino_u, int cin, int cout) {
     return reinterpret_cast<unsigned short*>(wino_u + (size_t)16 * cin * cout);
 }
@@ -282,6 +285,7 @@
 
 hipError_t run_conv(hpe_ctx* c, int idx, const ConvRoute& r, const float* x, int B, const float* res, int relu, float* y, hipStream_t st,
                     float* wino_v = nullptr, int slot = 0, const float* scale = nullptr, const float* shift = nullptr);
+hipError_t run_dual(hpe_ctx* c, int i2c, int i1, const ConvRoute& r, const float* t2, const float* x, int B, float* y, hipStream_t st);
 hipError_t run_conv_nhwc(hpe_ctx* c, int idx, const float* x, int B, const float* res, int relu, float* y, hipStream_t st,
                          const float* scale = nullptr, const float* shift = nullptr);
 hipError_t run_chain(hpe_ctx* c, int i2c, bool first, const float* t2, const float* res, int B, float* t3, float* u1, hipStream_t st,
diff --git a/human-pose-estimation_amd/csrc/hpe_encoder.hip b/human-pose-estimation_amd/csrc/hpe_encoder.hip
--- a/human-pose-estimation_amd/csrc/hpe_encoder.hip
+++ b/human-pose-estimation_amd/csrc/hpe_encoder.hip
@@ -66,6 +66,13 @@
     p.cin_slabs = s.cin / (c->bf16 ? 64 : 32);
     p.relu = relu, p.y_slab8 = r.out_slab8 ? 1 : 0;
     if (r.mode == GEMM_STEM) p.Hi = STEM_HP, p.Wi = STEM_WP, p.Cin = 4;
+    if (r.stream) {
+        if (!L.w_stream || !res) return hipErrorInvalidValue;
+        p.w = reinterpret_cast<const float*>(L.w_stream);
+        p.w_piece = p.ldw;
+        p.ldw *= 3;
+        return hpe_launch_stream_f32s(p, GEMM_DENSE, c->plan.stream1x1_walkers, st);
+    }
     return launch_gemm(c, p, r, L.w_split, st);
 }
 
@@ -80,7 +87,7 @@
     return run_conv(c, idx, r, x, B, res, relu, y, st, c->wino_v, 0, scale, shift);
 }
 
-static hipError_t run_dual(hpe_ctx* c, int i2c, int i1, const ConvRoute& r, const float* t2, const float* x, int B, float* y, hipStream_t st) {
+hipError_t run_dual(hpe_ctx* c, int i2c, int i1, const ConvRoute& r, const float* t2, const float* x, int B, float* y, hipStream_t st) {
     const ConvSpec& s2 = specs()[i2c];
     const ConvSpec& s1 = specs()[i1];
     const ConvLayer& L = c->conv[i2c];
@@ -90,6 +97,13 @@
     p.k1_slabs = L.k1_dual / (c->bf16 ? 64 : 32), p.relu = 1;
     p.lda = s2.cin, p.ldw = L.k_dual, p.w_rows = round_up(s2.cout, 128), p.ldy = s2.cout;
     p.Hi = p.Wi = s1.hin, p.Cin = s1.cin, p.Ho = p.Wo = s1.hout, p.stride = s1.stride;
+    if (r.stream) {
+        if (!L.w_dual_stream) return hipErrorInvalidValue;
+        p.w = reinterpret_cast<const float*>(L.w_dual_stream);
+        p.w_piece = p.ldw;
+        p.ldw *= 3;
+        return hpe_launch_stream_f32s(p, GEMM_DUAL, c->plan.stream1x1_walkers, st);
+    }
     return launch_gemm(c, p, r, L.w_dual_split, st);
 }
 
diff --git a/human-pose-estimation_amd/csrc/hpe_finalize.hip b/human-pose-estimation_amd/csrc/hpe_finalize.hip
--- a/human-pose-estimation_amd/csrc/hpe_finalize.hip
+++ b/human-pose-estimation_amd/csrc/hpe_finalize.hip
@@ -67,6 +67,19 @@
             d[2 * K] = h[2];
         }
     return upload_bf16(c, p, ws);
+}
+
+static void append_split(std::vector<float>& wt, int rows, int K) {
+    const size_t nw = (size_t)rows * K;
+    std::vector<unsigned short> ws(nw * 3);
+    for (int n = 0; n < rows; ++n)
+        for (int k = 0; k < K; ++k) {
+            unsigned short h[3];
+            bf16_split3(wt[(size_t)n * K + k], h);
+            for (int j = 0; j < 3; ++j) ws[((size_t)n * 3 + j) * K + k] = h[j];
+        }
+    wt.resize(nw + nw * 3 / 2);
+    memcpy(wt.data() + nw, ws.data(), ws.size() * 2);
 }
 
 #pragma GCC visibility push(default)
@@ -220,8 +233,11 @@
         if (c->bf16) {
             if ((rc = upload_bf16(c, &L2.w_dual, to_bf16(wt)))) return rc;
         } else {
+            const bool stream = stream1x1_dual(c->plan, c->bf16, blk), derived = stream && !(packs & PACK_W_DUAL_SPLIT);
+            if (derived) append_split(wt, n_pad, K);
             if ((rc = upload_to(c, &L2.w_dual, wt))) return rc;
             if ((packs & PACK_W_DUAL_SPLIT) && (rc = upload_split(c, &L2.w_dual_split, wt, n_pad, K))) return rc;
+            if (stream) L2.w_dual_stream = derived ? w_stream_of(L2.w_dual, n_pad, K) : static_cast<unsigned short*>(L2.w_dual_split);
         }
         if ((rc = upload_to(c, &L2.shift_dual, sh))) return rc;
         L2.k_dual = K;
@@ -319,8 +335,11 @@
         if (c->bf16) {
             if ((rc = upload_bf16(c, &L.w, to_bf16(wt)))) return rc;
         } else {
+            const bool stream = stream1x1_layer(c->plan, c->bf16, i), derived = stream && !(packs & PACK_W_SPLIT);
+            if (derived) append_split(wt, L.n_pad, L.k_pad);
             if ((rc = upload_to(c, &L.w, wt))) return rc;
             if ((packs & PACK_W_SPLIT) && (rc = upload_split(c, &L.w_split, wt, L.n_pad, L.k_pad))) return rc;
+            if (stream) L.w_stream = derived ? w_stream_of(L.w, L.n_pad, L.k_pad) : static_cast<unsigned short*>(L.w_split);
             if ((packs & PACK_WINO_U) && (rc = pack_wino_weights(c, s, L))) return rc;
             if ((packs & PACK_WINO4_U) && (rc = pack_wino4_weights(c, s, L))) return rc;
         }
diff --git a/human-pose-estimation_amd/csrc/hpe_internal.h b/human-pose-estimation_amd/csrc/hpe_internal.h
--- a/human-pose-estimation_amd/csrc/hpe_internal.h
+++ b/human-pose-estimation_amd/csrc/hpe_internal.h
@@ -46,6 +46,9 @@
 
 hipError_t hpe_launch_gemm(GemmArgs p, int mode, int tile, int splitk_min_slabs, hipStream_t st, int* split_k_out = nullptr);
 hipError_t hpe_launch_gemm_f32s(GemmArgs p, int mode, int tile, hipStream_t st);
+bool hpe_stream_f32s_supported(int M, int N, int K);
+bool hpe_stream_f32s_dual_supported(int M, int N, int K1, int K2, int stride, int Hi, int Ho);
+hipError_t hpe_launch_stream_f32s(GemmArgs p, int mode, int max_walkers, hipStream_t st);
 
 size_t hpe_wino_v_floats(int B, int H, int W, int C);
 hipError_t hpe_wino_init_device();
diff --git a/human-pose-estimation_amd/csrc/hpe_plan.h b/human-pose-estimation_amd/csrc/hpe_plan.h
--- a/human-pose-estimation_amd/csrc/hpe_plan.h
+++ b/human-pose-estimation_amd/csrc/hpe_plan.h
@@ -22,6 +22,9 @@
     int min_chunk = 32;
     int halo3_two = 4;
     int f32s_min_tiles = 128;
+    int stream1x1 = 3;
+    int stream1x1_min_m = 25088;
+    int stream1x1_walkers = 0;
     int wino_streamk = 0;
     int concurrent_tiles = 0;
     int bf16_w8_min_tiles = 128;
@@ -50,6 +53,7 @@
 constexpr unsigned PACK_W_SPLIT = 1u << HPE_PACK_W_SPLIT, PACK_WINO_U = 1u << HPE_PACK_WINO_U, PACK_WINO4_U = 1u << HPE_PACK_WINO4_U,
                    PACK_STEM_W = 1u << HPE_PACK_STEM_W, PACK_W_DUAL = 1u << HPE_PACK_W_DUAL, PACK_W_DUAL_SPLIT = 1u << HPE_PACK_W_DUAL_SPLIT;
 unsigned layer_packs(const HpePlan& pl, bool bf16, int idx);
+bool stream1x1_layer(const HpePlan& pl, bool bf16, int idx);
 
 enum ConvKernel { CONV_K_F32 = 0, CONV_K_F32S, CONV_K_BF16, CONV_K_BF16_P8, CONV_K_HALO3, CONV_K_WINO, CONV_K_WINO_FUSED, CONV_K_WINO4, CONV_K_WINO4_FUSED };
 struct ConvQuery { int B; bool concurrent, residual, workspace; };
@@ -58,6 +62,7 @@
     bool in_slab8;
     bool out_slab8;
     bool concurrent;
+    bool stream;
 };
 enum BlockJoin { JOIN_SEPARATE = 0, JOIN_DUAL, JOIN_CHAIN };
 struct BlockRoute {
@@ -66,6 +71,7 @@
     bool u1_slab8;
 };
 struct ResBlock;
+bool stream1x1_dual(const HpePlan& pl, bool bf16, const ResBlock& blk);
 ConvRoute route_conv(const HpePlan& pl, bool bf16, int idx, const ConvQuery& q);
 BlockRoute route_block(const HpePlan& pl, bool bf16, const ResBlock& blk, ConvQuery q);
 int pick_tile(const HpePlan& pl, int M, int N, int K, bool residual_expand = false, bool concurrent = false);
diff --git a/human-pose-estimation_amd/csrc/hpe_plan.hip b/human-pose-estimation_amd/csrc/hpe_plan.hip
--- a/human-pose-estimation_amd/csrc/hpe_plan.hip
+++ b/human-pose-estimation_amd/csrc/hpe_plan.hip
@@ -102,6 +102,9 @@
     {&HpePlan::min_chunk, nullptr, "HPE_MIN_CHUNK", {32, 24}, {ANY, ANY}, NO_LO, NO_HI},
     {&HpePlan::halo3_two, nullptr, "HPE_HALO3_TWO", {4, 4}, {7, 7}, NO_LO, NO_HI},
     {&HpePlan::f32s_min_tiles, nullptr, "HPE_F32S_MIN_TILES", {128, 128}, {ANY, ANY}, NO_LO, NO_HI},
+    {&HpePlan::stream1x1, nullptr, "HPE_STREAM1X1", {3, 0}, {3, 0}, 0, 3},
+    {&HpePlan::stream1x1_min_m, nullptr, "HPE_STREAM1X1_MIN_M", {25088, 25088}, {ANY, ANY}, 1, NO_HI},
+    {&HpePlan::stream1x1_walkers, nullptr, "HPE_STREAM1X1_WALKERS", {0, 0}, {ANY, ANY}, 0, NO_HI},
     {&HpePlan::wino_streamk, nullptr, "HPE_WINO_STREAMK", {0, 0}, {ANY, ANY}, NO_LO, NO_HI},
     {&HpePlan::concurrent_tiles, nullptr, "HPE_CONCURRENT_TILES", {0, 0}, {ANY, ANY}, NO_LO, NO_HI},
     {&HpePlan::bf16_w8_min_tiles, nullptr, "HPE_BF16_W8_MIN_TILES", {128, 128}, {ANY, ANY}, NO_LO, NO_HI},
@@ -183,8 +186,26 @@
     return m;
 }
 
-static ConvRoute route_gemm(const HpePlan& pl, bool bf16, int mode, int M, int N, int K, bool expand, bool split_packed, bool concurrent) {
-    ConvRoute r{CONV_K_F32, mode, -1, false, false, concurrent};
+static bool use_chain(const HpePlan& pl, bool bf16, const ResBlock& blk);
+bool stream1x1_layer(const HpePlan& pl, bool bf16, int idx) {
+    if (bf16 || !(pl.stream1x1 & 1) || !pl.f32_split) return false;
+    const ConvSpec& s = specs()[idx];
+    for (const ResBlock& b : blocks())
+        if (b.i2c == idx && !b.first && !use_chain(pl, bf16, b))
+            return s.kh == 1 && s.stride == 1 && s.cout == 4 * s.cin && hpe_stream_f32s_supported(1, s.cout, conv_k_pad(idx, bf16));
+    return false;
+}
+
+bool stream1x1_dual(const HpePlan& pl, bool bf16, const ResBlock& blk) {
+    if (bf16 || !(pl.stream1x1 & 2) || !pl.f32_split || !blk.first || use_chain(pl, bf16, blk) || !(layer_packs(pl, bf16, blk.i2c) & PACK_W_DUAL)) return false;
+    const ConvSpec& s2 = specs()[blk.i2c];
+    const ConvSpec& s1 = specs()[blk.i1];
+    return hpe_stream_f32s_dual_supported(1, s2.cout, s2.cin, s1.cin, s1.stride, s1.hin, s1.hout);
+}
+
+static ConvRoute route_gemm(const HpePlan& pl, bool bf16, int mode, int M, int N, int K, bool expand, bool split_packed, bool concurrent,
+                            bool stream_layer = false) {
+    ConvRoute r{CONV_K_F32, mode, -1, false, false, concurrent, stream_layer && expand && M >= pl.stream1x1_min_m};
     if (bf16) {
         r.tile = pick_bf16(pl, M, N, K, expand, concurrent, mode);
         r.kernel = r.tile == TILE_P8_256x256 ? CONV_K_BF16_P8 : CONV_K_BF16;
@@ -214,7 +235,7 @@
         return special(CONV_K_WINO);
     if (bf16 && plain3 && (pl.halo3 & f4_bit(H)) && hpe_halo3_bf16_supported(H, s.cin, s.cout)) return special(CONV_K_HALO3);
     return route_gemm(pl, bf16, mode, B * s.hout * s.hout, s.cout, conv_k_pad(idx, bf16), mode == GEMM_DENSE && q.residual && s.cout == 4 * s.cin,
-                      (packs & PACK_W_SPLIT) != 0, q.concurrent);
+                      (packs & PACK_W_SPLIT) != 0, q.concurrent, stream1x1_layer(pl, bf16, idx));
 }
 
 static bool use_chain(const HpePlan& pl, bool bf16, const ResBlock& blk) {
@@ -247,6 +268,7 @@
         b.join = JOIN_DUAL;
         b.r2c = route_gemm(pl, bf16, GEMM_DUAL, q.B * s2.hout * s2.hout, s2.cout, s2.cin + specs()[blk.i1].cin, false,
                            (layer_packs(pl, bf16, blk.i2c) & PACK_W_DUAL_SPLIT) != 0, q.concurrent);
+        b.r2c.stream = stream1x1_dual(pl, bf16, blk) && q.B * s2.hout * s2.hout >= pl.stream1x1_min_m;
     } else {
         if (blk.first) b.r1 = route_conv(pl, bf16, blk.i1, q);
         q.residual = true;
diff --git a/human-pose-estimation_amd/engine.py b/human-pose-estimation_amd/engine.py
--- a/human-pose-estimation_amd/engine.py
+++ b/human-pose-estimation_amd/engine.py
@@ -847,6 +847,18 @@
     def conv_route(self, idx, B, concurrent=False, residual=False, workspace=True):
         return _lib.conv_route(self.lib, self._cfg, idx, B, concurrent, residual, workspace)
 
+    def debug_dual(self, idx2c, t2, x):
+        s = CONV_SPECS[idx2c]
+        t2 = _require_cuda_tensor(t2, "t2")
+        x = _require_cuda_tensor(x, "x")
+        B = t2.shape[0]
+        y = self._new(B, s.hout, s.hout, s.cout)
+        _lib.check(self.lib.hpe_debug_dual(self._h, int(idx2c), t2.data_ptr(), x.data_ptr(), B, y.data_ptr(), self._stream()))
+        return y
+
+    def conv_stream1x1(self, idx, B, concurrent=False, residual=True):
+        return int(self.lib.hpe_debug_conv_stream1x1(C.byref(self._cfg), int(idx), int(B), int(concurrent), int(residual)))
+
     def _debug_gemm(self, call, what, mode, tile, x, wt, y, M, N, K, kw):
         g = _lib.HpeDebugGemm()
         g.struct_size = C.sizeof(_lib.HpeDebugGemm)
diff --git a/include/hpe.h b/include/hpe.h
--- a/include/hpe.h
+++ b/include/hpe.h
@@ -412,6 +412,8 @@
     int reserved;
 } HpeConvRoute;
 int hpe_debug_conv_route(const HpeConfig* cfg, int idx, int B, int concurrent, int residual, int workspace, HpeConvRoute* out);
+int hpe_debug_conv_stream1x1(const HpeConfig* cfg, int idx, int B, int concurrent, int residual);
+int hpe_debug_dual(hpe_ctx* ctx, int idx2c, const float* t2_dev, const float* x_dev, int B, float* y_dev, void* stream);
 int hpe_debug_gemm(hpe_ctx* ctx, const float* x_dev, const float* wt_dev, int M, int N, int K, int w_rows, int tile,
                    const float* residual_dev, int relu, float* y_dev, void* stream);
 int hpe_debug_maxpool(const float* x_dev, int B, int H, int C, float* y_dev, void* stream);
```

Measured after the change: 22940 images/sec (median of 6 runs). +3.5%, better.
